# ziyangwang007/CV-SSL-MIS

Hardware: AMD Instinct MI355X
Metric: training images-or-volumes/sec/node (Mean-Teacher step) (higher is better)
Workload: dtype f32

## Files before the change

### cv-ssl-mis_amd/csrc/common.h

```cpp
#pragma once
#include <hip/hip_runtime.h>
#include <stdint.h>

#define MIS_OK 0
#define MIS_ERR_ARG (-1)
#define MIS_ERR_UNSUPPORTED (-2)
#define MIS_ERR_LAUNCH (-3)
#define MIS_ERR_WORKSPACE (-4)

#define MIS_NUM_XCD 8
#define MIS_WAVE 64

typedef float f32x4 __attribute__((ext_vector_type(4)));

typedef __bf16 mis_bf16x8 __attribute__((ext_vector_type(8)));
typedef unsigned mis_u32x4 __attribute__((ext_vector_type(4)));
struct MisBf3 { mis_u32x4 h, m, l; };

__device__ __forceinline__ void mis_bf3_split_pair(float x0, float x1, unsigned& h, unsigned& m, unsigned& l) {
    const unsigned u0 = __float_as_uint(x0), u1 = __float_as_uint(x1);
    h = __builtin_amdgcn_perm(u1, u0, 0x07060302u);
    const float r0 = x0 - __uint_as_float(u0 & 0xFFFF0000u), r1 = x1 - __uint_as_float(u1 & 0xFFFF0000u);
    const unsigned v0 = __float_as_uint(r0), v1 = __float_as_uint(r1);
    m = __builtin_amdgcn_perm(v1, v0, 0x07060302u);
// ... 81 lines not shown
__device__ __forceinline__ void dma_dwordx4(unsigned lds_byte, unsigned voff, i32x4 rsrc) {
    unsigned keep;
    asm volatile("s_mov_b32 %0, m0\n\ts_mov_b32 m0, %1\n\ts_nop 0\n\t"
                 "buffer_load_dwordx4 %2, %3, 0 offen lds\n\ts_mov_b32 m0, %0"
                 : "=&s"(keep) : "s"(lds_byte), "v"(voff), "s"(rsrc) : "memory");
}
__device__ __forceinline__ void dma_wait() { asm volatile("s_waitcnt vmcnt(0)" ::: "memory"); }

}

__device__ __forceinline__ float mis_dpp_f(float v, int ctrl) {
    switch (ctrl) {
        case 0: return __builtin_bit_cast(float, __builtin_amdgcn_update_dpp(0, __builtin_bit_cast(int, v), 0xB1, 0xF, 0xF, false));
        case 1: return __builtin_bit_cast(float, __builtin_amdgcn_update_dpp(0, __builtin_bit_cast(int, v), 0x4E, 0xF, 0xF, false));
        case 2: return __builtin_bit_cast(float, __builtin_amdgcn_update_dpp(0, __builtin_bit_cast(int, v), 0x141, 0xF, 0xF, false));
        default: return __builtin_bit_cast(float, __builtin_amdgcn_update_dpp(0, __builtin_bit_cast(int, v), 0x140, 0xF, 0xF, false));
    }
}
template <int LPR>
__device__ __forceinline__ float mis_group_sum(float v) {
    static_assert(LPR == 32 || LPR == 64, "row groups of 32 or 64 lanes");
    v += mis_dpp_f(v, 0);
    v += mis_dpp_f(v, 1);
    v += mis_dpp_f(v, 2);
    v += mis_dpp_f(v, 3);
    v += __builtin_bit_cast(float, __builtin_amdgcn_ds_swizzle(__builtin_bit_cast(int, v), (0x10 << 10) | 0x1F));
    if (LPR == 64) v += __shfl_xor(v, 32, 64);
    return v;
}

__device__ __forceinline__ float mis_sum8(float v) {
    v += mis_dpp_f(v, 0);
    v += mis_dpp_f(v, 1);
    v += mis_dpp_f(v, 2);
    return v;
}

template <int NCM>
__device__ __forceinline__ void mis_ln96_head_row(const float4 (&v)[3], const float4 (&g)[3], const float4 (&bt)[3],
                                                  const float4 (&wv)[NCM][3], float eps, float& mu, float& rs,
                                                  float (&pl)[NCM]) {
    float s = 0.f;
#pragma unroll
    for (int q = 0; q < 3; ++q) s += (v[q].x + v[q].y) + (v[q].z + v[q].w);
    mu = mis_sum8(s) / 96.f;
    float4 a[3];
    float ss = 0.f;
#pragma unroll
    for (int q = 0; q < 3; ++q) {
        a[q] = make_float4(v[q].x - mu, v[q].y - mu, v[q].z - mu, v[q].w - mu);
        ss += (a[q].x * a[q].x + a[q].y * a[q].y) + (a[q].z * a[q].z + a[q].w * a[q].w);
    }
    rs = 1.f / sqrtf(mis_sum8(ss) / 96.f + eps);
    float4 y[3];
#pragma unroll
    for (int q = 0; q < 3; ++q)
        y[q] = make_float4(a[q].x * rs * g[q].x + bt[q].x, a[q].y * rs * g[q].y + bt[q].y, a[q].z * rs * g[q].z + bt[q].z,
                           a[q].w * rs * g[q].w + bt[q].w);
#pragma unroll
    for (int n = 0; n < NCM; ++n) {
        float p = 0.f;
#pragma unroll
        for (int q = 0; q < 3; ++q) p += (y[q].x * wv[n][q].x + y[q].y * wv[n][q].y) + (y[q].z * wv[n][q].z + y[q].w * wv[n][q].w);
        pl[n] = mis_sum8(p);
    }
}

__device__ __forceinline__ float mis_wave_sum(float v) {
#pragma unroll
    for (int o = 32; o > 0; o >>= 1) v += __shfl_xor(v, o, 64);
    return v;
}

__device__ __forceinline__ double mis_wave_sum_d(double v) {
#pragma unroll
    for (int o = 32; o > 0; o >>= 1) v += __shfl_xor(v, o, 64);
    return v;
}

template <int NV>
__device__ __forceinline__ void mis_block_sum(float (&v)[NV], float* red) {
    const int lane = threadIdx.x & 63, wave = threadIdx.x >> 6;
#pragma unroll
    for (int i = 0; i < NV; ++i) v[i] = mis_wave_sum(v[i]);
    __syncthreads();
    if (lane == 0) {
#pragma unroll
        for (int i = 0; i < NV; ++i) red[wave * NV + i] = v[i];
    }
    __syncthreads();
    if (threadIdx.x == 0) {
        const int nw = blockDim.x >> 6;
#pragma unroll
        for (int i = 0; i < NV; ++i) {
            float s = 0.f;
            for (int w = 0; w < nw; ++w) s += red[w * NV + i];
            v[i] = s;
        }
    }
}

__device__ __forceinline__ void mis_philox4(uint32_t c0, uint32_t c1, uint32_t c2, uint32_t c3,
                                            uint32_t k0, uint32_t k1, uint32_t out[4]) {
#pragma unroll
    for (int r = 0; r < 10; ++r) {
        const uint64_t p0 = (uint64_t)0xD2511F53u * c0;
        const uint64_t p1 = (uint64_t)0xCD9E8D57u * c2;
        const uint32_t n0 = (uint32_t)(p1 >> 32) ^ c1 ^ k0;
        const uint32_t n1 = (uint32_t)p1;
        const uint32_t n2 = (uint32_t)(p0 >> 32) ^ c3 ^ k1;
        const uint32_t n3 = (uint32_t)p0;
        c0 = n0; c1 = n1; c2 = n2; c3 = n3;
        k0 += 0x9E3779B9u; k1 += 0xBB67AE85u;
    }
    out[0] = c0; out[1] = c1; out[2] = c2; out[3] = c3;
}

__device__ __forceinline__ float mis_u01(uint32_t r) { return (float)(r >> 8) * (1.0f / 16777216.0f); }

struct MisStepState {
    uint64_t seed;
    uint64_t offset;
    int64_t iter_num;
    float lr;
    float ema_alpha;
    float cons_weight;
    float cons_gate;
};

__device__ __forceinline__ void mis_gelu_parts(float x, float& cdf, float& u) {
    const float t = __builtin_amdgcn_rcpf(fmaf(0.3f, fabsf(x), 1.f));
    float p = 3.664988946e-02f;
    p = fmaf(p, t, -1.611761927e-01f);
    p = fmaf(p, t, 2.130432014e-01f);
    p = fmaf(p, t, -5.969779766e-02f);
    p = fmaf(p, t, 1.316696142e-01f);
    p = fmaf(p, t, 9.899286856e-02f);
    p = fmaf(p, t, 1.208983674e-01f);
    p = fmaf(p, t, 1.196200560e-01f);
    u = __builtin_amdgcn_exp2f(x * x * -0.72134752044448170f);
    const float e = p * t * u;
    cdf = x < 0.f ? e : 1.f - e;
}
__device__ __forceinline__ float mis_gelu(float x) {
    float cdf, u;
    mis_gelu_parts(x, cdf, u);
    return x * cdf;
}
__device__ __forceinline__ float mis_gelu_grad(float x) {
    float cdf, u;
    mis_gelu_parts(x, cdf, u);
    return fmaf(x * 0.3989422804014327f, u, cdf);
}
```

### cv-ssl-mis_amd/csrc/conv_fwd.hip

```cpp
#include "common.h"
#include <stdio.h>
#include <stdlib.h>

namespace {

struct ConvFwdArgs {
    const float* x; long long x_bs;
    const float* wp;
    const float* bias;
    float* y; long long y_bs;
    int N, Cin, Cout, Cin_pad, Cout_pad, D, H, W;
    int tiles_z, tiles_y, tiles_x, co_blocks;
    unsigned n_blocks, n_blocks_padded;
    int st2;
    float2* stat; long long stat_sc, stat_sn;
    int stagger, stagger_mod;
};

using namespace mis_dma;

template <int KD_, int KH_, int KW_, int TZ_, int TY_, int TX_, int CO_B_, int CI_B_, int NT_>
struct Cfg {
    static constexpr int KD = KD_, KH = KH_, KW = KW_, TZ = TZ_, TY = TY_, TX = TX_;
    static constexpr int CO_B = CO_B_, CI_B = CI_B_, NT = NT_;
// ... 218 lines not shown
            if (tid < C::CO_B) {
                const float2 p0 = red[tid], p1 = red[C::CO_B + tid], p2 = red[2 * C::CO_B + tid], p3 = red[3 * C::CO_B + tid];
                const long long tile = ((long long)tz * a.tiles_y + ty) * a.tiles_x + tx;
                a.stat[(long long)(co0 + tid) * a.stat_sc + (long long)n * a.stat_sn + tile] =
                    make_float2((p0.x + p1.x) + (p2.x + p3.x), (p0.y + p1.y) + (p2.y + p3.y));
            }
        }
        return;
    }
    float* __restrict__ yout = a.y + (long long)n * a.y_bs;
#pragma unroll
    for (int q = 0; q < C::NP; ++q) {
        const int p = (wave * C::NP + q) * 32 + 2 * lj;
        const int px = p % C::TX, py = (p / C::TX) % C::TY, pz = p / (C::TX * C::TY);
        const int gz = z0 + pz, gy = y0 + py, gx = x0 + px;
        const bool row_ok = gz < a.D && gy < a.H;
        const long long sp = ((long long)gz * a.H + gy) * a.W + gx;
#pragma unroll
        for (int m = 0; m < C::M; ++m) {
#pragma unroll
            for (int r = 0; r < 4; ++r) {
                const int co = co0 + m * 16 + lk * 4 + r;
                if (row_ok && co < a.Cout) {
                    const float bv = a.bias ? a.bias[co] : 0.f;
                    const float ve = acc[m][2 * q][r] + bv, vo = acc[m][2 * q + 1][r] + bv;
                    float* dst = yout + (long long)co * S + sp;
                    if (a.st2 && gx + 1 < a.W) {
                        *reinterpret_cast<float2*>(dst) = make_float2(ve, vo);
                    } else {
                        if (gx < a.W) dst[0] = ve;
                        if (gx + 1 < a.W) dst[1] = vo;
                    }
                }
            }
        }
    }
}

namespace small {
constexpr int TY = 8, TX = 64, HY = TY + 2, HX = TX + 2, RAW = HY * HX, NCH = (RAW + 63) / 64, XS = NCH * 64;
constexpr int CI = 16, LDS_BYTES = CI * XS * 4;
}

template <int STEP>
__device__ __forceinline__ void small_terms(const float* __restrict__ sx, int lane, const float* wreg, f32x4& acc0,
                                            f32x4& acc1) {
    if constexpr (STEP < small::CI * 12) {
        constexpr int c = STEP / 12, ir = (STEP % 12) / 3, dx = STEP % 3;
        const float b = sx[c * small::XS + ir * small::HX + dx + lane];
        if constexpr (ir <= 2) {
            constexpr int term = c * 9 + ir * 3 + dx;
            acc0 = __builtin_amdgcn_mfma_f32_4x4x1f32(wreg[term / 16], b, acc0, 4, term % 16, 0);
        }
        if constexpr (ir >= 1) {
            constexpr int term = c * 9 + (ir - 1) * 3 + dx;
            acc1 = __builtin_amdgcn_mfma_f32_4x4x1f32(wreg[term / 16], b, acc1, 4, term % 16, 0);
        }
        small_terms<STEP + 1>(sx, lane, wreg, acc0, acc1);
    }
}

__global__ __launch_bounds__(256) void conv_small_cout_kernel(const ConvFwdArgs a) {
    extern __shared__ __attribute__((aligned(16))) float mis_small_lds[];
    float* const sx = mis_small_lds;
    const unsigned L = mis_xcd_remap(blockIdx.x, a.n_blocks_padded);
    if (L >= a.n_blocks) return;
    const int tx = L % a.tiles_x, ty = (L / a.tiles_x) % a.tiles_y, n = L / (a.tiles_x * a.tiles_y);
    const int lane = threadIdx.x & 63;
    const int wave = __builtin_amdgcn_readfirstlane(threadIdx.x >> 6);
    const int y0 = ty * small::TY, x0 = tx * small::TX;
    const unsigned s_bytes = (unsigned)(a.H * a.W) * 4u;
    const i32x4 rx = make_rsrc(a.x + (long long)n * a.x_bs, (unsigned)a.Cin * s_bytes);
    const unsigned lds0 = lds_addr(sx);
#pragma unroll
    for (int p = 0; p < small::NCH; ++p) {
        const int e = p * 64 + lane;
        const int hy = e / small::HX, hx = e - hy * small::HX;
        const int gy = y0 + hy - 1, gx = x0 + hx - 1;
        const bool ok = e < small::RAW && (unsigned)gy < (unsigned)a.H && (unsigned)gx < (unsigned)a.W;
        const unsigned vo = ok ? (unsigned)(gy * a.W + gx) * 4u : OOB;
#pragma unroll
        for (int i = 0; i < 4; ++i) {
            const int c = wave + 4 * i;
            dma_dword(lds0 + (unsigned)(c * small::XS + p * 64) * 4u, vo + (unsigned)c * s_bytes, rx);
        }
    }
    float wreg[9];
#pragma unroll
    for (int k = 0; k < 9; ++k) {
        const int term = 16 * k + (lane >> 2);
        const int ci = term / 9;
        wreg[k] = ci < a.Cin_pad ? a.wp[(long long)term * a.Cout_pad + (lane & 3)] : 0.f;
    }
    dma_wait();
    __syncthreads();
    f32x4 acc[2] = {f32x4{0.f, 0.f, 0.f, 0.f}, f32x4{0.f, 0.f, 0.f, 0.f}};
    small_terms<0>(sx + (wave * 2) * small::HX, lane, wreg, acc[0], acc[1]);
#pragma unroll
    for (int r = 0; r < 2; ++r) {
        const int gy = y0 + wave * 2 + r, gx = x0 + lane;
        if (gy < a.H && gx < a.W) {
            float* __restrict__ o = a.y + (long long)n * a.y_bs + (long long)gy * a.W + gx;
#pragma unroll
            for (int m = 0; m < 4; ++m)
                if (m < a.Cout) o[(long long)m * a.H * a.W] = acc[r][m] + (a.bias ? a.bias[m] : 0.f);
        }
    }
}

template <int KD>
struct Cin1 {
    static constexpr int TZ = KD == 3 ? 4 : 1, TY = KD == 3 ? 8 : 32, TX = 16, WROWS = 8;
    static constexpr int HZ = TZ + KD - 1, HY = TY + 2, HX = TX + 2, HALO = HZ * HY * HX;
    static constexpr int TAPS = 9 * KD, NG = (TAPS + 3) / 4;
};

template <int KD>
__global__ __launch_bounds__(256) void conv_fwd_cin1_kernel(const ConvFwdArgs a) {
    using C = Cin1<KD>;
    __shared__ float sx[C::HALO];
    __shared__ float2 red[4 * 16];
    const unsigned L = mis_xcd_remap(blockIdx.x, a.n_blocks_padded);
    if (L >= a.n_blocks) return;
    unsigned t = L;
    const int tx = t % a.tiles_x; t /= a.tiles_x;
    const int ty = t % a.tiles_y; t /= a.tiles_y;
    const int tz = t % a.tiles_z; t /= a.tiles_z;
    const int n = t;
    const int z0 = tz * C::TZ, y0 = ty * C::TY, x0 = tx * C::TX;
    const int tid = threadIdx.x, lane = tid & 63, wave = tid >> 6, lk = lane >> 4, lj = lane & 15;
    const long long S = (long long)a.D * a.H * a.W;
    const float* __restrict__ xn = a.x + (long long)n * a.x_bs;
    for (int e = tid; e < C::HALO; e += 256) {
        const int hz = e / (C::HY * C::HX), r2 = e - hz * (C::HY * C::HX), hy = r2 / C::HX, hx = r2 - hy * C::HX;
        const int gz = z0 + hz - (KD == 3 ? 1 : 0), gy = y0 + hy - 1, gx = x0 + hx - 1;
        const bool ok = (unsigned)gz < (unsigned)a.D && (unsigned)gy < (unsigned)a.H && (unsigned)gx < (unsigned)a.W;
        sx[e] = ok ? xn[((long long)gz * a.H + gy) * a.W + gx] : 0.f;
    }
    float wa[C::NG];
    int toff[C::NG];
#pragma unroll
    for (int g = 0; g < C::NG; ++g) {
        const int tap = 4 * g + lk;
        wa[g] = tap < C::TAPS ? a.wp[tap * a.Cout_pad + lj] : 0.f;
        const int tc = tap < C::TAPS ? tap : C::TAPS - 1;
        toff[g] = ((tc / 9) * C::HY + (tc / 3) % 3) * C::HX + tc % 3;
    }
    float bv[4];
#pragma unroll
    for (int r = 0; r < 4; ++r) bv[r] = a.bias ? a.bias[lk * 4 + r] : 0.f;
    __syncthreads();
    const int wz = KD == 3 ? wave : 0, wy = KD == 3 ? 0 : wave * C::WROWS;
    const float* __restrict__ sb = sx + (wz * C::HY + wy) * C::HX + lj;
    float* __restrict__ yo = a.y + (long long)n * a.y_bs + ((long long)(z0 + wz) * a.H + y0 + wy) * a.W + x0 + lj;
    float s1[4] = {0.f, 0.f, 0.f, 0.f}, s2[4] = {0.f, 0.f, 0.f, 0.f};
#pragma unroll 2
    for (int row = 0; row < C::WROWS; ++row) {
        f32x4 acc = {0.f, 0.f, 0.f, 0.f};
#pragma unroll
        for (int g = 0; g < C::NG; ++g)
            acc = __builtin_amdgcn_mfma_f32_16x16x4f32(wa[g], sb[row * C::HX + toff[g]], acc, 0, 0, 0);
#pragma unroll
        for (int r = 0; r < 4; ++r) {
            const float v = acc[r] + bv[r];
            yo[(long long)(lk * 4 + r) * S + (long long)row * a.W] = v;
            s1[r] += v; s2[r] += v * v;
        }
    }
    if (a.stat) {
#pragma unroll
        for (int r = 0; r < 4; ++r)
#pragma unroll
            for (int o = 1; o < 16; o <<= 1) { s1[r] += __shfl_xor(s1[r], o, 64); s2[r] += __shfl_xor(s2[r], o, 64); }
        if (lj == 0) {
#pragma unroll
            for (int r = 0; r < 4; ++r) red[wave * 16 + lk * 4 + r] = make_float2(s1[r], s2[r]);
        }
        __syncthreads();
        if (tid < 16) {
            const float2 p0 = red[tid], p1 = red[16 + tid], p2 = red[32 + tid], p3 = red[48 + tid];
            const long long tile = ((long long)tz * a.tiles_y + ty) * a.tiles_x + tx;
            a.stat[(long long)tid * a.stat_sc + (long long)n * a.stat_sn + tile] =
                make_float2((p0.x + p1.x) + (p2.x + p3.x), (p0.y + p1.y) + (p2.y + p3.y));
        }
    }
}

int cin1_kd(const ConvFwdArgs& a, int kd, int kh, int kw) {
    if (kh != 3 || kw != 3 || a.Cin != 1 || a.Cout != 16) return 0;
    if (kd == 3 && a.D % Cin1<3>::TZ == 0 && a.H % Cin1<3>::TY == 0 && a.W % Cin1<3>::TX == 0) return 3;
    if (kd == 1 && a.D == 1 && a.H % Cin1<1>::TY == 0 && a.W % Cin1<1>::TX == 0) return 1;
    return 0;
}

template <int KD>
int launch_cin1(ConvFwdArgs a, hipStream_t stream) {
    using C = Cin1<KD>;
    a.tiles_z = a.D / C::TZ; a.tiles_y = a.H / C::TY; a.tiles_x = a.W / C::TX;
    const long long nb = (long long)a.N * a.tiles_z * a.tiles_y * a.tiles_x;
    if (nb <= 0 || nb > 0x7fffffffLL) return MIS_ERR_ARG;
    a.n_blocks = (unsigned)nb;
    a.n_blocks_padded = (unsigned)(mis_cdiv(nb, MIS_NUM_XCD) * MIS_NUM_XCD);
    hipLaunchKernelGGL(conv_fwd_cin1_kernel<KD>, dim3(a.n_blocks_padded), dim3(256), 0, stream, a);
    return mis_launch_status();
}

int launch_small_cout(ConvFwdArgs a, hipStream_t stream) {
    a.tiles_y = (int)mis_cdiv(a.H, small::TY);
    a.tiles_x = (int)mis_cdiv(a.W, small::TX);
    const long long nb = (long long)a.N * a.tiles_y * a.tiles_x;
    if (nb <= 0 || nb > 0x7fffffffLL) return MIS_ERR_ARG;
    a.n_blocks = (unsigned)nb;
    a.n_blocks_padded = (unsigned)(mis_cdiv(nb, MIS_NUM_XCD) * MIS_NUM_XCD);
    hipLaunchKernelGGL(conv_small_cout_kernel, dim3(a.n_blocks_padded), dim3(256), small::LDS_BYTES, stream, a);
    return mis_launch_status();
}

template <class C>
int launch_cfg(ConvFwdArgs a, hipStream_t stream) {
    a.tiles_z = (int)mis_cdiv(a.D, C::TZ);
    a.tiles_y = (int)mis_cdiv(a.H, C::TY);
    a.tiles_x = (int)mis_cdiv(a.W, C::TX);
    a.co_blocks = (int)mis_cdiv(a.Cout_pad, C::CO_B);
    const long long nb = (long long)a.N * a.tiles_z * a.tiles_y * a.tiles_x * a.co_blocks;
    if (nb <= 0 || nb > 0x7fffffffLL) return MIS_ERR_ARG;
    a.n_blocks = (unsigned)nb;
    a.n_blocks_padded = (unsigned)(mis_cdiv(nb, MIS_NUM_XCD) * MIS_NUM_XCD);
    static const int stagger = getenv("MIS_CF_STAGGER") ? atoi(getenv("MIS_CF_STAGGER")) : 0;
    static const int stagger_mod = getenv("MIS_CF_STAGGER_MOD") ? atoi(getenv("MIS_CF_STAGGER_MOD")) : 4;
    a.stagger = stagger; a.stagger_mod = stagger_mod;
    static std::atomic<unsigned long long> attr_done{0};
    if (mis_set_lds_attr(reinterpret_cast<const void*>(&conv_fwd_kernel<C>), C::LDS_BYTES, attr_done) != MIS_OK) return MIS_ERR_LAUNCH;
    hipLaunchKernelGGL(conv_fwd_kernel<C>, dim3(a.n_blocks_padded), dim3(256), C::LDS_BYTES, stream, a);
    return mis_launch_status();
}

}

extern "C" int mis_conv_cin_pad(int cin) { return (cin + 3) / 4 * 4; }
extern "C" int mis_conv_cout_pad(int cout) { return (cout + 15) / 16 * 16; }

namespace {

int dispatch_fwd(ConvFwdArgs a, int kd, int kh, int kw, hipStream_t stream, char* name, int name_len,
                 long long* stat_tiles = nullptr) {
#define MIS_CF(KD, KH, KW, TZ, TY, TX, COB, CIB, NT)                                                  \
    do {                                                                                              \
        if (stat_tiles) {    \
            const bool all = a.st2 && a.D % TZ == 0 && a.H % TY == 0 && a.W % TX == 0 && a.Cout % COB == 0;  \
            *stat_tiles = all ? (long long)(a.D / TZ) * (a.H / TY) * (a.W / TX) : 0;                  \
            return MIS_OK;                                                                            \
        }                                                                                             \
        if (name) {                                                                                   \
            snprintf(name, name_len, "conv_fwd_kernel<Cfg<%d, %d, %d, %d, %d, %d, %d, %d, %d>>", KD, KH, KW, \
                     TZ, TY, TX, COB, CIB, NT);                                                       \
            return MIS_OK;                                                                            \
        }                                                                                             \
        return launch_cfg<Cfg<KD, KH, KW, TZ, TY, TX, COB, CIB, NT>>(a, stream);                      \
    } while (0)
    const bool wide = a.Cout_pad >= 32 && a.Cout_pad % 32 == 0;
    if (const int c1 = cin1_kd(a, kd, kh, kw)) {
        if (stat_tiles) {
            *stat_tiles = c1 == 3 ? (long long)(a.D / Cin1<3>::TZ) * (a.H / Cin1<3>::TY) * (a.W / Cin1<3>::TX)
                                  : (long long)(a.H / Cin1<1>::TY) * (a.W / Cin1<1>::TX);
            return MIS_OK;
        }
        if (name) { snprintf(name, name_len, c1 == 3 ? "conv_fwd_cin1_kernel<3>" : "conv_fwd_cin1_kernel<1>"); return MIS_OK; }
        return c1 == 3 ? launch_cin1<3>(a, stream) : launch_cin1<1>(a, stream);
    }
    if (kd == 3 && kh == 3 && kw == 3) {
        if (a.W % 16 == 0 || a.W >= 64) {
            if (wide) MIS_CF(3, 3, 3, 4, 8, 16, 32, 4, 8); else MIS_CF(3, 3, 3, 4, 8, 16, 16, 4, 8);
        } else if (a.W % 8 == 0 && a.W >= 16) {
            const long long nb888 = (long long)a.N * mis_cdiv(a.D, 8) * mis_cdiv(a.H, 8) * mis_cdiv(a.W, 8) *
                                    mis_cdiv(a.Cout_pad, wide ? 32 : 16);
            if (nb888 < 512) {
                if (wide) MIS_CF(3, 3, 3, 4, 8, 8, 32, 4, 4); else MIS_CF(3, 3, 3, 4, 8, 8, 16, 4, 4);
            }
            if (wide) MIS_CF(3, 3, 3, 8, 8, 8, 32, 4, 8); else MIS_CF(3, 3, 3, 8, 8, 8, 16, 4, 8);
        } else if (a.W > 12) {
            if (wide) MIS_CF(3, 3, 3, 4, 4, 16, 32, 4, 4); else MIS_CF(3, 3, 3, 4, 4, 16, 16, 4, 4);
        } else if (a.W > 8) {
            MIS_CF(3, 3, 3, 2, 4, 16, 16, 4, 2);
        } else {
            MIS_CF(3, 3, 3, 2, 8, 8, 16, 4, 2);
        }
    }
    if (kd == 1 && kh == 3 && kw == 3) {
        if (a.D != 1) return MIS_ERR_UNSUPPORTED;
        if (a.Cout <= 4 && a.Cin_pad <= small::CI && a.H * (long long)a.W * (a.Cin + 1) * 4 < (1LL << 31)) {
            if (stat_tiles) { *stat_tiles = 0; return MIS_OK; }
            if (name) { snprintf(name, name_len, "conv_small_cout_kernel"); return MIS_OK; }
            return launch_small_cout(a, stream);
        }
        if (a.W >= 128) {
            if (wide) MIS_CF(1, 3, 3, 1, 16, 32, 32, 8, 8); else MIS_CF(1, 3, 3, 1, 16, 32, 16, 8, 8);
        } else {
            if (wide) MIS_CF(1, 3, 3, 1, 16, 16, 32, 8, 4); else MIS_CF(1, 3, 3, 1, 16, 16, 16, 8, 4);
        }
    }
    if (kd == 1 && kh == 1 && kw == 1) {
        if (a.D > 1) {
            if (wide) MIS_CF(1, 1, 1, 4, 8, 16, 32, 16, 8); else MIS_CF(1, 1, 1, 4, 8, 16, 16, 16, 8);
        } else if (a.W >= 32) {
            if (wide) MIS_CF(1, 1, 1, 1, 16, 32, 32, 16, 8); else MIS_CF(1, 1, 1, 1, 16, 32, 16, 16, 8);
        } else {
            if (wide) MIS_CF(1, 1, 1, 1, 16, 16, 32, 16, 4); else MIS_CF(1, 1, 1, 1, 16, 16, 16, 16, 4);
        }
    }
#undef MIS_CF
    return MIS_ERR_UNSUPPORTED;
}

ConvFwdArgs make_fwd_args(const float* x, long long x_bs, const float* wp, const float* bias, float* y,
                          long long y_bs, int N, int Cin, int Cout, int D, int H, int W) {
    ConvFwdArgs a{};
    a.x = x; a.x_bs = x_bs; a.wp = wp; a.bias = bias; a.y = y; a.y_bs = y_bs;
    a.N = N; a.Cin = Cin; a.Cout = Cout; a.D = D; a.H = H; a.W = W;
    a.Cin_pad = mis_conv_cin_pad(Cin);
    a.Cout_pad = mis_conv_cout_pad(Cout);
    a.st2 = (W % 2 == 0 && y_bs % 2 == 0 && ((uintptr_t)y & 7) == 0) ? 1 : 0;
    return a;
}

}

extern "C" int mis_conv_fwd(const float* x, long long x_bs, const float* wp, const float* bias,
                            float* y, long long y_bs, int N, int Cin, int Cout, int D, int H, int W,
                            int kd, int kh, int kw, hipStream_t stream) {
    if (!x || !wp || !y || N <= 0 || Cin <= 0 || Cout <= 0 || D <= 0 || H <= 0 || W <= 0) return MIS_ERR_ARG;
    const long long S = (long long)D * H * W;
    if (x_bs < (long long)Cin * S || y_bs < (long long)Cout * S) return MIS_ERR_ARG;
    if (((long long)Cin + 32) * S * 4 >= (1LL << 30) || ((uintptr_t)wp & 15) != 0) return MIS_ERR_UNSUPPORTED;
    return dispatch_fwd(make_fwd_args(x, x_bs, wp, bias, y, y_bs, N, Cin, Cout, D, H, W), kd, kh, kw, stream,
                        nullptr, 0);
}

extern "C" long long mis_conv_fwd_stat_tiles(int N, int Cin, int Cout, int D, int H, int W, int kd, int kh, int kw) {
    if (N <= 0 || Cin <= 0 || Cout <= 0 || D <= 0 || H <= 0 || W <= 0) return MIS_ERR_ARG;
    long long tiles = 0;
    const int st = dispatch_fwd(make_fwd_args(nullptr, 0, nullptr, nullptr, nullptr, 0, N, Cin, Cout, D, H, W), kd, kh,
                                kw, nullptr, nullptr, 0, &tiles);
    return st ? st : tiles;
}

extern "C" int mis_conv_fwd_stats(const float* x, long long x_bs, const float* wp, const float* bias, float* y,
                                  long long y_bs, int N, int Cin, int Cout, int D, int H, int W, int kd, int kh, int kw,
                                  float* stat, long long stat_sc, long long stat_sn, hipStream_t stream) {
    if (!x || !wp || !y || !stat || N <= 0 || Cin <= 0 || Cout <= 0 || D <= 0 || H <= 0 || W <= 0) return MIS_ERR_ARG;
    const long long S = (long long)D * H * W;
    if (x_bs < (long long)Cin * S || y_bs < (long long)Cout * S) return MIS_ERR_ARG;
    if (((long long)Cin + 32) * S * 4 >= (1LL << 30) || ((uintptr_t)wp & 15) != 0 || ((uintptr_t)stat & 7) != 0)
        return MIS_ERR_UNSUPPORTED;
    ConvFwdArgs a = make_fwd_args(x, x_bs, wp, bias, y, y_bs, N, Cin, Cout, D, H, W);
    long long tiles = 0;
    int st = dispatch_fwd(a, kd, kh, kw, nullptr, nullptr, 0, &tiles);
    if (st) return st;
    if (tiles <= 0) return MIS_ERR_UNSUPPORTED;
    a.stat = reinterpret_cast<float2*>(stat); a.stat_sc = stat_sc; a.stat_sn = stat_sn;
    return dispatch_fwd(a, kd, kh, kw, stream, nullptr, 0);
}

extern "C" int mis_conv_fwd_kernel_name(int N, int Cin, int Cout, int D, int H, int W, int kd, int kh, int kw,
                                        char* name, int name_len) {
    if (!name || name_len <= 0 || N <= 0 || Cin <= 0 || Cout <= 0 || D <= 0 || H <= 0 || W <= 0) return MIS_ERR_ARG;
    return dispatch_fwd(make_fwd_args(nullptr, 0, nullptr, nullptr, nullptr, 0, N, Cin, Cout, D, H, W), kd, kh, kw,
                        nullptr, name, name_len);
}
```

### cv-ssl-mis_amd/csrc/conv_wgrad_cin1.hip

```cpp
#include "common.h"

namespace {

template <int KD>
struct WC1 {
    static constexpr int TZ = KD == 3 ? 4 : 1, TY = KD == 3 ? 8 : 32, TX = 32;
    static constexpr int HZ = TZ + KD - 1, HY = TY + 2, HX = TX + 2, HALO = HZ * HY * HX;
    static constexpr int TAPS = 9 * KD, NG = (TAPS + 15) / 16;
};

struct Cin1Norm {
    const float* y; long long y_bs;
    const float* mean; const float* rstd; const float* gamma; const float* beta;
    const float2* sums;
    float slope;
    int per_sample;
};

struct Cin1Args {
    const float* x; long long x_bs;
    const float* dy; long long dy_bs;
    float* ws;
    int N, D, H, W;
    int tz, ty, tx, n_tiles;
};

template <int KD, bool NORM>
__global__ __launch_bounds__(256) void wgrad_cin1_kernel(const Cin1Args a, const Cin1Norm nb) {
    using C = WC1<KD>;
    constexpr int TZ = C::TZ, TY = C::TY, TX = C::TX, HY = C::HY, HX = C::HX, HALO = C::HALO, NG = C::NG;
    __shared__ float sx[HALO];
    const int tid = threadIdx.x, lane = tid & 63, wave = tid >> 6;
    const int lk = lane >> 4, lj = lane & 15;
    const long long S = (long long)a.D * a.H * a.W;
    int toff[NG];
#pragma unroll
    for (int g = 0; g < NG; ++g) {
        const int tap = g * 16 + lj < C::TAPS ? g * 16 + lj : C::TAPS - 1;
        toff[g] = ((tap / 9) * HY + (tap / 3) % 3) * HX + tap % 3;
    }
    f32x4 acc[NG];
#pragma unroll
    for (int g = 0; g < NG; ++g) acc[g] = f32x4{0.f, 0.f, 0.f, 0.f};
    const int wz = KD == 3 ? wave : 0, wy = KD == 3 ? 0 : wave * 8;
    for (int t = blockIdx.x; t < a.n_tiles; t += gridDim.x) {
        int r = t;
        const int bx = r % a.tx; r /= a.tx;
        const int by = r % a.ty; r /= a.ty;
        const int bz = r % a.tz; r /= a.tz;
        const int n = r;
        const int z0 = bz * TZ, y0 = by * TY, x0 = bx * TX;
        const float* __restrict__ xn = a.x + (long long)n * a.x_bs;
        __syncthreads();
        for (int e = tid; e < HALO; e += 256) {
            const int hz = e / (HY * HX), r2 = e - hz * (HY * HX), hy = r2 / HX, hx = r2 - hy * HX;
            const int gz = z0 + hz - (KD == 3 ? 1 : 0), gy = y0 + hy - 1, gx = x0 + hx - 1;
            const bool ok = (unsigned)gz < (unsigned)a.D && (unsigned)gy < (unsigned)a.H && (unsigned)gx < (unsigned)a.W;
            sx[e] = ok ? xn[((long long)gz * a.H + gy) * a.W + gx] : 0.f;
        }
        __syncthreads();
        const long long voff = (long long)lj * S + ((long long)(z0 + wz) * a.H + y0 + wy) * a.W + x0 + 4 * lk;
        const float* __restrict__ dyp = a.dy + (long long)n * a.dy_bs + voff;
        const float* __restrict__ yp = NORM ? nb.y + (long long)n * nb.y_bs + voff : nullptr;
        float cm = 0.f, crs = 1.f, cga = 1.f, cbe = 0.f, s1 = 0.f, s2 = 0.f;
        if constexpr (NORM) {
            const int grp = nb.per_sample ? n * 16 + lj : lj;
            cm = nb.mean[grp]; crs = nb.rstd[grp];
            cga = nb.gamma ? nb.gamma[lj] : 1.f; cbe = nb.beta ? nb.beta[lj] : 0.f;
            const float2 sm = nb.sums[grp];
            s1 = sm.x; s2 = sm.y;
        }
        const float* __restrict__ sb = sx + (wz * HY + wy) * HX + 4 * lk;
#pragma unroll 4
        for (int it = 0; it < 16; ++it) {
            const int row = it >> 1, half = it & 1;
            f32x4 d4 = *reinterpret_cast<const f32x4*>(dyp + (long long)row * a.W + half * 16);
            if constexpr (NORM) {
                const f32x4 y4 = *reinterpret_cast<const f32x4*>(yp + (long long)row * a.W + half * 16);
#pragma unroll
                for (int s = 0; s < 4; ++s) {
                    const float xh = (y4[s] - cm) * crs;
                    const float dz = xh * cga + cbe > 0.f ? d4[s] : d4[s] * nb.slope;
                    d4[s] = cga * crs * (dz - s1 - xh * s2);
                }
            }
            const float* __restrict__ sp = sb + row * HX + half * 16;
#pragma unroll
            for (int s = 0; s < 4; ++s) {
#pragma unroll
                for (int g = 0; g < NG; ++g)
                    acc[g] = __builtin_amdgcn_mfma_f32_16x16x4f32(d4[s], sp[toff[g] + s], acc[g], 0, 0, 0);
            }
        }
    }
    float* __restrict__ out = a.ws + ((long long)blockIdx.x * 4 + wave) * (NG * 256);
#pragma unroll
    for (int g = 0; g < NG; ++g)
#pragma unroll
        for (int r = 0; r < 4; ++r) out[g * 256 + (lk * 4 + r) * 16 + lj] = acc[g][r];
}

__global__ __launch_bounds__(256) void wgrad_cin1_reduce_kernel(const float* __restrict__ ws, float* __restrict__ dw,
                                                                int parts, int taps, int ng, int accumulate) {
    __shared__ float red[4];
    const int o = blockIdx.x;
    const int co = o / taps, tap = o - co * taps;
    const float* p = ws + (tap / 16) * 256 + co * 16 + tap % 16;
    float s = 0.f;
    for (int k = threadIdx.x; k < parts; k += 256) s += p[(long long)k * (ng * 256)];
#pragma unroll
    for (int d = 32; d > 0; d >>= 1) s += __shfl_xor(s, d, 64);
    if ((threadIdx.x & 63) == 0) red[threadIdx.x >> 6] = s;
    __syncthreads();
    if (threadIdx.x == 0) {
        s = (red[0] + red[1]) + (red[2] + red[3]);
        dw[o] = accumulate ? dw[o] + s : s;
    }
}

int grid_for(long long n_tiles) { return (int)(n_tiles < 1024 ? n_tiles : 1024); }

template <int KD>
long long tiles_of(int N, int D, int H, int W) {
    return (long long)N * (D / WC1<KD>::TZ) * (H / WC1<KD>::TY) * (W / WC1<KD>::TX);
}

template <int KD>
int launch_cin1_kd(const float* x, long long x_bs, const float* dy, long long dy_bs, const Cin1Norm* nb, float* dw,
                   float* ws, int N, int D, int H, int W, int accumulate, hipStream_t stream) {
    using C = WC1<KD>;
    Cin1Args a{};
    a.x = x; a.x_bs = x_bs; a.dy = dy; a.dy_bs = dy_bs; a.ws = ws;
    a.N = N; a.D = D; a.H = H; a.W = W;
    a.tz = D / C::TZ; a.ty = H / C::TY; a.tx = W / C::TX;
    const long long n_tiles = tiles_of<KD>(N, D, H, W);
    if (n_tiles > 0x7fffffffLL) return MIS_ERR_ARG;
    a.n_tiles = (int)n_tiles;
    const int grid = grid_for(n_tiles);
    if (nb) hipLaunchKernelGGL((wgrad_cin1_kernel<KD, true>), dim3(grid), dim3(256), 0, stream, a, *nb);
    else hipLaunchKernelGGL((wgrad_cin1_kernel<KD, false>), dim3(grid), dim3(256), 0, stream, a, Cin1Norm{});
    hipLaunchKernelGGL(wgrad_cin1_reduce_kernel, dim3(16 * C::TAPS), dim3(256), 0, stream, ws, dw, grid * 4, C::TAPS, C::NG,
                       accumulate);
    return mis_launch_status();
}

}

bool mis_wgrad_cin1_eligible(int N, int Cin, int Cout, int D, int H, int W, int kd, int kh, int kw) {
    if (kh != 3 || kw != 3 || Cin != 1 || Cout != 16) return false;
    if (kd == 3) return D % WC1<3>::TZ == 0 && H % WC1<3>::TY == 0 && W % WC1<3>::TX == 0;
    return kd == 1 && D == 1 && H % WC1<1>::TY == 0 && W % WC1<1>::TX == 0;
}

long long mis_wgrad_cin1_workspace_bytes(int N, int D, int H, int W) {
    return D == 1 ? (long long)grid_for(tiles_of<1>(N, D, H, W)) * 4 * WC1<1>::NG * 256 * 4
                  : (long long)grid_for(tiles_of<3>(N, D, H, W)) * 4 * WC1<3>::NG * 256 * 4;
}

static int launch_cin1(const float* x, long long x_bs, const float* dy, long long dy_bs, const Cin1Norm* nb, float* dw,
                       float* ws, long long ws_bytes, int N, int D, int H, int W, int accumulate, hipStream_t stream) {
    if (((uintptr_t)dy & 15) || dy_bs % 4) return MIS_ERR_UNSUPPORTED;
    if (ws_bytes < mis_wgrad_cin1_workspace_bytes(N, D, H, W)) return MIS_ERR_WORKSPACE;
    return D == 1 ? launch_cin1_kd<1>(x, x_bs, dy, dy_bs, nb, dw, ws, N, D, H, W, accumulate, stream)
                  : launch_cin1_kd<3>(x, x_bs, dy, dy_bs, nb, dw, ws, N, D, H, W, accumulate, stream);
}

int mis_wgrad_cin1(const float* x, long long x_bs, const float* dy, long long dy_bs, float* dw, float* ws,
                   long long ws_bytes, int N, int D, int H, int W, int accumulate, hipStream_t stream) {
    return launch_cin1(x, x_bs, dy, dy_bs, nullptr, dw, ws, ws_bytes, N, D, H, W, accumulate, stream);
}

extern "C" int mis_conv_wgrad_cin1_norm_eligible(int N, int Cout, int D, int H, int W) {
    return mis_wgrad_cin1_eligible(N, 1, Cout, D, H, W, D == 1 ? 1 : 3, 3, 3) ? 1 : 0;
}

extern "C" int mis_conv_wgrad_cin1_norm(const float* x, long long x_bs, const float* da, long long da_bs, const float* y,
                                        long long y_bs, int N, int D, int H, int W, int per_sample, const float* mean,
                                        const float* rstd, const float* gamma, const float* beta, const float* sums,
                                        float slope, float* dw, float* workspace, long long workspace_bytes,
                                        int accumulate, hipStream_t stream) {
    if (!x || !da || !y || !mean || !rstd || !sums || !dw || !workspace || N <= 0) return MIS_ERR_ARG;
    if (!mis_wgrad_cin1_eligible(N, 1, 16, D, H, W, D == 1 ? 1 : 3, 3, 3) || (per_sample && (gamma || beta)))
        return MIS_ERR_UNSUPPORTED;
    if (((uintptr_t)y & 15) || y_bs % 4 || ((uintptr_t)sums & 7)) return MIS_ERR_UNSUPPORTED;
    const Cin1Norm nb{y, y_bs, mean, rstd, gamma, beta, reinterpret_cast<const float2*>(sums), slope, per_sample};
    return launch_cin1(x, x_bs, da, da_bs, &nb, dw, workspace, workspace_bytes, N, D, H, W, accumulate, stream);
}
```

### cv-ssl-mis_amd/csrc/norm_act.hip

```cpp
#include "common.h"
#include <type_traits>

namespace {

struct Geo {
    int N, C, per_sample;
    long long S;
    long long x_bs;
    int P;
    int nchunks;
    int G;
    int cg;
};

__host__ __device__ inline int pick_P(long long S) {
    long long p = (S + 16383) / 16384;
    if (p < 1) p = 1;
    if (p > 32) p = 32;
    return (int)p;
}

Geo make_geo(int N, int C, long long S, long long x_bs, int per_sample, int cg = 1) {
    Geo g;
    g.N = N; g.C = C; g.S = S; g.x_bs = x_bs; g.per_sample = per_sample; g.cg = cg;
// ... 46 lines not shown
    long long So;
};

__device__ __forceinline__ void pool_grad4(const PoolGrad& pg, int n, int c, int C, unsigned e, float (&g)[4]) {
    const unsigned HW = (unsigned)(pg.H * pg.W);
    const unsigned z = e / HW, r = e - z * HW;
    const unsigned y = r / (unsigned)pg.W, x0 = r - y * (unsigned)pg.W;
    const unsigned zo = z / (unsigned)pg.pz;
    const unsigned o = (zo * ((unsigned)pg.H >> 1) + (y >> 1)) * ((unsigned)pg.W >> 1) + (x0 >> 1);
    const unsigned local = (z - zo * (unsigned)pg.pz) * 4u + (y & 1u) * 2u;
    const float2 d = *reinterpret_cast<const float2*>(pg.dp + (long long)n * pg.dp_bs + (long long)c * pg.So + o);
    const unsigned code = *reinterpret_cast<const unsigned short*>(pg.idx + ((long long)n * C + c) * pg.So + o);
    const unsigned c0 = code & 0xffu, c1 = code >> 8;
    g[0] = c0 == local ? d.x : 0.f;
    g[1] = c0 == local + 1u ? d.x : 0.f;
    g[2] = c1 == local ? d.y : 0.f;
    g[3] = c1 == local + 1u ? d.y : 0.f;
}

__device__ __forceinline__ void block_sum2_d(double (&v)[2], double* red) {
    const int lane = threadIdx.x & 63, wave = threadIdx.x >> 6;
    v[0] = mis_wave_sum_d(v[0]); v[1] = mis_wave_sum_d(v[1]);
    __syncthreads();
    if (lane == 0) { red[wave * 2] = v[0]; red[wave * 2 + 1] = v[1]; }
    __syncthreads();
    if (threadIdx.x == 0) {
        v[0] = ((red[0] + red[2]) + red[4]) + red[6];
        v[1] = ((red[1] + red[3]) + red[5]) + red[7];
    }
}

template <typename T2>
__global__ __launch_bounds__(256) void stats_partial_kernel(const float* __restrict__ x, Geo g,
                                                            T2* __restrict__ part) {
    __shared__ double red[8];
    const int p = blockIdx.x, k = blockIdx.y, grp = blockIdx.z;
    const int n = g.per_sample ? grp / g.C : k;
    const int c = g.per_sample ? grp % g.C : grp;
    const float* __restrict__ base = x + (long long)n * g.x_bs + (long long)c * g.S;
    const long long units = g.S >> 2;
    const long long per = (units + g.P - 1) / g.P;
    const long long u0 = p * per, u1 = (u0 + per < units) ? u0 + per : units;
    double v[2] = {0.0, 0.0};
    for (long long u = u0 + threadIdx.x; u < u1; u += 256) {
        const float4 q = *reinterpret_cast<const float4*>(base + u * 4);
        v[0] += ((double)q.x + (double)q.y) + ((double)q.z + (double)q.w);
        v[1] += ((double)q.x * q.x + (double)q.y * q.y) + ((double)q.z * q.z + (double)q.w * q.w);
    }
    block_sum2_d(v, red);
    if (threadIdx.x == 0) {
        T2 o;
        o.x = (decltype(o.x))v[0]; o.y = (decltype(o.y))v[1];
        part[((long long)grp * g.nchunks + k) * g.P + p] = o;
    }
}

template <typename T2>
__global__ __launch_bounds__(256) void stats_final_kernel(const T2* __restrict__ part, Geo g, float eps,
                                                          float* __restrict__ mean, float* __restrict__ rstd,
                                                          float* running_mean, float* running_var,
                                                          long long* num_batches, float momentum, int tpg) {
    constexpr bool WIDE = std::is_same<T2, double2>::value;
    __shared__ double red[16];
    const int lane = threadIdx.x & 63, wave = threadIdx.x >> 6;
    const int grp = tpg == 256 ? (int)blockIdx.x : (int)blockIdx.x * 4 + wave;
    const int t = tpg == 256 ? (int)threadIdx.x : lane;
    const int np = g.nchunks * g.P;
    double s = 0.0, ss = 0.0, sf = 0.0, ssf = 0.0;
    if (grp < g.G) {
        const T2* __restrict__ pg = part + (long long)grp * np;
        int i = t;
        for (; i + 3 * tpg < np; i += 4 * tpg) {
            const T2 q0 = pg[i], q1 = pg[i + tpg], q2 = pg[i + 2 * tpg], q3 = pg[i + 3 * tpg];
            s += q0.x; ss += q0.y; s += q1.x; ss += q1.y; s += q2.x; ss += q2.y; s += q3.x; ss += q3.y;
            if constexpr (WIDE) {
                sf += (float)q0.x; ssf += (float)q0.y; sf += (float)q1.x; ssf += (float)q1.y;
                sf += (float)q2.x; ssf += (float)q2.y; sf += (float)q3.x; ssf += (float)q3.y;
            }
        }
        for (; i < np; i += tpg) {
            const T2 q = pg[i];
            s += q.x; ss += q.y;
            if constexpr (WIDE) { sf += (float)q.x; ssf += (float)q.y; }
        }
    }
    s = mis_wave_sum_d(s); ss = mis_wave_sum_d(ss);
    if constexpr (WIDE) { sf = mis_wave_sum_d(sf); ssf = mis_wave_sum_d(ssf); }
    if (tpg == 256) {
        if (lane == 0) { red[wave] = s; red[4 + wave] = ss; red[8 + wave] = sf; red[12 + wave] = ssf; }
        __syncthreads();
        s = ((red[0] + red[1]) + red[2]) + red[3];
        ss = ((red[4] + red[5]) + red[6]) + red[7];
        sf = ((red[8] + red[9]) + red[10]) + red[11];
        ssf = ((red[12] + red[13]) + red[14]) + red[15];
    }
    if (grp < g.G && t == 0) {
        const double E = (double)g.nchunks * (double)g.S;
        double m = s / E;
        double var = ss / E - m * m;
        if (var < 0.0) var = 0.0;
        if constexpr (WIDE) {
            const double mf = sf / E;
            double vf = ssf / E - mf * mf;
            if (vf < 0.0) vf = 0.0;
            if (mf * mf <= 3.0 * vf) { m = mf; var = vf; }
        }
        mean[grp] = (float)m;
        rstd[grp] = (float)(1.0 / sqrt(var + (double)eps));
        if (running_mean && !g.per_sample) {
            const double unb = E > 1.0 ? var * E / (E - 1.0) : var;
            running_mean[grp] = (float)((1.0 - momentum) * running_mean[grp] + momentum * m);
            running_var[grp] = (float)((1.0 - momentum) * running_var[grp] + momentum * unb);
            if (num_batches && grp == 0) *num_batches += 1;
        }
    }
}

template <typename T2>
void launch_stats_final(const T2* part, const Geo& g, float eps, float* mean, float* rstd, float* running_mean,
                        float* running_var, long long* num_batches, float momentum, hipStream_t stream) {
    const int tpg = g.nchunks * g.P > 256 ? 256 : 64;
    hipLaunchKernelGGL(stats_final_kernel<T2>, dim3(tpg == 256 ? g.G : (g.G + 3) / 4), dim3(256), 0, stream, part, g, eps,
                       mean, rstd, running_mean, running_var, num_batches, momentum, tpg);
}

__global__ __launch_bounds__(256) void channel_sum_final_kernel(const float2* __restrict__ part, Geo g,
                                                                float* __restrict__ out, int accumulate) {
    const int grp = blockIdx.x * 4 + (threadIdx.x >> 6), lane = threadIdx.x & 63;
    if (grp >= g.G) return;
    const int np = g.nchunks * g.P;
    double s = 0.0;
    for (int i = lane; i < np; i += 64) s += part[(long long)grp * np + i].x;
    s = mis_wave_sum_d(s);
    if (lane == 0) out[grp] = accumulate ? out[grp] + (float)s : (float)s;
}

__global__ void running_to_stats_kernel(const float* __restrict__ rm, const float* __restrict__ rv, float eps,
                                        float* __restrict__ mean, float* __restrict__ rstd, int C) {
    const int c = blockIdx.x * blockDim.x + threadIdx.x;
    if (c < C) { mean[c] = rm[c]; rstd[c] = 1.f / sqrtf(rv[c] + eps); }
}

constexpr int APPLY_U = 4;

template <bool RES>
__global__ __launch_bounds__(256) void apply_fwd_kernel(const float* __restrict__ x, Geo g,
                                                        const float* __restrict__ mean,
                                                        const float* __restrict__ rstd,
                                                        const float* __restrict__ gamma,
                                                        const float* __restrict__ beta, float slope, DropCfg d,
                                                        float* __restrict__ y, long long y_bs, ResArgs ra) {
    const int c = blockIdx.y, n = blockIdx.z;
    const int grp = g.per_sample ? (n * g.C + c) / g.cg : c;
    const float sc = (gamma ? gamma[c] : 1.f) * rstd[grp];
    const float sh = (beta ? beta[c] : 0.f) - mean[grp] * sc;
    const float* __restrict__ xb = x + (long long)n * g.x_bs + (long long)c * g.S;
    float* __restrict__ yb = y + (long long)n * y_bs + (long long)c * g.S;
    const unsigned long long lbase = ((unsigned long long)n * g.C + c) * g.S;
    const long long units = g.S >> 2;
    const bool drop = d.p > 0.f;
#pragma unroll
    for (int i = 0; i < APPLY_U; ++i) {
        const long long u = ((long long)blockIdx.x * APPLY_U + i) * 256 + threadIdx.x;
        if (u >= units) break;
        const float4 q = *reinterpret_cast<const float4*>(xb + u * 4);
        float v[4] = {q.x * sc + sh, q.y * sc + sh, q.z * sc + sh, q.w * sc + sh};
        float4 rq = make_float4(0.f, 0.f, 0.f, 0.f);
        if constexpr (RES) {
            rq = *reinterpret_cast<const float4*>(ra.r + (long long)n * ra.r_bs + (long long)c * g.S + u * 4);
            if (!ra.post) { v[0] += rq.x; v[1] += rq.y; v[2] += rq.z; v[3] += rq.w; }
        }
#pragma unroll
        for (int j = 0; j < 4; ++j) v[j] = v[j] > 0.f ? v[j] : v[j] * slope;
        if constexpr (RES) {
            if (ra.post) { v[0] += rq.x; v[1] += rq.y; v[2] += rq.z; v[3] += rq.w; }
        }
        if (drop) {
            float s[4];
            drop_scale4(d, lbase + u * 4, (unsigned)(n * g.C + c), s);
#pragma unroll
            for (int j = 0; j < 4; ++j) v[j] *= s[j];
        }
        *reinterpret_cast<float4*>(yb + u * 4) = make_float4(v[0], v[1], v[2], v[3]);
    }
}

template <int PZ>
__global__ __launch_bounds__(256) void apply_fwd_pool_kernel(const float* __restrict__ x, Geo g,
                                                             const float* __restrict__ mean,
                                                             const float* __restrict__ rstd,
                                                             const float* __restrict__ gamma,
                                                             const float* __restrict__ beta, float slope, DropCfg d,
                                                             float* __restrict__ y, long long y_bs,
                                                             float* __restrict__ pooled, long long p_bs,
                                                             unsigned char* __restrict__ idx, int H, int W) {
    const int Ho = H >> 1, Wo = W >> 1, Wq = Wo >> 2;
    const int pl = blockIdx.x * 256 + threadIdx.x;
    if (pl >= Ho * Wq) return;
    const int zo = blockIdx.y, nc = blockIdx.z;
    const int n = nc / g.C, c = nc - n * g.C;
    const int yo = pl / Wq, xq = pl - yo * Wq;
    const int grp = g.per_sample ? (n * g.C + c) / g.cg : c;
    const float sc = (gamma ? gamma[c] : 1.f) * rstd[grp];
    const float sh = (beta ? beta[c] : 0.f) - mean[grp] * sc;
    const float* __restrict__ xb = x + (long long)n * g.x_bs + (long long)c * g.S;
    float* __restrict__ yb = y + (long long)n * y_bs + (long long)c * g.S;
    const unsigned long long lbase = ((unsigned long long)n * g.C + c) * g.S;
    const bool drop = d.p > 0.f;
    float best[4] = {-INFINITY, -INFINITY, -INFINITY, -INFINITY};
    unsigned bi[4] = {0, 0, 0, 0};
#pragma unroll
    for (int dz = 0; dz < PZ; ++dz)
#pragma unroll
        for (int dy = 0; dy < 2; ++dy) {
            const unsigned e = (unsigned)(((zo * PZ + dz) * H + (yo * 2 + dy)) * W + xq * 8);
            float v[8];
#pragma unroll
            for (int h = 0; h < 2; ++h) {
                const float4 q = *reinterpret_cast<const float4*>(xb + e + 4 * h);
                float t[4] = {q.x * sc + sh, q.y * sc + sh, q.z * sc + sh, q.w * sc + sh};
#pragma unroll
                for (int j = 0; j < 4; ++j) t[j] = t[j] > 0.f ? t[j] : t[j] * slope;
                if (drop) {
                    float s4[4];
                    drop_scale4(d, lbase + e + 4 * h, (unsigned)(n * g.C + c), s4);
#pragma unroll
                    for (int j = 0; j < 4; ++j) t[j] *= s4[j];
                }
                *reinterpret_cast<float4*>(yb + e + 4 * h) = make_float4(t[0], t[1], t[2], t[3]);
#pragma unroll
                for (int j = 0; j < 4; ++j) v[4 * h + j] = t[j];
            }
#pragma unroll
            for (int j = 0; j < 4; ++j)
#pragma unroll
                for (int dx = 0; dx < 2; ++dx) {
                    const float t = v[2 * j + dx];
                    if (t > best[j] || t != t) { best[j] = t; bi[j] = dz * 4 + dy * 2 + dx; }
                }
        }
    const long long So = (long long)gridDim.y * Ho * Wo;
    const unsigned o = (unsigned)((zo * Ho + yo) * Wo + xq * 4);
    *reinterpret_cast<float4*>(pooled + (long long)n * p_bs + (long long)c * So + o) =
        make_float4(best[0], best[1], best[2], best[3]);
    *reinterpret_cast<unsigned*>(idx + (long long)nc * So + o) = bi[0] | (bi[1] << 8) | (bi[2] << 16) | (bi[3] << 24);
}

template <bool DACC, bool RES = false>
__global__ __launch_bounds__(256) void bwd_partial_kernel(const float* __restrict__ x, Geo g,
                                                          const float* __restrict__ da, long long da_bs,
                                                          const float* __restrict__ mean,
                                                          const float* __restrict__ rstd,
                                                          const float* __restrict__ gamma,
                                                          const float* __restrict__ beta, float slope, DropCfg d,
                                                          float2* __restrict__ part, PoolGrad pg, ResArgs ra) {
    __shared__ double red[8];
    const int p = blockIdx.x, k = blockIdx.y, grp = blockIdx.z;
    const int n = g.per_sample ? grp / g.C : k;
    const int c = g.per_sample ? grp % g.C : grp;
    const int sg = g.per_sample ? grp / g.cg : grp;
    const float m = mean[sg], rs = rstd[sg];
    const float ga = gamma ? gamma[c] : 1.f, be = beta ? beta[c] : 0.f;
    const float* __restrict__ xb = x + (long long)n * g.x_bs + (long long)c * g.S;
    const float* __restrict__ db = da ? da + (long long)n * da_bs + (long long)c * g.S : nullptr;
    const unsigned long long lbase = ((unsigned long long)n * g.C + c) * g.S;
    const long long units = g.S >> 2;
    const long long per = (units + g.P - 1) / g.P;
    const long long u0 = p * per, u1 = (u0 + per < units) ? u0 + per : units;
    const bool drop = d.p > 0.f;
    typedef typename std::conditional<DACC, double, float>::type acc_t;
    acc_t v[2] = {0, 0};
    for (long long u = u0 + threadIdx.x; u < u1; u += 256) {
        const float4 q = *reinterpret_cast<const float4*>(xb + u * 4);
        const float4 gq = db ? *reinterpret_cast<const float4*>(db + u * 4) : make_float4(0.f, 0.f, 0.f, 0.f);
        const float xs[4] = {q.x, q.y, q.z, q.w};
        float gs[4] = {gq.x, gq.y, gq.z, gq.w};
        float rv[4] = {0.f, 0.f, 0.f, 0.f};
        if constexpr (RES) {
            const float4 rq = *reinterpret_cast<const float4*>(ra.r + (long long)n * ra.r_bs + (long long)c * g.S + u * 4);
            rv[0] = rq.x; rv[1] = rq.y; rv[2] = rq.z; rv[3] = rq.w;
        }
        if (pg.dp) {
            float pgr[4];
            pool_grad4(pg, n, c, g.C, (unsigned)(u * 4), pgr);
#pragma unroll
            for (int j = 0; j < 4; ++j) gs[j] += pgr[j];
        }
        if (drop) {
            float s[4];
            drop_scale4(d, lbase + u * 4, (unsigned)(n * g.C + c), s);
#pragma unroll
            for (int j = 0; j < 4; ++j) gs[j] *= s[j];
        }
#pragma unroll
        for (int j = 0; j < 4; ++j) {
            const float xh = (xs[j] - m) * rs;
            const float z = xh * ga + be + rv[j];
            const float dz = z > 0.f ? gs[j] : gs[j] * slope;
            v[0] += dz;
            v[1] += (acc_t)dz * (acc_t)xh;
        }
    }
    if constexpr (DACC) {
        block_sum2_d(v, red);
    } else {
        mis_block_sum<2>(v, reinterpret_cast<float*>(red));
    }
    if (threadIdx.x == 0) part[((long long)grp * g.nchunks + k) * g.P + p] = make_float2((float)v[0], (float)v[1]);
}

__global__ __launch_bounds__(256) void bwd_final_kernel(const float2* __restrict__ part, Geo g,
                                                        float2* __restrict__ sums, float* dgamma, float* dbeta,
                                                        int accumulate) {
    const int grp = blockIdx.x * 4 + (threadIdx.x >> 6), lane = threadIdx.x & 63;
    if (grp >= g.G) return;
    const int np = g.nchunks * g.P;
    double s1 = 0.0, s2 = 0.0;
    for (int i = lane; i < np; i += 64) {
        const float2 q = part[(long long)grp * np + i];
        s1 += q.x; s2 += q.y;
    }
    s1 = mis_wave_sum_d(s1); s2 = mis_wave_sum_d(s2);
    if (lane == 0) {
        const double E = (double)g.nchunks * (double)g.S;
        sums[grp] = make_float2((float)(s1 / E), (float)(s2 / E));
        if (dgamma && !g.per_sample) {
// ... 885 lines not shown
```

### cv-ssl-mis_amd/mis_hip/lib.py

```python
import ctypes
import os

import torch

_HERE = os.path.dirname(os.path.abspath(__file__))
LIB_PATH = os.environ.get("MIS_HIP_LIB") or os.path.join(_HERE, "libmis_hip.so")

_lib = None

_ERRORS = {
    -1: "MIS_ERR_ARG (bad pointer / size / stride)",
    -2: "MIS_ERR_UNSUPPORTED (shape not covered by the gfx950 kernel family)",
    -3: "MIS_ERR_LAUNCH (HIP launch failure)",
    -4: "MIS_ERR_WORKSPACE (workspace too small)",
}

c_p = ctypes.c_void_p
c_i = ctypes.c_int
c_ll = ctypes.c_longlong
c_f = ctypes.c_float
c_d = ctypes.c_double
c_u = ctypes.c_uint
c_ull = ctypes.c_ulonglong

PROTOTYPES = {
    "mis_abi_version": (c_i, []),
    "mis_conv_cin_pad": (c_i, [c_i]),
    "mis_conv_cout_pad": (c_i, [c_i]),
    "mis_conv_packed_floats": (c_ll, [c_i, c_i, c_i, c_i]),
    "mis_conv_pack_weights": (c_i, [c_p, c_p, c_i, c_i, c_i, c_i, c_p]),
    "mis_conv_pack_job_bytes": (c_i, []),
    "mis_conv_pack_job": (c_ll, [c_p, c_p, c_p, c_i, c_i, c_i, c_i, c_ll]),
    "mis_conv_pack_batch": (c_i, [c_p, c_i, c_ll, c_p]),
    "mis_conv_fwd": (c_i, [c_p, c_ll, c_p, c_p, c_p, c_ll, c_i, c_i, c_i, c_i, c_i, c_i, c_i, c_i, c_i, c_p]),
    "mis_conv_fwd_stat_tiles": (c_ll, [c_i, c_i, c_i, c_i, c_i, c_i, c_i, c_i, c_i]),
    "mis_conv_fwd_stats": (c_i, [c_p, c_ll, c_p, c_p, c_p, c_ll, c_i, c_i, c_i, c_i, c_i, c_i, c_i, c_i, c_i, c_p, c_ll,
                                 c_ll, c_p]),
    "mis_norm_stats_finalize": (c_i, [c_p, c_i, c_i, c_ll, c_i, c_i, c_f, c_p, c_p, c_p, c_p, c_p, c_f, c_p]),
    "mis_conv_fwd_kernel_name": (c_i, [c_i, c_i, c_i, c_i, c_i, c_i, c_i, c_i, c_i, ctypes.c_char_p, c_i]),
    "mis_conv3d_wino_select": (c_i, [c_i, c_i, c_i, c_i, c_i, c_i]),
    "mis_conv3d_wino_stat_tiles": (c_ll, [c_i, c_i, c_i, c_i]),
    "mis_conv3d_wino_kernel_name": (c_i, [c_i, ctypes.c_char_p, c_i]),
    "mis_conv3d_wino_fwd": (c_i, [c_p, c_ll, c_p, c_p, c_p, c_ll, c_i, c_i, c_i, c_i, c_i, c_i, c_p, c_ll, c_ll, c_i, c_p]),
    "mis_conv1x1_gemm_workspace_bytes": (c_ll, [c_i, c_i, c_i, c_ll]),
    "mis_conv1x1_gemm": (c_i, [c_p, c_ll, c_p, c_ll, c_p, c_p, c_ll, c_i, c_i, c_i, c_ll, c_i, c_p, c_ll, c_p]),
    "mis_conv1x1_wgrad_workspace_bytes": (c_ll, [c_i, c_i, c_i, c_ll]),
    "mis_conv1x1_wgrad": (c_i, [c_p, c_ll, c_p, c_ll, c_p, c_ll, c_i, c_i, c_i, c_ll, c_i, c_p, c_ll, c_p]),
    "mis_conv3d_wino_fwd_splits": (c_i, [c_i, c_i, c_i, c_i, c_i, c_i, c_i]),
    "mis_conv3d_wino_fwd_workspace_bytes": (c_ll, [c_i, c_i, c_i, c_i, c_i, c_i, c_i]),
    "mis_conv3d_wino_fwd_ws": (c_i, [c_p, c_ll, c_p, c_p, c_p, c_ll, c_i, c_i, c_i, c_i, c_i, c_i, c_p, c_ll, c_ll, c_i, c_p, c_ll,
                                     c_p]),
    "mis_conv3d_wino_dgrad_norm": (c_i, [c_p, c_ll, c_p, c_p, c_ll, c_i, c_i, c_i, c_i, c_i, c_i, c_p, c_ll, c_p, c_f, c_p,
                                         c_ll, c_ll, c_i, c_p]),
    "mis_norm_res_act_fwd": (c_i, [c_p, c_ll, c_p, c_ll, c_p, c_ll, c_i, c_i, c_ll, c_i, c_p, c_p, c_p, c_p, c_f, c_i, c_p]),
    "mis_norm_res_act_bwd": (c_i, [c_p, c_ll, c_p, c_ll, c_p, c_ll, c_p, c_ll, c_p, c_ll, c_i, c_i, c_i, c_ll, c_i, c_p, c_p,
                                   c_p, c_p, c_f, c_p, c_p, c_i, c_i, c_p, c_ll, c_p]),
    "mis_norm_act_bwd_tiles": (c_i, [c_p, c_ll, c_p, c_ll, c_p, c_ll, c_i, c_i, c_ll, c_p, c_p, c_f, c_p, c_i, c_p, c_p]),
    "mis_conv2d_wino_select": (c_i, [c_i, c_i, c_i, c_i, c_i]),
    "mis_conv2d_wino_stat_tiles": (c_ll, [c_i, c_i, c_i]),
    "mis_conv2d_wino_kernel_name": (c_i, [c_i, ctypes.c_char_p, c_i]),
    "mis_conv2d_wino_fwd": (c_i, [c_p, c_ll, c_p, c_p, c_p, c_ll, c_i, c_i, c_i, c_i, c_i, c_p, c_ll, c_ll, c_i, c_p]),
    "mis_conv2d_wino_wgrad_select": (c_i, [c_i, c_i, c_i, c_i, c_i]),
    "mis_conv2d_wino_wgrad_kernel_name": (c_i, [c_i, ctypes.c_char_p, c_i]),
    "mis_conv2d_wino_wgrad_workspace_bytes": (c_ll, [c_i, c_i, c_i, c_i, c_i, c_i]),
    "mis_conv2d_wino_wgrad": (c_i, [c_p, c_ll, c_p, c_ll, c_p, c_p, c_ll, c_i, c_i, c_i, c_i, c_i, c_i, c_i, c_p]),
    "mis_conv3d_wino_wgrad_select": (c_i, [c_i, c_i, c_i, c_i, c_i, c_i]),
    "mis_conv3d_wino_wgrad_kernel_name": (c_i, [c_i, ctypes.c_char_p, c_i]),
    "mis_conv3d_wino_wgrad_workspace_bytes": (c_ll, [c_i, c_i, c_i, c_i, c_i, c_i, c_i]),
    "mis_conv3d_wino_wgrad": (c_i, [c_p, c_ll, c_p, c_ll, c_p, c_p, c_ll, c_i, c_i, c_i, c_i, c_i, c_i, c_i, c_i, c_p]),
    "mis_conv_wgrad_workspace_bytes": (c_ll, [c_i, c_i, c_i, c_i, c_i, c_i, c_i, c_i, c_i]),
    "mis_conv_wgrad_kernel_name": (c_i, [c_i, c_i, c_i, c_i, c_i, c_i, c_i, c_i, c_i, ctypes.c_char_p, c_i]),
    "mis_conv_wgrad": (c_i, [c_p, c_ll, c_p, c_ll, c_p, c_p, c_ll, c_i, c_i, c_i, c_i, c_i, c_i, c_i, c_i, c_i,
                             c_i, c_p]),
    "mis_norm_workspace_bytes": (c_ll, [c_i, c_i, c_ll, c_i]),
    "mis_norm_stats": (c_i, [c_p, c_ll, c_i, c_i, c_ll, c_i, c_f, c_p, c_p, c_p, c_p, c_p, c_f, c_p, c_ll, c_p]),
    "mis_channel_sum": (c_i, [c_p, c_ll, c_i, c_i, c_ll, c_p, c_i, c_p, c_ll, c_p]),
    "mis_norm_stats_from_running":(c_i, [c_p, c_p, c_f, c_p, c_p, c_i, c_p]),
    "mis_norm_act_fwd": (c_i, [c_p, c_ll, c_p, c_ll, c_i, c_i, c_ll, c_i, c_p, c_p, c_p, c_p, c_f, c_f, c_u, c_p,
                               c_p, c_p]),
    "mis_norm_act_bwd": (c_i, [c_p, c_ll, c_p, c_ll, c_p, c_ll, c_i, c_i, c_ll, c_i, c_p, c_p, c_p, c_p, c_f, c_f,
                               c_u, c_p, c_p, c_p, c_p, c_i, c_p, c_ll, c_p]),
    "mis_norm_act_fwd_g": (c_i, [c_p, c_ll, c_p, c_ll, c_i, c_i, c_ll, c_i, c_i, c_p, c_p, c_p, c_p, c_f, c_f, c_u, c_p,
                                 c_p, c_p]),
    "mis_norm_act_bwd_g": (c_i, [c_p, c_ll, c_p, c_ll, c_p, c_ll, c_i, c_i, c_ll, c_i, c_i, c_i, c_p, c_p, c_p, c_p, c_f,
                                 c_f, c_u, c_p, c_p, c_p, c_p, c_i, c_p, c_ll, c_p]),
    "mis_norm_act_fwd_pool": (c_i, [c_p, c_ll, c_p, c_ll, c_p, c_ll, c_p, c_i, c_i, c_i, c_i, c_i, c_i, c_i, c_p, c_p, c_p,
                                    c_p, c_f, c_f, c_u, c_p, c_p, c_p]),
    "mis_norm_act_bwd_pool": (c_i, [c_p, c_ll, c_p, c_ll, c_p, c_ll, c_p, c_p, c_ll, c_i, c_i, c_i, c_i, c_i, c_i, c_i, c_p,
                                    c_p, c_p, c_p, c_f, c_f, c_u, c_p, c_p, c_p, c_p, c_i, c_p, c_ll, c_p]),
    "mis_norm_act_bwd_sums": (c_i, [c_p, c_ll, c_p, c_ll, c_i, c_i, c_ll, c_i, c_p, c_p, c_p, c_p, c_f, c_p, c_p, c_p, c_i,
                                    c_p, c_ll, c_p]),
    "mis_conv_wgrad_cin1_norm_eligible": (c_i, [c_i, c_i, c_i, c_i, c_i]),
    "mis_conv_wgrad_cin1_norm": (c_i, [c_p, c_ll, c_p, c_ll, c_p, c_ll, c_i, c_i, c_i, c_i, c_i, c_p, c_p, c_p, c_p, c_p,
                                       c_f, c_p, c_p, c_ll, c_i, c_p]),
    "mis_norm_head_eligible": (c_i, [c_i, c_i]),
    "mis_norm_head_workspace_bytes": (c_ll, [c_i, c_i, c_ll, c_i, c_i]),
    "mis_norm_head_fwd": (c_i, [c_p, c_ll, c_i, c_i, c_ll, c_i, c_p, c_p, c_p, c_p, c_f, c_f, c_u, c_p, c_p, c_p, c_p, c_i,
                                c_p, c_ll, c_p]),
    "mis_norm_head_bwd": (c_i, [c_p, c_ll, c_p, c_ll, c_p, c_ll, c_i, c_i, c_ll, c_i, c_p, c_p, c_p, c_p, c_f, c_f, c_u,
                                c_p, c_p, c_p, c_i, c_p, c_p, c_i, c_p, c_p, c_i, c_p, c_ll, c_p]),
    "mis_maxpool2_fwd": (c_i, [c_p, c_ll, c_p, c_ll, c_p, c_i, c_i, c_i, c_i, c_i, c_p]),
    "mis_maxpool2_bwd": (c_i, [c_p, c_ll, c_p, c_p, c_ll, c_i, c_i, c_i, c_i, c_i, c_i, c_p]),
    "mis_upsample2_fwd": (c_i, [c_p, c_ll, c_p, c_ll, c_i, c_i, c_i, c_i, c_i, c_i, c_p]),
    "mis_upsample2_bwd": (c_i, [c_p, c_ll, c_p, c_ll, c_i, c_i, c_i, c_i, c_i, c_i, c_i, c_p]),
    "mis_loss_tail_workspace_bytes": (c_ll, [c_i, c_i, c_ll]),
    "mis_loss_tail": (c_i, [c_p, c_ll, c_p, c_ll, c_p, c_i, c_i, c_i, c_i, c_ll, c_f, c_p, c_f, c_p, c_p, c_ll,
                            c_p, c_ll, c_p]),
    "mis_cross_teaching_tail_workspace_bytes": (c_ll, [c_i, c_i, c_ll]),
    "mis_cross_teaching_tail": (c_i, [c_p, c_ll, c_p, c_ll, c_p, c_i, c_i, c_i, c_i, c_ll, c_f, c_p, c_p, c_p, c_ll,
                                      c_p, c_ll, c_p]),
    "mis_softmax_mean_accumulate": (c_i, [c_p, c_ll, c_p, c_ll, c_i, c_i, c_i, c_ll, c_f, c_i, c_p]),
    "mis_uamt_tail_workspace_bytes": (c_ll, [c_i, c_i, c_ll]),
    "mis_uamt_tail": (c_i, [c_p, c_ll, c_p, c_ll, c_p, c_ll, c_p, c_i, c_i, c_i, c_i, c_ll, c_f, c_p, c_ll, c_d, c_f,
                            c_p, c_p, c_ll, c_p, c_ll, c_p]),
    "mis_beta_sample": (c_i, [c_p, c_i, c_d, c_u, c_p, c_p]),
    "mis_ict_mix": (c_i, [c_p, c_p, c_p, c_i, c_i, c_ll, c_p]),
    "mis_ict_tail_workspace_bytes": (c_ll, [c_i, c_i, c_ll]),
    "mis_ict_tail": (c_i, [c_p, c_ll, c_p, c_ll, c_p, c_ll, c_p, c_p, c_i, c_i, c_i, c_i, c_ll, c_f, c_p, c_f, c_p, c_p,
                           c_ll, c_p, c_ll, c_p]),
    "mis_rot90": (c_i, [c_p, c_ll, c_p, c_ll, c_i, c_i, c_i, c_i, c_p, c_ll, c_p, c_i, c_p]),
    "mis_dct_tail_workspace_bytes": (c_ll, [c_i, c_i, c_i, c_i, c_i]),
    "mis_dct_tail": (c_i, [c_p, c_ll, c_p, c_ll, c_p, c_i, c_i, c_i, c_i, c_i, c_i, c_p, c_ll, c_p, c_i, c_f, c_f, c_p, c_p,
                           c_ll, c_p, c_ll, c_p, c_ll, c_p]),
    "mis_grad_combine": (c_i, [c_p, c_p, c_ll, c_i, c_p]),
    "mis_triple_view_tail_workspace_bytes": (c_ll, [c_i, c_i, c_ll]),
    "mis_triple_view_tail": (c_i, [c_p, c_ll, c_p, c_ll, c_p, c_ll, c_p, c_i, c_i, c_i, c_i, c_ll, c_f, c_p, c_p, c_p, c_p,
                                   c_p, c_ll, c_p, c_ll, c_p, c_ll, c_p, c_ll, c_p]),
    "mis_cross_pseudo_tail": (c_i, [c_p, c_ll, c_p, c_ll, c_p, c_i, c_i, c_i, c_i, c_ll, c_f, c_p, c_i, c_p, c_p, c_ll,
                                    c_p, c_ll, c_p]),
    "mis_cross_pseudo_mt_tail": (c_i, [c_p, c_ll, c_p, c_ll, c_p, c_ll, c_p, c_i, c_i, c_i, c_i, c_ll, c_f, c_f, c_p,
                                       c_i, c_p, c_p, c_ll, c_p, c_ll, c_p]),
    "mis_dice_workspace_bytes": (c_ll, [c_i, c_i, c_ll]),
    "mis_dice_loss_fwd": (c_i, [c_p, c_ll, c_p, c_i, c_i, c_i, c_ll, c_p, c_p, c_p, c_ll, c_p]),
    "mis_dice_loss_bwd": (c_i, [c_p, c_ll, c_p, c_i, c_i, c_i, c_ll, c_p, c_p, c_p, c_ll, c_p]),
    "mis_softmax_mse": (c_i, [c_p, c_ll, c_p, c_ll, c_p, c_ll, c_p, c_ll, c_i, c_i, c_ll, c_i, c_p]),
    "mis_ema_update": (c_i, [c_p, c_p, c_ll, c_f, c_p]),
    "mis_sgd_ema_step": (c_i, [c_p, c_p, c_p, c_p, c_ll, c_f, c_f, c_f, c_f, c_f, c_p, c_p]),
    "mis_teacher_noise": (c_i, [c_p, c_p, c_ll, c_f, c_f, c_u, c_p, c_p]),
    "mis_step_init": (c_i, [c_p, c_ull, c_ll, c_d, c_d, c_d, c_d, c_d, c_ll, c_ll, c_i, c_p]),
    "mis_step_advance": (c_i, [c_p, c_d, c_d, c_d, c_d, c_d, c_ll, c_ll, c_i, c_p]),
    "mis_argmax_channels": (c_i, [c_p, c_ll, c_p, c_i, c_i, c_ll, c_p]),
    "mis_conv_k2s2_eligible": (c_i, [c_i, c_i, c_i, c_i, c_i, c_i]),
    "mis_conv_k2s2_down": (c_i, [c_p, c_ll, c_p, c_p, c_p, c_ll, c_i, c_i, c_i, c_i, c_i, c_i, c_i, c_p]),
    "mis_conv_k2s2_up": (c_i, [c_p, c_ll, c_p, c_p, c_p, c_ll, c_i, c_i, c_i, c_i, c_i, c_i, c_i, c_p]),
    "mis_conv_k2s2_wgrad_eligible": (c_i, [c_i, c_i, c_i, c_i, c_i]),
    "mis_conv_k2s2_wgrad_workspace_bytes": (c_ll, [c_i, c_i]),
    "mis_conv_k2s2_wgrad": (c_i, [c_p, c_ll, c_p, c_ll, c_p, c_i, c_i, c_i, c_i, c_i, c_i, c_i, c_p, c_ll, c_p]),
    "mis_debug_poison_lds": (c_i, [c_p, c_p]),
    "mis_debug_spin": (c_i, [c_i, c_i, c_i, c_p, c_p]),
    "mis_debug_wgrad_prof": (c_i, [c_p]),
    "mis_space_to_depth2": (c_i, [c_p, c_ll, c_p, c_ll, c_p, c_i, c_i, c_i, c_i, c_i, c_i, c_i, c_p]),
    "mis_space_to_depth2d": (c_i, [c_p, c_ll, c_p, c_ll, c_p, c_i, c_i, c_i, c_i, c_i, c_i, c_p]),
    "mis_add": (c_i, [c_p, c_ll, c_p, c_ll, c_p, c_ll, c_i, c_i, c_ll, c_p]),
    "mis_gemm_workspace_bytes": (c_ll, [c_i, c_i, c_i, c_i]),
    "mis_gemm_dw_workspace_bytes": (c_ll, [c_i, c_i, c_i]),
    "mis_gemm_dw": (c_i, [c_p, c_ll, c_p, c_ll, c_p, c_ll, c_p, c_i, c_i, c_i, c_i, c_p, c_ll, c_p]),
    "mis_gemm_dw_parts": (c_i, [c_p, c_ll, c_p, c_ll, c_p, c_ll, c_p, c_i, c_i, c_i, c_i, c_p, c_ll, c_p, c_p]),
    "mis_gemm_set_split_precision": (c_i, [c_i]),
    "mis_gemm_nt_kernel_name": (c_i, [c_i, c_i, c_i, c_i, ctypes.c_char_p, c_i]),
    "mis_gemm_tn_kernel_name": (c_i, [c_p, c_ll, c_p, c_ll, c_p, c_ll, c_i, c_i, c_i, ctypes.c_char_p, c_i]),
    "mis_gemm_expand_ln_head": (c_i, [c_p, c_ll, c_p, c_ll, c_p, c_i, c_i, c_i, c_i, c_i, c_i, c_p, c_p, c_p, c_i, c_f, c_p, c_p,
                                      c_p, c_ll, c_p]),
    "mis_gemm_split_bytes": (c_ll, [c_i, c_i]),
    "mis_gemm_split_b": (c_i, [c_p, c_ll, c_i, c_i, c_p, c_p]),
    "mis_gemm_split_b_layout": (c_i, [c_p, c_ll, c_i, c_i, c_p, c_i, c_p]),
    "mis_gemm_split_job_layout": (c_ll, [c_p, c_p, c_ll, c_i, c_i, c_p, c_ll, c_i]),
    "mis_gemm_nt_split_natural": (c_i, [c_i, c_i, c_i]),
    "mis_gemm_nt_split_layout": (c_i, [c_p, c_ll, c_p, c_p, c_ll, c_p, c_i, c_i, c_i, c_i, c_i, c_p, c_ll, c_p, c_ll, c_p, c_ll,
                                       c_i, c_i, c_i, c_i, c_p, c_ll, c_i, c_p]),
    "mis_gemm_nt_split_layout_kernel_name": (c_i, [c_i, c_i, c_i, c_i, c_i, ctypes.c_char_p, c_i]),
    "mis_gemm_expand_ln_head_split": (c_i, [c_p, c_ll, c_p, c_p, c_i, c_i, c_i, c_i, c_i, c_i, c_p, c_p, c_p, c_i, c_f, c_p, c_p, c_p,
                                            c_ll, c_p]),
    "mis_gemm_nt_residual_ln": (c_i, [c_p, c_ll, c_p, c_p, c_i, c_i, c_i, c_p, c_ll, c_p, c_ll, c_p, c_ll, c_p, c_p, c_f, c_p, c_ll,
                                      c_p, c_p, c_p]),
    "mis_gemm_split_job_bytes": (c_ll, []),
    "mis_gemm_split_job": (c_ll, [c_p, c_p, c_ll, c_i, c_i, c_p, c_ll]),
    "mis_gemm_split_batch": (c_i, [c_p, c_i, c_ll, c_p]),
    "mis_gemm_nt_split_workspace_bytes": (c_ll, [c_i, c_i, c_i]),
    "mis_gemm_nt_split": (c_i, [c_p, c_ll, c_p, c_p, c_ll, c_p, c_i, c_i, c_i, c_i, c_i, c_p, c_ll, c_p, c_ll, c_p, c_ll,
                                c_i, c_i, c_i, c_i, c_p, c_ll, c_p]),
    "mis_gemm_nt_split_kernel_name": (c_i, [c_i, c_i, c_i, c_i, ctypes.c_char_p, c_i]),
    "mis_gemm_expand": (c_i, [c_p, c_ll, c_p, c_ll, c_p, c_i, c_i, c_i, c_i, c_i, c_i, c_p]),
    "mis_gemm": (c_i, [c_p, c_ll, c_p, c_ll, c_p, c_ll, c_p, c_i, c_i, c_i, c_i, c_i, c_p, c_ll, c_p]),
    "mis_gemm_ex": (c_i, [c_p, c_ll, c_p, c_ll, c_p, c_ll, c_p, c_i, c_i, c_i, c_i, c_p, c_ll, c_p, c_ll, c_p, c_ll, c_p,
                          c_ll, c_p]),
    "mis_droppath_table": (c_i, [c_p, c_p, c_p, c_i, c_i, c_p, c_p]),
    "mis_transpose": (c_i, [c_p, c_ll, c_p, c_ll, c_i, c_i, c_p]),
    "mis_win3d_gather": (c_i, [c_p, c_p] + [c_i] * 12 + [c_p]),
    "mis_win3d_windows": (c_ll, [c_i] * 7),
    "mis_merge3d": (c_i, [c_p, c_p, c_i, c_i, c_i, c_i, c_i, c_i, c_p]),
    "mis_win3d_attn_fwd": (c_i, [c_p, c_ll, c_p, c_ll, c_p, c_p, c_p, c_i, c_i, c_i, c_i, c_p]),
    "mis_win3d_attn_workspace_bytes": (c_ll, [c_i, c_i, c_i]),
    "mis_win3d_attn_bwd": (c_i, [c_p, c_ll, c_p, c_p, c_ll, c_p, c_ll, c_p, c_p, c_p, c_p, c_i, c_i, c_i, c_i, c_i, c_p,
                                 c_ll, c_p]),
    "mis_transpose_job_bytes": (c_ll, []),
    "mis_transpose_job": (c_ll, [c_p, c_p, c_p, c_i, c_i, c_ll]),
    "mis_transpose_batch": (c_i, [c_p, c_i, c_ll, c_p]),
    "mis_layernorm_fwd": (c_i, [c_p, c_ll, c_p, c_ll, c_p, c_p, c_p, c_p, c_ll, c_i, c_f, c_p]),
    "mis_colreduce_workspace_bytes": (c_ll, [c_ll, c_i]),
    "mis_layernorm_bwd": (c_i, [c_p, c_ll, c_p, c_ll, c_p, c_ll, c_p, c_p, c_p, c_p, c_p, c_ll, c_i, c_i, c_i, c_p,
                                c_ll, c_p]),
    "mis_layernorm_bwd_parts": (c_i, [c_p, c_ll, c_p, c_ll, c_p, c_ll, c_p, c_p, c_p, c_ll, c_i, c_i, c_p, c_ll, c_p]),
    "mis_layernorm_bwd_final": (c_i, [c_p, c_ll, c_ll, c_i, c_p, c_p, c_i, c_p]),
    "mis_colsum_job_bytes": (c_ll, []),
    "mis_colreduce_slabs": (c_ll, [c_ll]),
    "mis_colsum_job": (c_ll, [c_p, c_p, c_ll, c_ll, c_i, c_i, c_p, c_p, c_i, c_ll]),
    "mis_colsum_batch": (c_i, [c_p, c_i, c_ll, c_p]),
    "mis_layernorm_bwd_residual_parts": (c_i, [c_p, c_ll, c_p, c_ll, c_p, c_ll, c_p, c_ll, c_i, c_p, c_ll, c_p, c_ll, c_p, c_p,
                                               c_p, c_ll, c_i, c_p, c_ll, c_p]),
    "mis_colsum": (c_i, [c_p, c_ll, c_ll, c_i, c_p, c_i, c_p, c_ll, c_p]),
    "mis_gelu": (c_i, [c_p, c_p, c_p, c_ll, c_i, c_p]),
    "mis_residual_droppath": (c_i, [c_p, c_ll, c_p, c_ll, c_p, c_ll, c_p, c_ll, c_ll, c_i, c_ll, c_f, c_u, c_p, c_p,
                                    c_i, c_p]),
    "mis_token_rearrange": (c_i, [c_p, c_ll, c_p, c_ll, c_i, c_i, c_i, c_i, c_i, c_i, c_i, c_p]),
    "mis_patch_im2col": (c_i, [c_p, c_ll, c_p, c_i, c_i, c_i, c_i, c_p]),
    "mis_ln_head_fwd": (c_i, [c_p, c_ll, c_p, c_p, c_p, c_p, c_p, c_p, c_ll, c_i, c_ll, c_i, c_i, c_f, c_p]),
    "mis_ln_head_workspace_bytes": (c_ll, [c_ll, c_i, c_i]),
    "mis_ln_head_bwd": (c_i, [c_p, c_ll, c_p, c_p, c_p, c_p, c_p, c_p, c_ll, c_p, c_ll, c_i, c_p, c_p, c_p, c_i, c_i, c_ll,
                              c_i, c_i, c_p, c_ll, c_p]),
    "mis_ln_head_bwd_unshuffle": (c_i, [c_p, c_ll, c_p, c_p, c_p, c_p, c_p, c_p, c_ll, c_p, c_ll, c_i, c_p, c_p, c_p, c_i, c_i, c_i,
                                        c_i, c_i, c_i, c_i, c_p, c_ll, c_p]),
    "mis_head_fwd": (c_i, [c_p, c_ll, c_p, c_p, c_ll, c_i, c_ll, c_i, c_i, c_p]),
    "mis_head_workspace_bytes": (c_ll, [c_i, c_i]),
    "mis_head_bwd": (c_i, [c_p, c_ll, c_p, c_p, c_ll, c_p, c_ll, c_p, c_i, c_i, c_ll, c_i, c_i, c_p, c_ll, c_p]),
    "mis_window_attention_fwd": (c_i, [c_p, c_ll, c_p, c_ll, c_p, c_i, c_i, c_i, c_i, c_i, c_f, c_p]),
    "mis_window_attention_workspace_bytes": (c_ll, [c_i, c_i, c_i, c_i]),
    "mis_window_attention_bwd": (c_i, [c_p, c_ll, c_p, c_ll, c_p, c_ll, c_p, c_p, c_i, c_i, c_i, c_i, c_i, c_i, c_f,
                                       c_p, c_ll, c_p]),
    "mis_patch_im2col_c": (c_i, [c_p, c_ll, c_p, c_i, c_i, c_i, c_i, c_i, c_p]),
    "mis_window_attention_fwd_ws": (c_i, [c_p, c_ll, c_p, c_ll, c_p, c_i, c_i, c_i, c_i, c_i, c_f, c_i, c_p]),
    "mis_window_attention_workspace_bytes_ws": (c_ll, [c_i, c_i, c_i, c_i, c_i]),
    "mis_window_attention_bwd_ws": (c_i, [c_p, c_ll, c_p, c_ll, c_p, c_ll, c_p, c_p, c_i, c_i, c_i, c_i, c_i, c_i, c_f,
                                          c_i, c_p, c_ll, c_p]),
    "mis_window_attention_bwd_parts_ws": (c_i, [c_p, c_ll, c_p, c_ll, c_p, c_ll, c_p, c_i, c_i, c_i, c_i, c_i, c_f, c_i, c_p,
                                                c_ll, c_p]),
    "mis_window_attention_dtable_ws": (c_i, [c_p, c_ll, c_p, c_i, c_i, c_i, c_i, c_i, c_i, c_p]),
    "mis_window_attention_table_partials": (c_i, [c_i, c_i, c_i, c_i, c_i, c_p, c_p]),
    "mis_full_attention_fwd": (c_i, [c_p, c_ll, c_p, c_ll, c_p, c_i, c_i, c_i, c_f, c_p]),
    "mis_full_attention_workspace_bytes": (c_ll, [c_i, c_i, c_i]),
    "mis_full_attention_bwd": (c_i, [c_p, c_ll, c_p, c_ll, c_p, c_ll, c_p, c_i, c_i, c_i, c_f, c_p, c_ll, c_p]),
    "mis_patch3d_im2col": (c_i, [c_p, c_ll, c_p, c_i, c_i, c_i, c_i, c_i, c_p]),
    "mis_add_rowcycle": (c_i, [c_p, c_ll, c_p, c_p, c_ll, c_ll, c_i, c_i, c_p]),
    "mis_sum_rowcycle": (c_i, [c_p, c_ll, c_p, c_ll, c_i, c_i, c_p]),
    "mis_augment2d": (c_i, [c_p, c_p, c_p, c_i, c_i, c_i, c_p, c_p, c_p]),
    "mis_crop_rotflip3d": (c_i, [c_p, c_p, c_p, c_i, c_i, c_i, c_i, c_p, c_p, c_i, c_p]),
    "mis_surface_metrics_workspace_bytes": (c_ll, [c_i, c_i, c_i]),
    "mis_surface_metrics": (c_i, [c_p, c_p, c_i, c_i, c_i, c_i, c_i, c_p, c_p, c_ll, c_p]),
# ... 176 lines not shown
```

### cv-ssl-mis_amd/mis_hip/ops.py

```python
import ctypes as _ctypes
import os as _os

import torch

from . import lib as _l

_scratch = {}


def _geom(t):
    if t.dim() != 5 or t.dtype != torch.float32:
        raise RuntimeError(f"expected 5-D fp32 [N,C,D,H,W], got {tuple(t.shape)} {t.dtype}")
    _l.require_gpu(t)
    N, C, D, H, W = t.shape
    S = D * H * W
    st = t.stride()
    if C > 1 and st[1] != S or (D > 1 and st[2] != H * W) or (H > 1 and st[3] != W) or (W > 1 and st[4] != 1):
        raise RuntimeError(f"activation view must be dense in (C,D,H,W); strides {st} shape {tuple(t.shape)}")
    bs = st[0] if N > 1 else max(st[0], C * S)
    if bs < C * S:
        bs = C * S
    return N, C, D, H, W, S, bs


# ... 372 lines not shown
        nb = L.mis_conv2d_wino_wgrad_workspace_bytes(N, Cin, Cout, H, W, wino2)
        if nb < 0:
            _l.check(nb, "mis_conv2d_wino_wgrad_workspace_bytes")
        ws = scratch(nb, "wgrad")
        _l.check(L.mis_conv2d_wino_wgrad(_l.ptr(x), xbs, _l.ptr(dy), dbs, _l.ptr(dw), _l.ptr(ws), ws.numel(), N, Cin, Cout,
                                         H, W, int(accumulate), wino2, _l.stream_ptr()), "mis_conv2d_wino_wgrad")
        buf = _ctypes.create_string_buffer(96)
        _l.check(L.mis_conv2d_wino_wgrad_kernel_name(wino2, buf, 96), "mis_conv2d_wino_wgrad_kernel_name")
        return buf.value.decode()
    nb = L.mis_conv_wgrad_workspace_bytes(N, Cin, Cout, D, H, W, kd, kh, kw)
    if nb < 0:
        _l.check(nb, "mis_conv_wgrad_workspace_bytes")
    ws = scratch(nb, "wgrad")
    _tag(f"direct_wgrad:k{kd}{kh}{kw}@{W}")
    _l.check(L.mis_conv_wgrad(_l.ptr(x), xbs, _l.ptr(dy), dbs, _l.ptr(dw), _l.ptr(ws), ws.numel(), N, Cin, Cout,
                              D, H, W, kd, kh, kw, int(accumulate), _l.stream_ptr()), "mis_conv_wgrad")
    buf = _ctypes.create_string_buffer(96)
    _l.check(L.mis_conv_wgrad_kernel_name(N, Cin, Cout, D, H, W, kd, kh, kw, buf, 96), "mis_conv_wgrad_kernel_name")
    return buf.value.decode()


def norm_stats(x, per_sample, eps, mean, rstd, running_mean=None, running_var=None, num_batches=None,
               momentum=0.1):
    L = _l.load()
    N, C, D, H, W, S, xbs = _geom(x)
    nb = L.mis_norm_workspace_bytes(N, C, S, int(per_sample))
    ws = scratch(nb, "norm")
    _l.check(L.mis_norm_stats(_l.ptr(x), xbs, N, C, S, int(per_sample), eps, _l.ptr(mean), _l.ptr(rstd),
                              _l.ptr(running_mean), _l.ptr(running_var), _l.ptr(num_batches), momentum,
                              _l.ptr(ws), ws.numel(), _l.stream_ptr()), "mis_norm_stats")


def channel_sum(x, out, accumulate=False):
    L = _l.load()
    N, C, D, H, W, S, xbs = _geom(x)
    nb = L.mis_norm_workspace_bytes(N, C, S, 0)
    ws = scratch(nb, "norm")
    _l.check(L.mis_channel_sum(_l.ptr(x), xbs, N, C, S, _l.ptr(out), int(accumulate), _l.ptr(ws), ws.numel(),
                               _l.stream_ptr()), "mis_channel_sum")


def norm_stats_from_running(running_mean, running_var, eps, mean, rstd):
    L = _l.load()
    _l.check(L.mis_norm_stats_from_running(_l.ptr(running_mean), _l.ptr(running_var), eps, _l.ptr(mean),
                                           _l.ptr(rstd), running_mean.numel(), _l.stream_ptr()),
             "mis_norm_stats_from_running")


def norm_act_fwd(x, y, per_sample, mean, rstd, gamma, beta, slope, drop_p=0.0, drop_salt=0, state=None,
                 drop_mask=None, cg=1):
    L = _l.load()
    N, C, D, H, W, S, xbs = _geom(x)
    _, _, _, _, _, _, ybs = _geom(y)
    _l.check(L.mis_norm_act_fwd_g(_l.ptr(x), xbs, _l.ptr(y), ybs, N, C, S, int(per_sample), int(cg), _l.ptr(mean),
                                  _l.ptr(rstd), _l.ptr(gamma), _l.ptr(beta), slope, drop_p, drop_salt,
                                  _l.ptr(state), _l.ptr(drop_mask), _l.stream_ptr()), "mis_norm_act_fwd_g")


def norm_act_bwd(x, da, dx, per_sample, mean, rstd, gamma, beta, slope, drop_p=0.0, drop_salt=0, state=None,
                 drop_mask=None, dgamma=None, dbeta=None, accumulate_affine=False, cg=1, no_norm=False):
    L = _l.load()
    N, C, D, H, W, S, xbs = _geom(x)
    _, _, _, _, _, _, dabs = _geom(da)
    _, _, _, _, _, _, dxbs = _geom(dx)
    nb = L.mis_norm_workspace_bytes(N, C, S, int(per_sample))
    ws = scratch(nb, "norm")
    _l.check(L.mis_norm_act_bwd_g(_l.ptr(x), xbs, _l.ptr(da), dabs, _l.ptr(dx), dxbs, N, C, S, int(per_sample),
                                  int(cg), int(no_norm), _l.ptr(mean), _l.ptr(rstd), _l.ptr(gamma), _l.ptr(beta),
                                  slope, drop_p, drop_salt, _l.ptr(state), _l.ptr(drop_mask), _l.ptr(dgamma),
                                  _l.ptr(dbeta), int(accumulate_affine), _l.ptr(ws), ws.numel(), _l.stream_ptr()),
             "mis_norm_act_bwd_g")


def norm_res_act_fwd(x, res, y, per_sample, mean, rstd, gamma, beta, slope, post=False):
    L = _l.load()
    N, C, D, H, W, S, xbs = _geom(x)
    rbs, ybs = _geom(res)[6], _geom(y)[6]
    _l.check(L.mis_norm_res_act_fwd(_l.ptr(x), xbs, _l.ptr(res), rbs, _l.ptr(y), ybs, N, C, S, int(per_sample),
                                    _l.ptr(mean), _l.ptr(rstd), _l.ptr(gamma), _l.ptr(beta), slope, int(post),
                                    _l.stream_ptr()), "mis_norm_res_act_fwd")


def norm_res_act_bwd(x, res, dy, dx, dres, accumulate_dres, per_sample, mean, rstd, gamma, beta, slope, dgamma=None,
                     dbeta=None, accumulate_affine=False, post=False):
    L = _l.load()
    N, C, D, H, W, S, xbs = _geom(x)
    rbs, dybs, dxbs, drbs = _geom(res)[6], _geom(dy)[6], _geom(dx)[6], _geom(dres)[6]
    ws = scratch(L.mis_norm_workspace_bytes(N, C, S, int(per_sample)), "norm")
    _l.check(L.mis_norm_res_act_bwd(_l.ptr(x), xbs, _l.ptr(res), rbs, _l.ptr(dy), dybs, _l.ptr(dx), dxbs, _l.ptr(dres),
                                    drbs, int(accumulate_dres), N, C, S, int(per_sample), _l.ptr(mean), _l.ptr(rstd),
                                    _l.ptr(gamma), _l.ptr(beta), slope, _l.ptr(dgamma), _l.ptr(dbeta),
                                    int(accumulate_affine), int(post), _l.ptr(ws), ws.numel(), _l.stream_ptr()),
             "mis_norm_res_act_bwd")


def norm_act_fwd_pool(x, y, pooled, idx, per_sample, mean, rstd, gamma, beta, slope, drop_p=0.0, drop_salt=0, state=None,
                      drop_mask=None, cg=1):
    L = _l.load()
    N, C, D, H, W, S, xbs = _geom(x)
    _, _, _, _, _, _, ybs = _geom(y)
    _, _, _, _, _, _, pbs = _geom(pooled)
    _l.check(L.mis_norm_act_fwd_pool(_l.ptr(x), xbs, _l.ptr(y), ybs, _l.ptr(pooled), pbs, _l.ptr(idx), N, C, D, H, W,
                                     int(per_sample), int(cg), _l.ptr(mean), _l.ptr(rstd), _l.ptr(gamma), _l.ptr(beta),
                                     slope, drop_p, drop_salt, _l.ptr(state), _l.ptr(drop_mask), _l.stream_ptr()),
             "mis_norm_act_fwd_pool")


def norm_act_bwd_pool(x, da, dpool, idx, dx, per_sample, mean, rstd, gamma, beta, slope, drop_p=0.0, drop_salt=0,
                      state=None, drop_mask=None, dgamma=None, dbeta=None, accumulate_affine=False, cg=1):
    L = _l.load()
    N, C, D, H, W, S, xbs = _geom(x)
    dabs = _geom(da)[6] if da is not None else 0
    _, _, _, _, _, _, dpbs = _geom(dpool)
    _, _, _, _, _, _, dxbs = _geom(dx)
    ws = scratch(L.mis_norm_workspace_bytes(N, C, S, int(per_sample)), "norm")
    _l.check(L.mis_norm_act_bwd_pool(_l.ptr(x), xbs, _l.ptr(da), dabs, _l.ptr(dpool), dpbs, _l.ptr(idx), _l.ptr(dx), dxbs,
                                     N, C, D, H, W, int(per_sample), int(cg), _l.ptr(mean), _l.ptr(rstd), _l.ptr(gamma),
                                     _l.ptr(beta), slope, drop_p, drop_salt, _l.ptr(state), _l.ptr(drop_mask),
                                     _l.ptr(dgamma), _l.ptr(dbeta), int(accumulate_affine), _l.ptr(ws), ws.numel(),
                                     _l.stream_ptr()), "mis_norm_act_bwd_pool")


def norm_act_bwd_sums(x, da, per_sample, mean, rstd, gamma, beta, slope, sums, dgamma=None, dbeta=None,
                      accumulate_affine=False):
    L = _l.load()
    N, C, D, H, W, S, xbs = _geom(x)
    _, _, _, _, _, _, dabs = _geom(da)
    ws = scratch(L.mis_norm_workspace_bytes(N, C, S, int(per_sample)), "norm")
    _l.check(L.mis_norm_act_bwd_sums(_l.ptr(x), xbs, _l.ptr(da), dabs, N, C, S, int(per_sample), _l.ptr(mean),
                                     _l.ptr(rstd), _l.ptr(gamma), _l.ptr(beta), slope, _l.ptr(sums), _l.ptr(dgamma),
                                     _l.ptr(dbeta), int(accumulate_affine), _l.ptr(ws), ws.numel(), _l.stream_ptr()),
             "mis_norm_act_bwd_sums")


def conv_wgrad_cin1_norm_eligible(N, Cout, D, H, W):
    return bool(_l.load().mis_conv_wgrad_cin1_norm_eligible(N, Cout, D, H, W))


def conv_wgrad_cin1_norm(x, da, y, per_sample, mean, rstd, gamma, beta, sums, slope, dw, accumulate=False):
    L = _l.load()
    N, Cin, D, H, W, S, xbs = _geom(x)
    _, _, _, _, _, _, dabs = _geom(da)
    _, Cout, _, _, _, _, ybs = _geom(y)
    nb = L.mis_conv_wgrad_workspace_bytes(N, Cin, Cout, D, H, W, 1 if D == 1 else 3, 3, 3)
    if nb < 0:
        _l.check(nb, "mis_conv_wgrad_workspace_bytes")
    ws = scratch(nb, "wgrad")
    _l.check(L.mis_conv_wgrad_cin1_norm(_l.ptr(x), xbs, _l.ptr(da), dabs, _l.ptr(y), ybs, N, D, H, W, int(per_sample),
                                        _l.ptr(mean), _l.ptr(rstd), _l.ptr(gamma), _l.ptr(beta), _l.ptr(sums), slope,
                                        _l.ptr(dw), _l.ptr(ws), ws.numel(), int(accumulate), _l.stream_ptr()),
             "mis_conv_wgrad_cin1_norm")


def norm_head_eligible(C, K, per_sample, gamma, beta, cg=1, no_norm=False):
    return bool(_l.load().mis_norm_head_eligible(C, K)) and cg == 1 and not no_norm and not (
        per_sample and (gamma is not None or beta is not None))


def norm_head_fwd(x, logits, per_sample, mean, rstd, gamma, beta, slope, w, b, drop_p=0.0, drop_salt=0, state=None,
                  drop_mask=None):
    L = _l.load()
    N, C, D, H, W, S, xbs = _geom(x)
    _, K, _, _, _, _, lbs = _geom(logits)
    _l.check(L.mis_norm_head_fwd(_l.ptr(x), xbs, N, C, S, int(per_sample), _l.ptr(mean), _l.ptr(rstd), _l.ptr(gamma),
                                 _l.ptr(beta), slope, drop_p, drop_salt, _l.ptr(state), _l.ptr(drop_mask), _l.ptr(w),
                                 _l.ptr(b), K, _l.ptr(logits), lbs, _l.stream_ptr()), "mis_norm_head_fwd")


def norm_head_bwd(x, dlogits, dx, per_sample, mean, rstd, gamma, beta, slope, w, dw, db, drop_p=0.0, drop_salt=0,
                  state=None, drop_mask=None, dgamma=None, dbeta=None, accumulate_affine=False, accumulate_w=False):
    L = _l.load()
    N, C, D, H, W, S, xbs = _geom(x)
    _, K, _, _, _, _, dlbs = _geom(dlogits)
    _, _, _, _, _, _, dxbs = _geom(dx)
    nb = L.mis_norm_head_workspace_bytes(N, C, S, int(per_sample), K)
    ws = scratch(nb, "norm")
    _l.check(L.mis_norm_head_bwd(_l.ptr(x), xbs, _l.ptr(dlogits), dlbs, _l.ptr(dx), dxbs, N, C, S, int(per_sample),
                                 _l.ptr(mean), _l.ptr(rstd), _l.ptr(gamma), _l.ptr(beta), slope, drop_p, drop_salt,
                                 _l.ptr(state), _l.ptr(drop_mask), _l.ptr(w), K, _l.ptr(dgamma), _l.ptr(dbeta),
                                 int(accumulate_affine), _l.ptr(dw), _l.ptr(db), int(accumulate_w), _l.ptr(ws),
                                 ws.numel(), _l.stream_ptr()), "mis_norm_head_bwd")


def group_norm_stats(x, cg, eps, mean, rstd):
    L = _l.load()
    N, C, D, H, W, S, xbs = _geom(x)
    G = C // cg
    nb = L.mis_norm_workspace_bytes(N, G, cg * S, 1)
    ws = scratch(nb, "norm")
    _l.check(L.mis_norm_stats(_l.ptr(x), xbs, N, G, cg * S, 1, eps, _l.ptr(mean), _l.ptr(rstd), None, None, None,
                              0.0, _l.ptr(ws), ws.numel(), _l.stream_ptr()), "mis_norm_stats")


def maxpool2_fwd(x, y, idx):
    L = _l.load()
    N, C, D, H, W, S, xbs = _geom(x)
    _, _, _, _, _, _, ybs = _geom(y)
    _l.check(L.mis_maxpool2_fwd(_l.ptr(x), xbs, _l.ptr(y), ybs, _l.ptr(idx), N, C, D, H, W, _l.stream_ptr()),
             "mis_maxpool2_fwd")


def maxpool2_bwd(dy, idx, dx, accumulate=False):
    L = _l.load()
    N, C, D, H, W, S, dxbs = _geom(dx)
    _, _, _, _, _, _, dybs = _geom(dy)
    _l.check(L.mis_maxpool2_bwd(_l.ptr(dy), dybs, _l.ptr(idx), _l.ptr(dx), dxbs, N, C, D, H, W, int(accumulate),
                                _l.stream_ptr()), "mis_maxpool2_bwd")


def upsample2_fwd(x, y, align_corners):
    L = _l.load()
    N, C, D, H, W, S, xbs = _geom(x)
    _, _, _, _, _, _, ybs = _geom(y)
    _l.check(L.mis_upsample2_fwd(_l.ptr(x), xbs, _l.ptr(y), ybs, N, C, D, H, W, int(align_corners),
                                 _l.stream_ptr()), "mis_upsample2_fwd")


def upsample2_bwd(dy, dx, align_corners, accumulate=False):
    L = _l.load()
    N, C, D, H, W, S, dxbs = _geom(dx)
    _, _, _, _, _, _, dybs = _geom(dy)
    _l.check(L.mis_upsample2_bwd(_l.ptr(dy), dybs, _l.ptr(dx), dxbs, N, C, D, H, W, int(align_corners),
                                 int(accumulate), _l.stream_ptr()), "mis_upsample2_bwd")


def loss_tail(student, teacher, label, labeled_bs, out, dlogits=None, cons_weight=0.0, state=None,
              loss_scale=1.0):
    L = _l.load()
    B, C, D, H, W, S, sbs = _geom(student)
    tbs = 0
    if teacher is not None:
        Bt, Ct, _, _, _, St, tbs = _geom(teacher)
        assert Bt == B - labeled_bs and Ct == C and St == S
    if label is not None:
        _l.require_gpu(label)
        assert label.is_contiguous() and label.dtype in (torch.uint8, torch.int64)
        assert label.numel() >= labeled_bs * S
    lb = 1 if (label is None or label.dtype == torch.uint8) else 8
    dbs = 0
    if dlogits is not None:
        dbs = _geom(dlogits)[6]
    nb = L.mis_loss_tail_workspace_bytes(B, C, S)
    ws = scratch(nb, "tail")
    _l.check(L.mis_loss_tail(_l.ptr(student), sbs, _l.ptr(teacher), tbs, _l.ptr(label), lb, B, labeled_bs, C, S,
                             cons_weight, _l.ptr(state), loss_scale, _l.ptr(out), _l.ptr(dlogits), dbs,
                             _l.ptr(ws), ws.numel(), _l.stream_ptr()), "mis_loss_tail")


def softmax_mean_accumulate(logits, acc, repeats, scale, first):
    L = _l.load()
    Bl, C, D, H, W, S, lbs = _geom(logits)
    U, Ca, _, _, _, Sa, abs_ = _geom(acc)
    assert Bl == repeats * U and Ca == C and Sa == S
    _l.check(L.mis_softmax_mean_accumulate(_l.ptr(logits), lbs, _l.ptr(acc), abs_, U, repeats, C, S, scale,
                                           int(first), _l.stream_ptr()), "mis_softmax_mean_accumulate")


def uamt_tail(student, teacher, mean_probs, label, labeled_bs, out, max_iterations, dlogits=None, cons_weight=0.0,
              state=None, iter_num=0, loss_scale=1.0):
    L = _l.load()
    B, C, D, H, W, S, sbs = _geom(student)
    Bt, Ct, _, _, _, St, tbs = _geom(teacher)
    Bm, Cm, _, _, _, Sm, mbs = _geom(mean_probs)
    assert Bt == Bm == B - labeled_bs and Ct == Cm == C and St == Sm == S
    _l.require_gpu(label)
    assert label.is_contiguous() and label.dtype in (torch.uint8, torch.int64) and label.numel() >= labeled_bs * S
    lb = 1 if label.dtype == torch.uint8 else 8
    dbs = _geom(dlogits)[6] if dlogits is not None else 0
    nb = L.mis_uamt_tail_workspace_bytes(B, C, S)
    ws = scratch(nb, "tail")
    _l.check(L.mis_uamt_tail(_l.ptr(student), sbs, _l.ptr(teacher), tbs, _l.ptr(mean_probs), mbs, _l.ptr(label), lb,
                             B, labeled_bs, C, S, cons_weight, _l.ptr(state), int(iter_num), float(max_iterations),
                             loss_scale, _l.ptr(out), _l.ptr(dlogits), dbs, _l.ptr(ws), ws.numel(),
                             _l.stream_ptr()), "mis_uamt_tail")


ICT_BETA_SALT = 0x1C7BE7A0


def beta_sample(lam, alpha, state, salt=ICT_BETA_SALT):
    L = _l.load()
    _l.require_gpu(lam, state)
    assert lam.dtype == torch.float32 and lam.is_contiguous() and lam.numel() > 0
    if not float(alpha) > 0.0:
        raise ValueError(f"Beta(alpha, alpha) needs alpha > 0, got {alpha}")
    _l.check(L.mis_beta_sample(_l.ptr(lam), lam.numel(), float(alpha), int(salt) & 0xFFFFFFFF, _l.ptr(state),
                               _l.stream_ptr()), "mis_beta_sample")


def ict_mix(x, lam, labeled_bs, out):
    L = _l.load()
    _l.require_gpu(x, lam, out)
    M = lam.numel()
    assert x.dtype == out.dtype == lam.dtype == torch.float32
    assert x.is_contiguous() and out.is_contiguous() and lam.is_contiguous()
    assert x.shape[0] == labeled_bs + 2 * M and out.shape[0] == labeled_bs + M
    assert tuple(x.shape[1:]) == tuple(out.shape[1:])
    n = x[0].numel()
    _l.check(L.mis_ict_mix(_l.ptr(x), _l.ptr(out), _l.ptr(lam), labeled_bs, M, n, _l.stream_ptr()), "mis_ict_mix")


def ict_tail(student, teacher0, teacher1, lam, label, labeled_bs, out, dlogits=None, cons_weight=0.0, state=None,
             loss_scale=1.0):
    L = _l.load()
    B, C, D, H, W, S, sbs = _geom(student)
    M = B - labeled_bs
# ... 218 lines not shown
```

### cv-ssl-mis_amd/mis_hip/plan.py

```python
import itertools
import math
import os

import torch
import torch.nn as nn

from . import lib as _lib
from . import ops

_net_ids = itertools.count(1)

FUSE_CONV_STATS = os.environ.get("MIS_FUSE_STATS", "1") != "0"
FUSE_HEAD = os.environ.get("MIS_FUSE_HEAD", "1") != "0"
FUSE_FIRST = os.environ.get("MIS_FUSE_FIRST", "1") != "0"
FUSE_POOL = os.environ.get("MIS_FUSE_POOL", "1") != "0"
FUSE_POOL_FWD = os.environ.get("MIS_FUSE_POOL_FWD", "1") != "0"
WGRAD_STREAM = os.environ.get("MIS_WGRAD_STREAM", "1") != "0"
FUSE_DGRAD_NORM = os.environ.get("MIS_FUSE_DGRAD_NORM", "1") != "0"
PROGRESS_SYNC_MAIN = os.environ.get("MIS_PROGRESS_SYNC_MAIN", "0") == "1"
NORM_RES = os.environ.get("MIS_NORM_RES", "1") != "0"


class Act:

    def __init__(self, shape=None, parent=None, c0=0, C=None, tensor=None):
        self.parent, self.c0 = parent, c0
        self._written = False
        self.g = None
        if tensor is not None:
            self.t = tensor
        elif parent is not None:
            self.t = parent.t[:, c0:c0 + C]
        else:
            self.t = torch.empty(shape, dtype=torch.float32, device="cuda")

    @property
    def shape(self):
        return tuple(self.t.shape)

    def slice(self, c0, C):
        return Act(parent=self, c0=c0, C=C)

    def grad(self):
        if self.g is None:
            if self.parent is not None:
                self.g = self.parent.grad()[:, self.c0:self.c0 + self.t.shape[1]]
            else:
                self.g = torch.empty(self.shape, dtype=torch.float32, device="cuda")
        return self.g

    def _root(self):
        a = self
        while a.parent is not None:
            a = a.parent
        return a

    @property
    def written(self):
        return self._written or self._root()._written

    def mark_written(self):
        self._written = True

    def reset(self):
        self._written = False


class Ctx:

    def __init__(self, training, state=None, drop_masks=None, dropout=True, rng_stream=0):
        self.training = training
        self.rng_stream = rng_stream
        self.dropout = dropout
        self.state = state
        self.drop_masks = drop_masks


class ConvOp:
    def __init__(self, x, y, w, b, ksize, need_dx, bias_grad):
        self.x, self.y, self.w, self.b = x, y, w, b
        self.ksize, self.need_dx, self.bias_grad = tuple(ksize), need_dx, bias_grad
        self.cout, self.cin = w.data.shape[0], w.data.shape[1]
        N, _, D, H, W = y.shape
        self.wino_f = ops.conv_wino_select(N, self.cin, self.cout, D, H, W, self.ksize)
        self.wino_b = ops.conv_wino_select(N, self.cout, self.cin, D, H, W, self.ksize) if need_dx else -1
        self.wp = None
        self.wpd = None
        self.batched = False
        self.stat = None
        self.stat_norm = None
        self._dx_tmp = None
        self.fused_into = None
        self.norm_bwd = None
        self.dgrad_norm = None

    def fwd(self, ctx):
        if self.fused_into is not None:
            return
        if not self.batched:
            self.wp = ops.conv_pack(self.w.data, ops.conv_wino_pack_mode(self.wino_f, False) if self.wino_f >= 0 else 0,
                                    out=self.wp)
        stat = self.stat if (self.stat is not None and (self.stat_norm.per_sample or ctx.training)) else None
        ops.conv_fwd(self.x.t, self.wp, None if self.b is None else self.b.data, self.y.t, self.cin, self.cout,
                     self.ksize, stat=stat, wino=self.wino_f)

    def bwd(self, ctx):
        if self.fused_into is not None:
            return
        if self.norm_bwd is not None:
            n = self.norm_bwd
            ops.conv_wgrad_cin1_norm(self.x.t, n.y.grad(), self.y.t, n.per_sample, n.mean, n.rstd,
                                     None if n.gamma is None else n.gamma.data, None if n.beta is None else n.beta.data,
                                     n.sums, n.slope, self.w.grad)
            return
        dy = self.y.grad()
        side = getattr(ctx, "wgrad_stream", None) if self.need_dx else None
        if side is not None:
            _lib.wait_stream(side, torch.cuda.current_stream())
            with torch.cuda.stream(side):
                run_deferred(ctx)
                ops.conv_wgrad(self.x.t, dy, self.w.grad, self.ksize)
                if self.b is not None and self.bias_grad:
                    ops.channel_sum(dy, self.b.grad)
        else:
            ops.conv_wgrad(self.x.t, dy, self.w.grad, self.ksize)
            if self.b is not None and self.bias_grad:
                ops.channel_sum(dy, self.b.grad)
        if self.need_dx:
            if not self.batched:
                self.wpd = ops.conv_pack(self.w.data, ops.conv_wino_pack_mode(self.wino_b, True) if self.wino_b >= 0 else 1,
                                         out=self.wpd)
            if self.x.written:
                if self._dx_tmp is None:
                    self._dx_tmp = torch.empty(self.x.shape, dtype=torch.float32, device="cuda")
                ops.conv_fwd(dy, self.wpd, None, self._dx_tmp, self.cout, self.cin, self.ksize, wino=self.wino_b)
                ops.add(self.x.grad(), self._dx_tmp, self.x.grad())
            elif self.dgrad_norm is not None:
                n = self.dgrad_norm
                ops.conv_dgrad_norm(dy, self.wpd, self.x.grad(), self.cout, self.cin, n.x.t, n.mean, n.slope, n.ext_part,
                                    self.wino_b)
                n.ext_ready = True
            else:
                ops.conv_fwd(dy, self.wpd, None, self.x.grad(), self.cout, self.cin, self.ksize, wino=self.wino_b)
            self.x.mark_written()


class NormActOp:

    def __init__(self, x, y, per_sample, gamma, beta, running, slope, drop_p, site, eps=1e-5, momentum=0.1, cg=1,
                 no_norm=False):
        self.x, self.y, self.per_sample = x, y, per_sample
        self.cg, self.no_norm = cg, no_norm
        self.gamma, self.beta, self.running = gamma, beta, running
        self.slope, self.drop_p, self.site, self.eps, self.momentum = slope, drop_p, site, eps, momentum
        self.salt = 0
        self.fused = None
        self.drop3d = False
        N, C = x.shape[0], x.shape[1]
        G = N * C // cg if per_sample else C
        self.mean = torch.zeros(G, dtype=torch.float32, device="cuda")
        self.rstd = torch.ones(G, dtype=torch.float32, device="cuda")
        self._p = 0.0
        self._mask = None
        self.pool = None
        self.sums = None
        self.ext_part = None
        self.ext_tiles, self.ext_ready, self.ext_sums = 0, False, None
        self.res = None
        self.res_post = False
        self.head = None
        self.head_w = self.head_b = None

    def fwd(self, ctx):
        if self.no_norm:
            pass
        elif not self.per_sample and not ctx.training:
            ops.norm_stats_from_running(self.running[0], self.running[1], self.eps, self.mean, self.rstd)
        else:
            rm, rv, nbt = self.running if (self.running is not None and ctx.training) else (None, None, None)
            if self.fused is not None:
                N, C = self.x.shape[0], self.x.shape[1]
                S = self.x.shape[2] * self.x.shape[3] * self.x.shape[4]
                ops.norm_stats_finalize(self.fused[0], N, C // self.cg, S * self.cg, self.fused[1] * self.cg,
                                        self.per_sample, self.eps, self.mean, self.rstd, rm, rv, nbt, self.momentum)
            elif self.cg > 1:
                ops.group_norm_stats(self.x.t, self.cg, self.eps, self.mean, self.rstd)
            else:
                ops.norm_stats(self.x.t, self.per_sample, self.eps, self.mean, self.rstd, rm, rv, nbt, self.momentum)
        self._p = self.drop_p if (ctx.training and ctx.dropout) else 0.0
        self._mask = ctx.drop_masks.get(self.site) if (ctx.drop_masks and self._p > 0) else None
        self.salt = ((ctx.rng_stream & 0x7FFF) << 16) | self.site | (0x80000000 if self.drop3d else 0)
        self._state = ctx.state
        if self._p > 0 and self._mask is None and ctx.state is None:
            raise RuntimeError("dropout is active but no device step state was supplied (Ctx.state)")
        if self.res is not None:
            ops.norm_res_act_fwd(self.x.t, self.res.t, self.y.t, self.per_sample, self.mean, self.rstd,
                                 None if self.gamma is None else self.gamma.data,
                                 None if self.beta is None else self.beta.data, self.slope, post=self.res_post)
            return
        if self.pool is not None and self.pool.fwd_fused:
            pl = self.pool
            ops.norm_act_fwd_pool(self.x.t, self.y.t, pl.y.t, pl.idx, self.per_sample, self.mean, self.rstd,
                                  None if self.gamma is None else self.gamma.data,
                                  None if self.beta is None else self.beta.data, self.slope, self._p, self.salt,
                                  self._state, self._mask, cg=self.cg)
            return
        if self.head is not None:
            h = self.head
            ops.norm_head_fwd(self.x.t, h.y.t, self.per_sample, self.mean, self.rstd,
                              None if self.gamma is None else self.gamma.data,
                              None if self.beta is None else self.beta.data, self.slope,
                              h.w.data.view(h.cout, h.cin), None if h.b is None else h.b.data, self._p, self.salt,
                              self._state, self._mask)
            return
        ops.norm_act_fwd(self.x.t, self.y.t, self.per_sample, self.mean, self.rstd,
                         None if self.gamma is None else self.gamma.data,
                         None if self.beta is None else self.beta.data, self.slope, self._p, self.salt,
                         self._state, self._mask, cg=self.cg)

    def bwd(self, ctx):
        assert not self.x.written
        if self.res is not None:
            r = self.res
            ops.norm_res_act_bwd(self.x.t, r.t, self.y.grad(), self.x.grad(), r.grad(), r.written, self.per_sample,
                                 self.mean, self.rstd, None if self.gamma is None else self.gamma.data,
                                 None if self.beta is None else self.beta.data, self.slope,
                                 None if self.gamma is None else self.gamma.grad,
                                 None if self.beta is None else self.beta.grad, post=self.res_post)
            r.mark_written()
            self.x.mark_written()
            return
        if self.ext_ready:
            self.ext_ready = False
            to_sums = self.sums is not None
            ops.norm_act_bwd_tiles(self.x.t, self.y.grad(), None if to_sums else self.x.grad(), self.mean, self.rstd,
                                   self.slope, self.ext_part, self.ext_tiles, self.sums if to_sums else self.ext_sums)
            if not to_sums:
                self.x.mark_written()
            return
        if self.sums is not None:
            ops.norm_act_bwd_sums(self.x.t, self.y.grad(), self.per_sample, self.mean, self.rstd,
                                  None if self.gamma is None else self.gamma.data,
                                  None if self.beta is None else self.beta.data, self.slope, self.sums,
                                  None if self.gamma is None else self.gamma.grad,
                                  None if self.beta is None else self.beta.grad)
            return
        if self.pool is not None:
            pl = self.pool
            ops.norm_act_bwd_pool(self.x.t, self.y.grad() if self.y.written else None, pl.y.grad(), pl.idx, self.x.grad(),
                                  self.per_sample, self.mean, self.rstd,
                                  None if self.gamma is None else self.gamma.data,
                                  None if self.beta is None else self.beta.data, self.slope, self._p, self.salt,
                                  self._state, self._mask, None if self.gamma is None else self.gamma.grad,
                                  None if self.beta is None else self.beta.grad, cg=self.cg)
            self.x.mark_written()
            return
        if self.head is not None:
            h = self.head
            ops.norm_head_bwd(self.x.t, h.y.grad(), self.x.grad(), self.per_sample, self.mean, self.rstd,
                              None if self.gamma is None else self.gamma.data,
                              None if self.beta is None else self.beta.data, self.slope,
                              h.w.data.view(h.cout, h.cin), h.w.grad.view(h.cout, h.cin),
                              h.b.grad if (h.b is not None and h.bias_grad) else None, self._p, self.salt, self._state,
                              self._mask, None if self.gamma is None else self.gamma.grad,
                              None if self.beta is None else self.beta.grad)
            self.x.mark_written()
            return
        ops.norm_act_bwd(self.x.t, self.y.grad(), self.x.grad(), self.per_sample, self.mean, self.rstd,
                         None if self.gamma is None else self.gamma.data,
                         None if self.beta is None else self.beta.data, self.slope, self._p, self.salt,
                         self._state, self._mask,
                         None if self.gamma is None else self.gamma.grad,
                         None if self.beta is None else self.beta.grad, cg=self.cg, no_norm=self.no_norm)
        self.x.mark_written()


class MaxPoolOp:
    def __init__(self, x, y):
        self.x, self.y = x, y
        self.idx = torch.empty(y.t.numel(), dtype=torch.uint8, device="cuda")
        self.fused_into = None
        self.fwd_fused = False

    def fwd(self, ctx):
        if self.fwd_fused:
            return
        ops.maxpool2_fwd(self.x.t, self.y.t, self.idx)

    def bwd(self, ctx):
        if self.fused_into is not None:
            return
        ops.maxpool2_bwd(self.y.grad(), self.idx, self.x.grad(), accumulate=self.x.written)
        self.x.mark_written()


class UpsampleOp:
    def __init__(self, x, y, align_corners):
        self.x, self.y, self.align = x, y, align_corners

    def fwd(self, ctx):
        ops.upsample2_fwd(self.x.t, self.y.t, self.align)

    def bwd(self, ctx):
        ops.upsample2_bwd(self.y.grad(), self.x.grad(), self.align, accumulate=self.x.written)
        self.x.mark_written()


class DownConvOp:

    def __init__(self, x, y, w, b, bias_grad=False, need_dx=True, in_shape=None):
        self.x, self.y, self.w, self.b, self.bias_grad, self.need_dx = x, y, w, b, bias_grad, need_dx
        N, Cin, D, H, W = in_shape if in_shape is not None else x.shape
        self.in_shape = (N, Cin, D, H, W)
        self.cin8, self.cout = 8 * Cin, w.data.shape[0]
        coarse = (D // 2, H // 2, W // 2)
        self.direct = ops.conv_k2s2_eligible(Cin, self.cout, coarse, False)
        self.direct_dx = ops.conv_k2s2_eligible(self.cout, Cin, coarse, True)
        self.direct_wg = ops.conv_k2s2_wgrad_eligible(Cin, self.cout, coarse)
        self._xs = None if self.direct else self._new_xs()
        self._xs_valid = False
        self.dxs = None
        self.wp = self.wpd = None
        self._wT = None

    def _new_xs(self):
        N, Cin, D, H, W = self.in_shape
        return torch.empty((N, self.cin8, D // 2, H // 2, W // 2), dtype=torch.float32, device="cuda")

    def fwd(self, ctx):
        if self.direct:
            self._xs_valid = False
            ops.conv_k2s2_down(self.x.t, self.w.data, None if self.b is None else self.b.data, self.y.t)
            return
        ops.space_to_depth2(self.x.t, self._xs, self.in_shape, True)
        self._xs_valid = True
        if ops.conv1x1_gemm_eligible(self._xs, self.y.t, self.cin8, self.cout):
            from . import tops
            if self._wT is None:
                self._wT = torch.empty((self.cin8, self.cout), dtype=torch.float32, device="cuda")
            tops.transpose(self.w.data.view(self.cout, self.cin8), self._wT)
            ops.conv1x1_gemm(self._xs, self._wT, None if self.b is None else self.b.data, self.y.t)
            return
        self.wp = ops.conv_pack_raw(self.w.data, self.cout, self.cin8, 1, 0, out=self.wp)
        ops.conv_fwd(self._xs, self.wp, None if self.b is None else self.b.data, self.y.t, self.cin8, self.cout, (1, 1, 1))

    def bwd(self, ctx):
        dy = self.y.grad()
# ... 45 lines not shown
    def _new_y8(self):
        N, _, d, h, wd = self.x.shape
        return torch.empty((N, self.cout8, d, h, wd), dtype=torch.float32, device="cuda")

    def fwd(self, ctx):
        if self.direct and ops.conv_k2s2_up_output_ok(self.y.t):
            ops.conv_k2s2_up(self.x.t, self.w.data, None if self.b is None else self.b.data, self.y.t)
            return
        if self.y8 is None:
            self.y8 = self._new_y8()
        if ops.conv1x1_gemm_eligible(self.x.t, self.y8, self.cin, self.cout8):
            ops.conv1x1_gemm(self.x.t, self.w.data.view(self.cin, self.cout8), None, self.y8)
        else:
            self.wp = ops.conv_pack_raw(self.w.data, self.cout8, self.cin, 1, 2, out=self.wp)
            ops.conv_fwd(self.x.t, self.wp, None, self.y8, self.cin, self.cout8, (1, 1, 1))
        ops.space_to_depth2(self.y8, self.y.t, self.y.shape, False, bias=None if self.b is None else self.b.data)

    def bwd(self, ctx):
        from . import tops
        if self.bias_grad and self.b is not None:
            ops.channel_sum(self.y.grad(), self.b.grad)
        dyf = self.y.grad()
        if self.direct_wg and self.direct_dx and ops.conv_k2s2_wgrad_operands_ok(self.x.t, dyf):
            ops.conv_k2s2_wgrad(self.x.t, dyf, self.w.grad.view(-1))
        else:
            if self.dy8 is None:
                self.dy8 = self._new_y8()
                self.dw8 = torch.empty((self.cout8, self.cin), dtype=torch.float32, device="cuda")
            ops.space_to_depth2(dyf, self.dy8, self.y.shape, True)
            if ops.conv1x1_wgrad_eligible(self.x.t, self.dy8):
                ops.conv1x1_wgrad(self.x.t, self.dy8, self.w.grad.view(self.cin, self.cout8))
            else:
                ops.conv_wgrad(self.x.t, self.dy8, self.dw8, (1, 1, 1))
                tops.transpose(self.dw8, self.w.grad.view(self.cin, self.cout8))
        assert not self.x.written
        if self.direct_dx:
            ops.conv_k2s2_down(self.y.grad(), self.w.data, None, self.x.grad())
            self.x.mark_written()
            return
        if ops.conv1x1_gemm_eligible(self.dy8, self.x.grad(), self.cout8, self.cin):
            if self._wT is None:
                self._wT = torch.empty((self.cout8, self.cin), dtype=torch.float32, device="cuda")
            tops.transpose(self.w.data.view(self.cin, self.cout8), self._wT)
            ops.conv1x1_gemm(self.dy8, self._wT, None, self.x.grad())
        else:
            self.wpd = ops.conv_pack_raw(self.w.data, self.cout8, self.cin, 1, 3, out=self.wpd)
            ops.conv_fwd(self.dy8, self.wpd, None, self.x.grad(), self.cout8, self.cin, (1, 1, 1))
        self.x.mark_written()


class UpConv2dOp:

    def __init__(self, x, y, w, b, bias_grad=True):
        self.x, self.y, self.w, self.b, self.bias_grad = x, y, w, b, bias_grad
        N, Cin, d, h, wd = x.shape
        assert d == 1
        self.cin, self.cout4 = Cin, 4 * w.data.shape[1]
        self.y4 = torch.empty((N, self.cout4, 1, h, wd), dtype=torch.float32, device="cuda")
        self.dy4 = self.dw4 = None
        self.wp = self.wpd = None

    def fwd(self, ctx):
        self.wp = ops.conv_pack_raw(self.w.data, self.cout4, self.cin, 1, 2, out=self.wp)
        ops.conv_fwd(self.x.t, self.wp, None, self.y4, self.cin, self.cout4, (1, 1, 1))
        ops.space_to_depth2d(self.y4, self.y.t, self.y.shape, False, bias=None if self.b is None else self.b.data)

    def bwd(self, ctx):
        from . import tops
        dyf = self.y.grad()
        if self.bias_grad and self.b is not None:
            ops.channel_sum(dyf, self.b.grad)
        if self.dy4 is None:
            self.dy4 = torch.empty_like(self.y4)
            self.dw4 = torch.empty((self.cout4, self.cin), dtype=torch.float32, device="cuda")
        ops.space_to_depth2d(dyf, self.dy4, self.y.shape, True)
        ops.conv_wgrad(self.x.t, self.dy4, self.dw4, (1, 1, 1))
        tops.transpose(self.dw4, self.w.grad.view(self.cin, self.cout4))
        assert not self.x.written
        self.wpd = ops.conv_pack_raw(self.w.data, self.cout4, self.cin, 1, 3, out=self.wpd)
        ops.conv_fwd(self.dy4, self.wpd, None, self.x.grad(), self.cout4, self.cin, (1, 1, 1))
        self.x.mark_written()


class AddOp:

    def __init__(self, a, b, out):
        self.a, self.b, self.out = a, b, out

    def fwd(self, ctx):
        ops.add(self.a.t, self.b.t, self.out.t)

    def bwd(self, ctx):
        dout = self.out.grad()
        for t in (self.a, self.b):
            if t.written:
                ops.add(t.grad(), dout, t.grad())
            else:
                ops.add(dout, None, t.grad())
            t.mark_written()


class Plan:

    def __init__(self, net, in_shape):
        self.net = net
        self.in_shape = tuple(in_shape)
        self._tbatch = None
        self.ops = []
        self.acts = []
        self.inp = Act(tensor=torch.empty(0, device="cuda"))
        self.acts.append(self.inp)
        self._wgrad_stream = None
        self._salt = itertools.count(0)
        self.out = None
        self._packs = None
        self._head_checked = False
        self.generation = 0
        self._progress = None

    def new(self, C, spatial, N=None):
        a = Act((self.in_shape[0] if N is None else N, C) + tuple(spatial))
        self.acts.append(a)
        return a

    def view(self, parent, c0, C):
        a = parent.slice(c0, C)
        self.acts.append(a)
        return a

    def conv(self, x, y, w, b, ksize, need_dx=True, bias_grad=True):
        self.ops.append(ConvOp(x, y, w, b, ksize, need_dx, bias_grad))
        return y

    def norm_act(self, x, y, per_sample, gamma=None, beta=None, running=None, slope=0.0, drop_p=0.0, drop3d=False,
                 cg=1, no_norm=False):
        op = NormActOp(x, y, per_sample, gamma, beta, running, slope, drop_p, next(self._salt), cg=cg, no_norm=no_norm)
        op.drop3d = drop3d
        prev = self.ops[-1] if self.ops else None
        if FUSE_CONV_STATS and not no_norm and type(prev) is ConvOp and prev.y is x:
            N, C, D, H, W = x.shape
            T = ops.conv_stat_tiles(N, prev.cin, prev.cout, D, H, W, prev.ksize, wino=prev.wino_f)
            if T > 0:
                part = torch.empty((C * N * T, 2), dtype=torch.float32, device="cuda")
                prev.stat = (part, T, C * T) if per_sample else (part, N * T, T)
                prev.stat_norm = op
                op.fused = (part, T)
        if (FUSE_FIRST and type(prev) is ConvOp and prev.y is x and not prev.need_dx and prev.cin == 1
                and prev.ksize in ((3, 3, 3), (1, 3, 3)) and drop_p == 0.0 and cg == 1 and not no_norm
                and not (per_sample and (gamma is not None or beta is not None)) and x.parent is None
                and ops.conv_wgrad_cin1_norm_eligible(x.shape[0], prev.cout, *x.shape[2:])):
            op.sums = torch.empty((x.shape[0] * x.shape[1] if per_sample else x.shape[1], 2), dtype=torch.float32,
                                  device="cuda")
            prev.norm_bwd = op
        self.ops.append(op)
        return y

    @staticmethod
    def can_norm_res_act(x):
        return NORM_RES and (x.shape[2] * x.shape[3] * x.shape[4]) % 4 == 0

    def norm_res_act(self, x, res, y, per_sample, gamma=None, beta=None, running=None, slope=0.0):
        assert self.can_norm_res_act(x) and tuple(res.shape) == tuple(x.shape)
        assert not (per_sample and (gamma is not None or beta is not None))
        self.norm_act(x, y, per_sample, gamma, beta, running, slope)
        self.ops[-1].res = res
        return y

    def down_conv(self, x, y, w, b, bias_grad=False):
        self.ops.append(DownConvOp(x, y, w, b, bias_grad))
        return y

    def up_conv(self, x, y, w, b, bias_grad=False):
        self.ops.append(UpConvOp(x, y, w, b, bias_grad))
        return y

    def up_conv2d(self, x, y, w, b, bias_grad=True):
        self.ops.append(UpConv2dOp(x, y, w, b, bias_grad))
        return y

    def add(self, a, b, out=None, fuse=False):
        prev = self.ops[-1] if self.ops else None
        if (fuse and NORM_RES and type(prev) is NormActOp and prev.y is a and a.parent is None and prev.res is None
                and prev.pool is None and prev.sums is None and not prev.no_norm and prev.drop_p == 0.0 and prev.cg == 1
                and not (prev.per_sample and (prev.gamma is not None or prev.beta is not None))
                and self.can_norm_res_act(a)):
            prev.res, prev.res_post = b, True
            if out is not None and out in self.acts:
                self.acts.remove(out)
            return a
        if out is None:
            out = self.new(a.shape[1], a.shape[2:], N=a.shape[0])
        self.ops.append(AddOp(a, b, out))
        return out

    def maxpool(self, x, y):
        op = MaxPoolOp(x, y)
        if FUSE_POOL:
            prod = next((o for o in reversed(self.ops) if type(o) is NormActOp and o.y is x), None)
            N, C, D, H, W = x.shape
            if (prod is not None and prod.pool is None and prod.head is None and prod.sums is None and not prod.no_norm
                    and W % 4 == 0 and H % 2 == 0 and (D == 1 or D % 2 == 0) and D * H * W < 2 ** 31):
                prod.pool, op.fused_into = op, prod
                op.fwd_fused = FUSE_POOL_FWD and D == 1 and W % 8 == 0 and prod is self.ops[-1] and y.parent is None
        self.ops.append(op)
        return y

    def upsample(self, x, y, align_corners):
        self.ops.append(UpsampleOp(x, y, align_corners))
        return y

    def _pack(self, mode):
        if self._packs is None:
            convs = [op for op in self.ops if type(op) is ConvOp]
            L = ops._l.load()
            fj, bj = [], []
            for op in convs:
                taps = op.w.data[0, 0].numel()
                mf = ops.conv_wino_pack_mode(op.wino_f, False) if op.wino_f >= 0 else 0
                mb = ops.conv_wino_pack_mode(op.wino_b, True) if op.wino_b >= 0 else 1
                op.wp = torch.empty(L.mis_conv_packed_floats(op.cout, op.cin, taps, mf), dtype=torch.float32,
                                    device="cuda")
                fj.append((op.w.data, op.wp, mf))
                if op.need_dx:
                    op.wpd = torch.empty(L.mis_conv_packed_floats(op.cout, op.cin, taps, mb), dtype=torch.float32,
                                         device="cuda")
                    bj.append((op.w.data, op.wpd, mb))
                op.batched = True
            self._packs = (ops.PackBatch(fj) if fj else None, ops.PackBatch(bj) if bj else None)
        if self._packs[mode] is not None:
            self._packs[mode].run()

    def _transpose_linear_weights(self):
        if self._tbatch is None:
            from . import tops
            from .swin_plan import LinearOp
            jobs = []
            for op in self.ops:
                if isinstance(op, LinearOp) and op.need_dx and op.w2.is_contiguous():
                    op.wT = torch.empty((op.w2.shape[1], op.w2.shape[0]), dtype=torch.float32, device="cuda")
                    op.wT_batched = True
                    jobs.append((op.w2, op.wT))
            self._tbatch = tops.TransposeBatch(jobs) if jobs else False
        if self._tbatch:
            self._tbatch.run()

    def _split_linear_weights(self, transposed):
        if self._tbatch is False:
            return False
        from .swin_plan import split_linear_weights
        return split_linear_weights(self, self.ops, transposed)

    def _fuse_dgrad_norm(self):
        if not FUSE_DGRAD_NORM:
            return
        L = ops._l.load()
        for conv in self.ops:
            if type(conv) is not ConvOp or not conv.need_dx or conv.wino_b not in (0, 1) or conv.ksize != (3, 3, 3):
                continue
            if conv.fused_into is not None or conv.x.parent is not None:
                continue
            norm = next((o for o in self.ops if type(o) is NormActOp and o.y is conv.x), None)
            if norm is None or not norm.per_sample or norm.gamma is not None or norm.beta is not None or norm.cg != 1:
                continue
            if norm.no_norm or norm.drop_p > 0 or norm.pool is not None or norm.head is not None or norm.res is not None:
                continue
            N, C = norm.x.shape[0], norm.x.shape[1]
            if N * C > 384:
                continue
            readers = 0
            for op in self.ops:
                if op is norm:
                    continue
                for v in vars(op).values():
                    if isinstance(v, Act) and v._root() is norm.y:
                        readers += 1
            if readers != 1:
                continue
            _, _, D, H, W = norm.x.shape
            tiles = int(L.mis_conv3d_wino_stat_tiles(D, H, W, conv.wino_b))
            norm.ext_part = torch.zeros(N * C * tiles, 2, dtype=torch.float32, device="cuda")
            norm.ext_tiles = tiles
            norm.ext_sums = torch.zeros(N * C, 2, dtype=torch.float32, device="cuda")
            conv.dgrad_norm = norm

    def _fuse_head(self):
        self._head_checked = True
        if not FUSE_HEAD or len(self.ops) < 2:
            return
        norm, conv = self.ops[-2], self.ops[-1]
        if type(norm) is not NormActOp or type(conv) is not ConvOp or conv.ksize != (1, 1, 1) or conv.x is not norm.y:
            return
        if norm.y.parent is not None or conv.y is not self.out or not conv.need_dx or norm.res is not None:
            return
        for op in self.ops[:-1]:
            for v in vars(op).values():
                if isinstance(v, Act) and v is not norm.y and v._root() is norm.y:
                    return
                if v is norm.y and op is not norm:
                    return
        if not ops.norm_head_eligible(conv.cin, conv.cout, norm.per_sample, norm.gamma, norm.beta, norm.cg, norm.no_norm):
            return
        norm.head, norm.head_w, norm.head_b = conv, conv.w, conv.b
        conv.fused_into = norm

    def forward(self, x5, ctx):
        assert tuple(x5.shape) == self.in_shape, (tuple(x5.shape), self.in_shape)
# ... 319 lines not shown
```

### include/mis_hip.h

```cpp
#ifndef MIS_HIP_H
#define MIS_HIP_H

#ifdef __cplusplus
extern "C" {
#endif

#define MIS_OK 0
#define MIS_ERR_ARG (-1)
#define MIS_ERR_UNSUPPORTED (-2)
#define MIS_ERR_LAUNCH (-3)
#define MIS_ERR_WORKSPACE (-4)

typedef void* mis_stream_t;

typedef struct MisStepState MisStepState;

int mis_abi_version(void);

int mis_conv_cin_pad(int cin);
int mis_conv_cout_pad(int cout);
long long mis_conv_packed_floats(int Cout, int Cin, int taps, int mode);
int mis_conv_pack_weights(const float* w, float* wp, int Cout, int Cin, int taps, int mode, mis_stream_t stream);
int mis_conv_pack_job_bytes(void);
long long mis_conv_pack_job(void* job_out, const float* w, float* wp, int Cout, int Cin, int taps, int mode,
                            long long start);
int mis_conv_pack_batch(const void* jobs_device, int n, long long total_floats, mis_stream_t stream);
int mis_conv_fwd(const float* x, long long x_bs, const float* wp, const float* bias, float* y, long long y_bs,
                 int N, int Cin, int Cout, int D, int H, int W, int kd, int kh, int kw, mis_stream_t stream);
long long mis_conv_fwd_stat_tiles(int N, int Cin, int Cout, int D, int H, int W, int kd, int kh, int kw);
int mis_conv_fwd_stats(const float* x, long long x_bs, const float* wp, const float* bias, float* y, long long y_bs,
                       int N, int Cin, int Cout, int D, int H, int W, int kd, int kh, int kw, float* stat,
                       long long stat_sc, long long stat_sn, mis_stream_t stream);
int mis_norm_stats_finalize(const float* part, int N, int C, long long S, int tiles, int per_sample, float eps,
                            float* mean, float* rstd, float* running_mean, float* running_var,
                            long long* num_batches_tracked, float momentum, mis_stream_t stream);
int mis_conv_fwd_kernel_name(int N, int Cin, int Cout, int D, int H, int W, int kd, int kh, int kw, char* name,
                             int name_len);
int mis_conv3d_wino_select(int N, int Cin, int Cout, int D, int H, int W);
long long mis_conv3d_wino_stat_tiles(int D, int H, int W, int variant);
int mis_conv3d_wino_kernel_name(int variant, char* name, int name_len);
int mis_conv3d_wino_fwd(const float* x, long long x_bs, const float* wt, const float* bias, float* y, long long y_bs,
                        int N, int Cin, int Cout, int D, int H, int W, float* stat, long long stat_sc,
                        long long stat_sn, int variant, mis_stream_t stream);
int mis_conv3d_wino_fwd_splits(int N, int Cin, int Cout, int D, int H, int W, int variant);
long long mis_conv3d_wino_fwd_workspace_bytes(int N, int Cin, int Cout, int D, int H, int W, int variant);
int mis_conv3d_wino_fwd_ws(const float* x, long long x_bs, const float* wt, const float* bias, float* y, long long y_bs,
                           int N, int Cin, int Cout, int D, int H, int W, float* stat, long long stat_sc, long long stat_sn,
                           int variant, float* workspace, long long workspace_bytes, mis_stream_t stream);
int mis_conv3d_wino_dgrad_norm(const float* dy, long long dy_bs, const float* wt, float* da, long long da_bs, int N,
                               int Cin, int Cout, int D, int H, int W, const float* xn, long long xn_bs,
                               const float* mean, float slope, float* part, long long part_sc, long long part_sn,
                               int variant, mis_stream_t stream);
int mis_conv2d_wino_select(int N, int Cin, int Cout, int H, int W);
long long mis_conv2d_wino_stat_tiles(int H, int W, int variant);
int mis_conv2d_wino_kernel_name(int variant, char* name, int name_len);
int mis_conv2d_wino_fwd(const float* x, long long x_bs, const float* wt, const float* bias, float* y, long long y_bs,
                        int N, int Cin, int Cout, int H, int W, float* stat, long long stat_sc, long long stat_sn,
                        int variant, mis_stream_t stream);
int mis_conv2d_wino_wgrad_select(int N, int Cin, int Cout, int H, int W);
int mis_conv2d_wino_wgrad_kernel_name(int variant, char* name, int name_len);
long long mis_conv2d_wino_wgrad_workspace_bytes(int N, int Cin, int Cout, int H, int W, int variant);
int mis_conv2d_wino_wgrad(const float* x, long long x_bs, const float* dy, long long dy_bs, float* dw, float* workspace,
                          long long workspace_bytes, int N, int Cin, int Cout, int H, int W, int accumulate, int variant,
                          mis_stream_t stream);
int mis_conv3d_wino_wgrad_select(int N, int Cin, int Cout, int D, int H, int W);
int mis_conv3d_wino_wgrad_kernel_name(int variant, char* name, int name_len);
long long mis_conv3d_wino_wgrad_workspace_bytes(int N, int Cin, int Cout, int D, int H, int W, int variant);
int mis_conv3d_wino_wgrad(const float* x, long long x_bs, const float* dy, long long dy_bs, float* dw, float* workspace,
                          long long workspace_bytes, int N, int Cin, int Cout, int D, int H, int W, int accumulate,
                          int variant, mis_stream_t stream);
long long mis_conv_wgrad_workspace_bytes(int N, int Cin, int Cout, int D, int H, int W, int kd, int kh, int kw);
int mis_conv_wgrad_kernel_name(int N, int Cin, int Cout, int D, int H, int W, int kd, int kh, int kw, char* name,
                               int name_len);
int mis_conv_wgrad(const float* x, long long x_bs, const float* dy, long long dy_bs, float* dw, float* workspace,
                   long long workspace_bytes, int N, int Cin, int Cout, int D, int H, int W, int kd, int kh,
                   int kw, int accumulate, mis_stream_t stream);
int mis_channel_sum(const float* x, long long x_bs, int N, int C, long long S, float* out, int accumulate,
                    void* workspace, long long workspace_bytes, mis_stream_t stream);

long long mis_norm_workspace_bytes(int N, int C, long long S, int per_sample);
int mis_norm_stats(const float* x, long long x_bs, int N, int C, long long S, int per_sample, float eps,
                   float* mean, float* rstd, float* running_mean, float* running_var,
                   long long* num_batches_tracked, float momentum, void* workspace, long long workspace_bytes,
                   mis_stream_t stream);
int mis_norm_stats_from_running(const float* running_mean, const float* running_var, float eps, float* mean,
                                float* rstd, int C, mis_stream_t stream);
int mis_norm_act_fwd(const float* x, long long x_bs, float* y, long long y_bs, int N, int C, long long S,
                     int per_sample, const float* mean, const float* rstd, const float* gamma, const float* beta,
                     float slope, float drop_p, unsigned drop_salt, const MisStepState* state,
                     const float* drop_mask, mis_stream_t stream);
int mis_norm_act_bwd(const float* x, long long x_bs, const float* da, long long da_bs, float* dx, long long dx_bs,
                     int N, int C, long long S, int per_sample, const float* mean, const float* rstd,
                     const float* gamma, const float* beta, float slope, float drop_p, unsigned drop_salt,
                     const MisStepState* state, const float* drop_mask, float* dgamma, float* dbeta,
                     int accumulate_affine, void* workspace, long long workspace_bytes, mis_stream_t stream);
int mis_norm_act_fwd_g(const float* x, long long x_bs, float* y, long long y_bs, int N, int C, long long S,
                       int per_sample, int cg, const float* mean, const float* rstd, const float* gamma,
                       const float* beta, float slope, float drop_p, unsigned drop_salt, const MisStepState* state,
                       const float* drop_mask, mis_stream_t stream);
int mis_norm_act_bwd_g(const float* x, long long x_bs, const float* da, long long da_bs, float* dx, long long dx_bs,
                       int N, int C, long long S, int per_sample, int cg, int no_norm, const float* mean,
                       const float* rstd, const float* gamma, const float* beta, float slope, float drop_p,
                       unsigned drop_salt, const MisStepState* state, const float* drop_mask, float* dgamma,
                       float* dbeta, int accumulate_affine, void* workspace, long long workspace_bytes,
                       mis_stream_t stream);

int mis_norm_act_bwd_sums(const float* x, long long x_bs, const float* da, long long da_bs, int N, int C, long long S,
                          int per_sample, const float* mean, const float* rstd, const float* gamma, const float* beta,
                          float slope, float* sums, float* dgamma, float* dbeta, int accumulate_affine, void* workspace,
                          long long workspace_bytes, mis_stream_t stream);
int mis_norm_act_bwd_tiles(const float* x, long long x_bs, const float* da, long long da_bs, float* dx, long long dx_bs,
                           int N, int C, long long S, const float* mean, const float* rstd, float slope,
                           const float* part, int tiles, float* sums, mis_stream_t stream);
int mis_norm_res_act_fwd(const float* x, long long x_bs, const float* res, long long res_bs, float* y, long long y_bs,
                         int N, int C, long long S, int per_sample, const float* mean, const float* rstd,
                         const float* gamma, const float* beta, float slope, int add_after_act, mis_stream_t stream);
int mis_norm_res_act_bwd(const float* x, long long x_bs, const float* res, long long res_bs, const float* dy,
                         long long dy_bs, float* dx, long long dx_bs, float* dres, long long dres_bs, int accumulate_dres,
                         int N, int C, long long S, int per_sample, const float* mean, const float* rstd,
                         const float* gamma, const float* beta, float slope, float* dgamma, float* dbeta,
                         int accumulate_affine, int add_after_act, void* workspace, long long workspace_bytes,
                         mis_stream_t stream);
int mis_conv_wgrad_cin1_norm_eligible(int N, int Cout, int D, int H, int W);
int mis_conv_wgrad_cin1_norm(const float* x, long long x_bs, const float* da, long long da_bs, const float* y,
                             long long y_bs, int N, int D, int H, int W, int per_sample, const float* mean,
                             const float* rstd, const float* gamma, const float* beta, const float* sums, float slope,
                             float* dw, float* workspace, long long workspace_bytes, int accumulate,
                             mis_stream_t stream);

int mis_norm_head_eligible(int C, int K);
long long mis_norm_head_workspace_bytes(int N, int C, long long S, int per_sample, int K);
int mis_norm_head_fwd(const float* x, long long x_bs, int N, int C, long long S, int per_sample, const float* mean,
                      const float* rstd, const float* gamma, const float* beta, float slope, float drop_p,
                      unsigned drop_salt, const MisStepState* state, const float* drop_mask, const float* w,
                      const float* b, int K, float* logits, long long l_bs, mis_stream_t stream);
int mis_norm_head_bwd(const float* x, long long x_bs, const float* dlogits, long long dl_bs, float* dx, long long dx_bs,
                      int N, int C, long long S, int per_sample, const float* mean, const float* rstd,
                      const float* gamma, const float* beta, float slope, float drop_p, unsigned drop_salt,
                      const MisStepState* state, const float* drop_mask, const float* w, int K, float* dgamma,
                      float* dbeta, int accumulate_affine, float* dw, float* db, int accumulate_w, void* workspace,
                      long long workspace_bytes, mis_stream_t stream);

int mis_norm_act_fwd_pool(const float* x, long long x_bs, float* y, long long y_bs, float* pooled, long long p_bs,
                          unsigned char* idx, int N, int C, int D, int H, int W, int per_sample, int cg,
                          const float* mean, const float* rstd, const float* gamma, const float* beta, float slope,
                          float drop_p, unsigned drop_salt, const MisStepState* state, const float* drop_mask,
                          mis_stream_t stream);
int mis_norm_act_bwd_pool(const float* x, long long x_bs, const float* da, long long da_bs, const float* dpool,
                          long long dp_bs, const unsigned char* idx, float* dx, long long dx_bs, int N, int C, int D,
                          int H, int W, int per_sample, int cg, const float* mean, const float* rstd,
                          const float* gamma, const float* beta, float slope, float drop_p, unsigned drop_salt,
                          const MisStepState* state, const float* drop_mask, float* dgamma, float* dbeta,
                          int accumulate_affine, void* workspace, long long workspace_bytes, mis_stream_t stream);

int mis_maxpool2_fwd(const float* x, long long x_bs, float* y, long long y_bs, unsigned char* idx, int N, int C,
                     int D, int H, int W, mis_stream_t stream);
int mis_maxpool2_bwd(const float* dy, long long dy_bs, const unsigned char* idx, float* dx, long long dx_bs,
                     int N, int C, int D, int H, int W, int accumulate, mis_stream_t stream);
int mis_upsample2_fwd(const float* x, long long x_bs, float* y, long long y_bs, int N, int C, int D, int H,
                      int W, int align_corners, mis_stream_t stream);
int mis_upsample2_bwd(const float* dy, long long dy_bs, float* dx, long long dx_bs, int N, int C, int D, int H,
                      int W, int align_corners, int accumulate, mis_stream_t stream);

long long mis_loss_tail_workspace_bytes(int B, int C, long long S);
int mis_loss_tail(const float* student, long long s_bs, const float* teacher, long long t_bs, const void* label,
                  int label_bytes, int B, int L, int C, long long S, float cons_weight,
                  const MisStepState* state, float loss_scale, float* out, float* dlogits, long long d_bs,
                  void* workspace, long long workspace_bytes, mis_stream_t stream);

long long mis_cross_teaching_tail_workspace_bytes(int B, int C, long long S);
int mis_cross_pseudo_tail(const float* own, long long s_bs, const float* other, long long o_bs, const void* label,
                          int label_bytes, int B, int L, int C, long long S, float cons_weight,
                          const MisStepState* state, int pseudo_ce, float* out, float* dlogits, long long d_bs,
                          void* workspace, long long workspace_bytes, mis_stream_t stream);
int mis_cross_pseudo_mt_tail(const float* own, long long s_bs, const float* other, long long o_bs,
                             const float* teacher, long long t_bs, const void* label, int label_bytes, int B, int L,
                             int C, long long S, float cons_weight, float mt_weight, const MisStepState* state,
                             int pseudo_ce, float* out, float* dlogits, long long d_bs, void* workspace,
                             long long workspace_bytes, mis_stream_t stream);
int mis_cross_teaching_tail(const float* own, long long s_bs, const float* other, long long o_bs, const void* label,
                            int label_bytes, int B, int L, int C, long long S, float cons_weight,
                            const MisStepState* state, float* out, float* dlogits, long long d_bs, void* workspace,
                            long long workspace_bytes, mis_stream_t stream);

int mis_softmax_mean_accumulate(const float* logits, long long l_bs, float* acc, long long a_bs, int U, int R, int C,
                                long long S, float scale, int first, mis_stream_t stream);
long long mis_uamt_tail_workspace_bytes(int B, int C, long long S);
int mis_uamt_tail(const float* student, long long s_bs, const float* teacher, long long t_bs, const float* mean_probs,
                  long long mp_bs, const void* label, int label_bytes, int B, int L, int C, long long S,
                  float cons_weight, const MisStepState* state, long long iter_num, double max_iterations,
                  float loss_scale, float* out, float* dlogits, long long d_bs, void* workspace,
                  long long workspace_bytes, mis_stream_t stream);

int mis_beta_sample(float* lam, int M, double alpha, unsigned salt, const MisStepState* state, mis_stream_t stream);
int mis_ict_mix(const float* x, float* out, const float* lam, int L, int M, long long n, mis_stream_t stream);
long long mis_ict_tail_workspace_bytes(int B, int C, long long S);
int mis_ict_tail(const float* student, long long s_bs, const float* teacher0, long long t0_bs, const float* teacher1,
                 long long t1_bs, const float* lam, const void* label, int label_bytes, int L, int M, int C,
                 long long S, float cons_weight, const MisStepState* state, float loss_scale, float* out,
                 float* dlogits, long long d_bs, void* workspace, long long workspace_bytes, mis_stream_t stream);

int mis_rot90(const float* in, long long in_bs, float* out, long long out_bs, int N, int C, int H, int W, const int* sched,
              long long n_sched, const MisStepState* state, int k_override, mis_stream_t stream);
long long mis_dct_tail_workspace_bytes(int L, int U, int C, int H, int W);
int mis_dct_tail(const float* logits_a, long long a_bs, const float* logits_r, long long r_bs, const void* label,
                 int label_bytes, int L, int U, int C, int H, int W, const int* sched, long long n_sched,
                 const MisStepState* state, int k_override, float cons_weight, float loss_scale, float* out, float* dA,
                 long long dA_bs, float* dR, long long dR_bs, void* workspace, long long workspace_bytes,
                 mis_stream_t stream);
int mis_grad_combine(float* dst, const float* src, long long n, int accumulate, mis_stream_t stream);

long long mis_triple_view_tail_workspace_bytes(int B, int C, long long S);
int mis_triple_view_tail(const float* z1, long long z1_bs, const float* z2, long long z2_bs, const float* z3,
                         long long z3_bs, const void* label, int label_bytes, int B, int L, int C, long long S,
                         float cons_weight, const MisStepState* state, float* out1, float* out2, float* out3, float* d1,
                         long long d1_bs, float* d2, long long d2_bs, float* d3, long long d3_bs, void* workspace,
                         long long workspace_bytes, mis_stream_t stream);

long long mis_dice_workspace_bytes(int B, int C, long long S);
int mis_dice_loss_fwd(const float* probs, long long p_bs, const void* label, int label_bytes, int B, int C,
                      long long S, const float* weight, float* out, void* workspace, long long workspace_bytes,
                      mis_stream_t stream);
int mis_dice_loss_bwd(const float* probs, long long p_bs, const void* label, int label_bytes, int B, int C,
                      long long S, const void* workspace, const float* grad_out, float* dprobs, long long d_bs,
                      mis_stream_t stream);
int mis_softmax_mse(const float* input_logits, long long a_bs, const float* target_logits, long long b_bs,
                    const float* grad_out, long long g_bs, float* out, long long o_bs, int B, int C, long long S,
                    int backward, mis_stream_t stream);
int mis_ema_update(float* ema_param, const float* param, long long n, float alpha, mis_stream_t stream);

int mis_sgd_ema_step(float* param, const float* grad, float* momentum_buf, float* ema_param, long long n,
                     float lr, float momentum, float weight_decay, float ema_alpha, float grad_scale,
                     const MisStepState* state, mis_stream_t stream);
int mis_teacher_noise(const float* x, float* y, long long n, float sigma, float clamp_abs, unsigned salt,
                      const MisStepState* state, mis_stream_t stream);
int mis_step_init(MisStepState* state, unsigned long long seed, long long iter_num, double base_lr,
                  double max_iterations, double ema_decay, double consistency, double rampup, long long ramp_div,
                  long long cons_start_iter, int lr_post_increment, mis_stream_t stream);
int mis_step_advance(MisStepState* state, double base_lr, double max_iterations, double ema_decay,
                     double consistency, double rampup, long long ramp_div, long long cons_start_iter,
                     int lr_post_increment, mis_stream_t stream);
int mis_argmax_channels(const float* x, long long x_bs, unsigned char* out, int B, int C, long long S,
                        mis_stream_t stream);

int mis_conv_k2s2_eligible(int Cin, int Cout, int Do, int Ho, int Wo, int up);
int mis_conv_k2s2_down(const float* x, long long x_bs, const float* w, const float* bias, float* y, long long y_bs, int N,
                       int Cin, int Cout, int Do, int Ho, int Wo, int accumulate, mis_stream_t stream);
int mis_conv_k2s2_up(const float* x, long long x_bs, const float* w, const float* bias, float* y, long long y_bs, int N,
                     int Cin, int Cout, int Do, int Ho, int Wo, int accumulate, mis_stream_t stream);
int mis_conv_k2s2_wgrad_eligible(int CF, int CC, int Do, int Ho, int Wo);
long long mis_conv_k2s2_wgrad_workspace_bytes(int CF, int CC);
int mis_conv_k2s2_wgrad(const float* coarse, long long c_bs, const float* fine, long long f_bs, float* dw, int N, int CF,
                        int CC, int Do, int Ho, int Wo, int accumulate, float* workspace, long long workspace_bytes,
                        mis_stream_t stream);
int mis_space_to_depth2(const float* src, long long src_bs, float* dst, long long dst_bs, const float* bias, int N,
                        int C, int D, int H, int W, int to_depth, int accumulate, mis_stream_t stream);
int mis_space_to_depth2d(const float* src, long long src_bs, float* dst, long long dst_bs, const float* bias, int N, int C,
                         int H, int W, int to_depth, int accumulate, mis_stream_t stream);
int mis_add(const float* a, long long a_bs, const float* b, long long b_bs, float* out, long long o_bs, int N, int C,
            long long S, mis_stream_t stream);

long long mis_gemm_workspace_bytes(int M, int N, int K, int trans);

long long mis_gemm_dw_workspace_bytes(int M, int N, int K);
int mis_gemm_dw(const float* dy, long long lddy, const float* x, long long ldx, float* dW, long long lddw, float* db, int M,
                int N, int K, int accumulate, float* workspace, long long workspace_bytes, hipStream_t stream);
int mis_gemm_dw_parts(const float* dy, long long lddy, const float* x, long long ldx, float* dW, long long lddw, float* db,
                      int M, int N, int K, int accumulate, float* workspace, long long workspace_bytes, int* slices,
                      hipStream_t stream);
int mis_gemm_nt_kernel_name(int M, int N, int K, int epilogue, char* name, int name_len);
int mis_gemm_set_split_precision(int mask);
int mis_gemm_tn_kernel_name(const float* A, long long lda, const float* B, long long ldb, const float* C, long long ldc,
                            int M, int N, int K, char* name, int name_len);
int mis_gemm_expand_ln_head(const float* x, long long lda, const float* W, long long ldb, float* out, int B, int H, int Wd,
                            int K, int P, int c, const float* gamma, const float* beta, const float* head_w, int NC,
                            float eps, float* mean, float* rstd, float* logits, long long logits_bs, mis_stream_t stream);
int mis_gemm_expand_ln_head_split(const float* x, long long lda, const void* B3, float* out, int B, int H, int W, int K, int P,
                                  int c, const float* gamma, const float* beta, const float* head_w, int NC, float eps,
                                  float* mean, float* rstd, float* logits, long long logits_bs, hipStream_t stream);
long long mis_gemm_split_bytes(int N, int K);
int mis_gemm_split_b(const float* B, long long ldb, int N, int K, void* B3, mis_stream_t stream);
// ... 179 lines not shown
```

Before: 452.8.

## Recompute first-layer Cin=1 conv instead of storing its pre-norm output

In the forward pass, the first 3x3x3 conv (Cin=1, Cout=16) now runs a stats-only pass that skips writing its 16-channel output. A fused conv+norm+LeakyReLU kernel then recomputes the conv and writes the activation directly. In the backward pass, the weight-gradient kernel recomputes the conv output with MFMA instead of reading the stored tensor. This trades cheap recomputation from a single-channel input for less memory traffic on a 16-channel full-resolution tensor, at the cost of running the conv three times. The pre-activation is still written in the fused forward when backward needs it.

```diff
diff --git a/cv-ssl-mis_amd/csrc/common.h b/cv-ssl-mis_amd/csrc/common.h
--- a/cv-ssl-mis_amd/csrc/common.h
+++ b/cv-ssl-mis_amd/csrc/common.h
@@ -257,3 +257,13 @@
     mis_gelu_parts(x, cdf, u);
     return fmaf(x * 0.3989422804014327f, u, cdf);
 }
+
+__device__ __forceinline__ void mis_norm_scale_shift(float gamma, float beta, float mean, float rstd, float& sc, float& sh) {
+    sc = gamma * rstd;
+    sh = beta - mean * sc;
+}
+__device__ __forceinline__ float mis_norm_lin(float x, float sc, float sh) { return x * sc + sh; }
+__device__ __forceinline__ float mis_lrelu(float v, float slope) { return v > 0.f ? v : v * slope; }
+__device__ __forceinline__ float mis_norm_act_apply(float x, float sc, float sh, float slope) {
+    return mis_lrelu(mis_norm_lin(x, sc, sh), slope);
+}
diff --git a/cv-ssl-mis_amd/csrc/conv_fwd.hip b/cv-ssl-mis_amd/csrc/conv_fwd.hip
--- a/cv-ssl-mis_amd/csrc/conv_fwd.hip
+++ b/cv-ssl-mis_amd/csrc/conv_fwd.hip
@@ -394,6 +394,7 @@
     __syncthreads();
     const int wz = KD == 3 ? wave : 0, wy = KD == 3 ? 0 : wave * C::WROWS;
     const float* __restrict__ sb = sx + (wz * C::HY + wy) * C::HX + lj;
+    const bool store = a.y != nullptr;
     float* __restrict__ yo = a.y + (long long)n * a.y_bs + ((long long)(z0 + wz) * a.H + y0 + wy) * a.W + x0 + lj;
     float s1[4] = {0.f, 0.f, 0.f, 0.f}, s2[4] = {0.f, 0.f, 0.f, 0.f};
 #pragma unroll 2
@@ -405,7 +406,7 @@
 #pragma unroll
         for (int r = 0; r < 4; ++r) {
             const float v = acc[r] + bv[r];
-            yo[(long long)(lk * 4 + r) * S + (long long)row * a.W] = v;
+            if (store) yo[(long long)(lk * 4 + r) * S + (long long)row * a.W] = v;
             s1[r] += v; s2[r] += v * v;
         }
     }
@@ -424,6 +425,100 @@
             const long long tile = ((long long)tz * a.tiles_y + ty) * a.tiles_x + tx;
             a.stat[(long long)tid * a.stat_sc + (long long)n * a.stat_sn + tile] =
                 make_float2((p0.x + p1.x) + (p2.x + p3.x), (p0.y + p1.y) + (p2.y + p3.y));
+        }
+    }
+}
+
+struct Cin1W {
+    static constexpr int TZ = 4, TY = 8, TX = 32;
+    static constexpr int HZ = TZ + 2, HY = TY + 2, HX = TX + 2, HALO = HZ * HY * HX;
+    static constexpr int TAPS = 27, NG = 7;
+    static constexpr int RS = TX + 4;
+};
+
+struct Cin1NormArgs {
+    const float* x; long long x_bs;
+    const float* wp; const float* bias;
+    float* r; long long r_bs;
+    float* y; long long y_bs;
+    const float* mean; const float* rstd; const float* gamma; const float* beta;
+    float slope;
+    int per_sample;
+    int D, H, W, Cout_pad;
+    int tiles_z, tiles_y, tiles_x;
+    unsigned n_blocks, n_blocks_padded;
+};
+
+__global__ __launch_bounds__(256) void conv_cin1_norm_act_kernel(const Cin1NormArgs a) {
+    using C = Cin1W;
+    __shared__ float sx[C::HALO];
+    __shared__ __attribute__((aligned(16))) float stage[4][2][16 * C::RS];
+    const unsigned L = mis_xcd_remap(blockIdx.x, a.n_blocks_padded);
+    if (L >= a.n_blocks) return;
+    unsigned t = L;
+    const int tx = t % a.tiles_x; t /= a.tiles_x;
+    const int ty = t % a.tiles_y; t /= a.tiles_y;
+    const int tz = t % a.tiles_z; t /= a.tiles_z;
+    const int n = t;
+    const int z0 = tz * C::TZ, y0 = ty * C::TY, x0 = tx * C::TX;
+    const int tid = threadIdx.x, lane = tid & 63, wave = tid >> 6, lk = lane >> 4, lj = lane & 15;
+    const long long S = (long long)a.D * a.H * a.W;
+    const float* __restrict__ xn = a.x + (long long)n * a.x_bs;
+    for (int e = tid; e < C::HALO; e += 256) {
+        const int hz = e / (C::HY * C::HX), r2 = e - hz * (C::HY * C::HX), hy = r2 / C::HX, hx = r2 - hy * C::HX;
+        const int gz = z0 + hz - 1, gy = y0 + hy - 1, gx = x0 + hx - 1;
+        const bool ok = (unsigned)gz < (unsigned)a.D && (unsigned)gy < (unsigned)a.H && (unsigned)gx < (unsigned)a.W;
+        sx[e] = ok ? xn[((long long)gz * a.H + gy) * a.W + gx] : 0.f;
+    }
+    float wa[C::NG];
+    int toff[C::NG];
+#pragma unroll
+    for (int g = 0; g < C::NG; ++g) {
+        const int tap = 4 * g + lk;
+        wa[g] = tap < C::TAPS ? a.wp[tap * a.Cout_pad + lj] : 0.f;
+        const int tc = tap < C::TAPS ? tap : C::TAPS - 1;
+        toff[g] = ((tc / 9) * C::HY + (tc / 3) % 3) * C::HX + tc % 3;
+    }
+    float bv[4];
+#pragma unroll
+    for (int r = 0; r < 4; ++r) bv[r] = a.bias ? a.bias[lk * 4 + r] : 0.f;
+    const int sc0 = lane >> 3, sx4 = (lane & 7) * 4;
+    float sc[2], sh[2];
+#pragma unroll
+    for (int i = 0; i < 2; ++i) {
+        const int c = sc0 + 8 * i, grp = a.per_sample ? n * 16 + c : c;
+        mis_norm_scale_shift(a.gamma ? a.gamma[c] : 1.f, a.beta ? a.beta[c] : 0.f, a.mean[grp], a.rstd[grp], sc[i], sh[i]);
+    }
+    __syncthreads();
+    const float* __restrict__ sb = sx + (wave * C::HY) * C::HX + lj;
+    const long long vbase = ((long long)(z0 + wave) * a.H + y0) * a.W + x0 + sx4;
+    float* __restrict__ yo = a.y + (long long)n * a.y_bs + vbase;
+    float* __restrict__ ro = a.r ? a.r + (long long)n * a.r_bs + vbase : nullptr;
+#pragma unroll 2
+    for (int row = 0; row < C::TY; ++row) {
+        float* __restrict__ st = stage[wave][row & 1];
+#pragma unroll
+        for (int half = 0; half < 2; ++half) {
+            f32x4 acc = {0.f, 0.f, 0.f, 0.f};
+#pragma unroll
+            for (int g = 0; g < C::NG; ++g)
+                acc = __builtin_amdgcn_mfma_f32_16x16x4f32(wa[g], sb[row * C::HX + half * 16 + toff[g]], acc, 0, 0, 0);
+#pragma unroll
+            for (int r = 0; r < 4; ++r) {
+                const float v = acc[r] + bv[r];
+                st[(lk * 4 + r) * C::RS + half * 16 + lj] = v;
+            }
+        }
+        __syncthreads();
+#pragma unroll
+        for (int i = 0; i < 2; ++i) {
+            const int c = sc0 + 8 * i;
+            const float4 q = *reinterpret_cast<const float4*>(st + c * C::RS + sx4);
+            const long long o = (long long)c * S + (long long)row * a.W;
+            if (ro) *reinterpret_cast<float4*>(ro + o) = q;
+            *reinterpret_cast<float4*>(yo + o) =
+                make_float4(mis_norm_act_apply(q.x, sc[i], sh[i], a.slope), mis_norm_act_apply(q.y, sc[i], sh[i], a.slope),
+                            mis_norm_act_apply(q.z, sc[i], sh[i], a.slope), mis_norm_act_apply(q.w, sc[i], sh[i], a.slope));
         }
     }
 }
@@ -609,3 +704,39 @@
     return dispatch_fwd(make_fwd_args(nullptr, 0, nullptr, nullptr, nullptr, 0, N, Cin, Cout, D, H, W), kd, kh, kw,
                         nullptr, name, name_len);
 }
+
+extern "C" int mis_conv_fwd_cin1_stats(const float* x, long long x_bs, const float* wp, const float* bias, int N, int D,
+                                       int H, int W, float* stat, long long stat_sc, long long stat_sn,
+                                       hipStream_t stream) {
+    if (!x || !wp || !stat || N <= 0 || D <= 0 || H <= 0 || W <= 0) return MIS_ERR_ARG;
+    const long long S = (long long)D * H * W;
+    if (x_bs < S) return MIS_ERR_ARG;
+    if (((uintptr_t)stat & 7) != 0) return MIS_ERR_UNSUPPORTED;
+    ConvFwdArgs a = make_fwd_args(x, x_bs, wp, bias, nullptr, 16 * S, N, 1, 16, D, H, W);
+    if (cin1_kd(a, 3, 3, 3) != 3) return MIS_ERR_UNSUPPORTED;
+    a.stat = reinterpret_cast<float2*>(stat); a.stat_sc = stat_sc; a.stat_sn = stat_sn;
+    return launch_cin1<3>(a, stream);
+}
+
+extern "C" int mis_conv_cin1_norm_act_fwd(const float* x, long long x_bs, const float* wp, const float* bias, float* r,
+                                          long long r_bs, float* y, long long y_bs, int N, int D, int H, int W,
+                                          int per_sample, const float* mean, const float* rstd, const float* gamma,
+                                          const float* beta, float slope, hipStream_t stream) {
+    if (!x || !wp || !y || !mean || !rstd || N <= 0 || D <= 0 || H <= 0 || W <= 0) return MIS_ERR_ARG;
+    const long long S = (long long)D * H * W;
+    if (x_bs < S || y_bs < 16 * S || (r && r_bs < 16 * S)) return MIS_ERR_ARG;
+    using C = Cin1W;
+    if (D % C::TZ || H % C::TY || W % C::TX) return MIS_ERR_UNSUPPORTED;
+    if (((uintptr_t)y & 15) || y_bs % 4 || ((uintptr_t)r & 15) || (r && r_bs % 4)) return MIS_ERR_UNSUPPORTED;
+    Cin1NormArgs a{};
+    a.x = x; a.x_bs = x_bs; a.wp = wp; a.bias = bias; a.r = r; a.r_bs = r_bs; a.y = y; a.y_bs = y_bs;
+    a.mean = mean; a.rstd = rstd; a.gamma = gamma; a.beta = beta; a.slope = slope; a.per_sample = per_sample ? 1 : 0;
+    a.D = D; a.H = H; a.W = W; a.Cout_pad = mis_conv_cout_pad(16);
+    a.tiles_z = D / C::TZ; a.tiles_y = H / C::TY; a.tiles_x = W / C::TX;
+    const long long nb = (long long)N * a.tiles_z * a.tiles_y * a.tiles_x;
+    if (nb > 0x7fffffffLL) return MIS_ERR_ARG;
+    a.n_blocks = (unsigned)nb;
+    a.n_blocks_padded = (unsigned)(mis_cdiv(nb, MIS_NUM_XCD) * MIS_NUM_XCD);
+    hipLaunchKernelGGL(conv_cin1_norm_act_kernel, dim3(a.n_blocks_padded), dim3(256), 0, stream, a);
+    return mis_launch_status();
+}
diff --git a/cv-ssl-mis_amd/csrc/conv_wgrad_cin1.hip b/cv-ssl-mis_amd/csrc/conv_wgrad_cin1.hip
--- a/cv-ssl-mis_amd/csrc/conv_wgrad_cin1.hip
+++ b/cv-ssl-mis_amd/csrc/conv_wgrad_cin1.hip
@@ -25,11 +25,17 @@
     int tz, ty, tx, n_tiles;
 };
 
-template <int KD, bool NORM>
-__global__ __launch_bounds__(256) void wgrad_cin1_kernel(const Cin1Args a, const Cin1Norm nb) {
+struct Cin1Rc {
+    const float* wp;
+    const float* bias;
+};
+
+template <int KD, bool NORM, bool RC>
+__device__ __forceinline__ void wgrad_cin1_body(const Cin1Args& a, const Cin1Norm& nb, const Cin1Rc& rc, float* sx) {
     using C = WC1<KD>;
     constexpr int TZ = C::TZ, TY = C::TY, TX = C::TX, HY = C::HY, HX = C::HX, HALO = C::HALO, NG = C::NG;
-    __shared__ float sx[HALO];
+    static_assert(!RC || (KD == 3 && NORM), "the recomputing form serves the 3-D first layer behind a normalisation");
+    constexpr int FG = 7;
     const int tid = threadIdx.x, lane = tid & 63, wave = tid >> 6;
     const int lk = lane >> 4, lj = lane & 15;
     const long long S = (long long)a.D * a.H * a.W;
@@ -42,6 +48,19 @@
     f32x4 acc[NG];
 #pragma unroll
     for (int g = 0; g < NG; ++g) acc[g] = f32x4{0.f, 0.f, 0.f, 0.f};
+    [[maybe_unused]] float wa[FG];
+    [[maybe_unused]] int ftoff[FG];
+    [[maybe_unused]] float bj = 0.f;
+    if constexpr (RC) {
+#pragma unroll
+        for (int g = 0; g < FG; ++g) {
+            const int tap = 4 * g + lk;
+            wa[g] = tap < C::TAPS ? rc.wp[tap * 16 + lj] : 0.f;
+            const int tc = tap < C::TAPS ? tap : C::TAPS - 1;
+            ftoff[g] = ((tc / 9) * HY + (tc / 3) % 3) * HX + tc % 3;
+        }
+        bj = rc.bias ? rc.bias[lj] : 0.f;
+    }
     const int wz = KD == 3 ? wave : 0, wy = KD == 3 ? 0 : wave * 8;
     for (int t = blockIdx.x; t < a.n_tiles; t += gridDim.x) {
         int r = t;
@@ -61,7 +80,7 @@
         __syncthreads();
         const long long voff = (long long)lj * S + ((long long)(z0 + wz) * a.H + y0 + wy) * a.W + x0 + 4 * lk;
         const float* __restrict__ dyp = a.dy + (long long)n * a.dy_bs + voff;
-        const float* __restrict__ yp = NORM ? nb.y + (long long)n * nb.y_bs + voff : nullptr;
+        const float* __restrict__ yp = NORM && !RC ? nb.y + (long long)n * nb.y_bs + voff : nullptr;
         float cm = 0.f, crs = 1.f, cga = 1.f, cbe = 0.f, s1 = 0.f, s2 = 0.f;
         if constexpr (NORM) {
             const int grp = nb.per_sample ? n * 16 + lj : lj;
@@ -71,12 +90,23 @@
             s1 = sm.x; s2 = sm.y;
         }
         const float* __restrict__ sb = sx + (wz * HY + wy) * HX + 4 * lk;
+        const float* __restrict__ sf = sx + (wz * HY + wy) * HX + lj;
 #pragma unroll 4
         for (int it = 0; it < 16; ++it) {
             const int row = it >> 1, half = it & 1;
             f32x4 d4 = *reinterpret_cast<const f32x4*>(dyp + (long long)row * a.W + half * 16);
             if constexpr (NORM) {
-                const f32x4 y4 = *reinterpret_cast<const f32x4*>(yp + (long long)row * a.W + half * 16);
+                f32x4 y4;
+                if constexpr (RC) {
+                    y4 = f32x4{0.f, 0.f, 0.f, 0.f};
+#pragma unroll
+                    for (int g = 0; g < FG; ++g)
+                        y4 = __builtin_amdgcn_mfma_f32_16x16x4f32(sf[row * HX + half * 16 + ftoff[g]], wa[g], y4, 0, 0, 0);
+#pragma unroll
+                    for (int s = 0; s < 4; ++s) y4[s] = y4[s] + bj;
+                } else {
+                    y4 = *reinterpret_cast<const f32x4*>(yp + (long long)row * a.W + half * 16);
+                }
 #pragma unroll
                 for (int s = 0; s < 4; ++s) {
                     const float xh = (y4[s] - cm) * crs;
@@ -98,6 +128,18 @@
     for (int g = 0; g < NG; ++g)
 #pragma unroll
         for (int r = 0; r < 4; ++r) out[g * 256 + (lk * 4 + r) * 16 + lj] = acc[g][r];
+}
+
+template <int KD, bool NORM>
+__global__ __launch_bounds__(256) void wgrad_cin1_kernel(const Cin1Args a, const Cin1Norm nb) {
+    __shared__ float sx[WC1<KD>::HALO];
+    wgrad_cin1_body<KD, NORM, false>(a, nb, Cin1Rc{}, sx);
+}
+
+template <int KD>
+__global__ __launch_bounds__(256) void wgrad_cin1_rc_kernel(const Cin1Args a, const Cin1Norm nb, const Cin1Rc rc) {
+    __shared__ float sx[WC1<KD>::HALO];
+    wgrad_cin1_body<KD, true, true>(a, nb, rc, sx);
 }
 
 __global__ __launch_bounds__(256) void wgrad_cin1_reduce_kernel(const float* __restrict__ ws, float* __restrict__ dw,
@@ -127,7 +169,7 @@
 
 template <int KD>
 int launch_cin1_kd(const float* x, long long x_bs, const float* dy, long long dy_bs, const Cin1Norm* nb, float* dw,
-                   float* ws, int N, int D, int H, int W, int accumulate, hipStream_t stream) {
+                   float* ws, int N, int D, int H, int W, int accumulate, hipStream_t stream, const Cin1Rc* rc = nullptr) {
     using C = WC1<KD>;
     Cin1Args a{};
     a.x = x; a.x_bs = x_bs; a.dy = dy; a.dy_bs = dy_bs; a.ws = ws;
@@ -137,6 +179,14 @@
     if (n_tiles > 0x7fffffffLL) return MIS_ERR_ARG;
     a.n_tiles = (int)n_tiles;
     const int grid = grid_for(n_tiles);
+    if constexpr (KD == 3) {
+        if (nb && rc) {
+            hipLaunchKernelGGL(wgrad_cin1_rc_kernel<KD>, dim3(grid), dim3(256), 0, stream, a, *nb, *rc);
+            hipLaunchKernelGGL(wgrad_cin1_reduce_kernel, dim3(16 * C::TAPS), dim3(256), 0, stream, ws, dw, grid * 4, C::TAPS,
+                               C::NG, accumulate);
+            return mis_launch_status();
+        }
+    }
     if (nb) hipLaunchKernelGGL((wgrad_cin1_kernel<KD, true>), dim3(grid), dim3(256), 0, stream, a, *nb);
     else hipLaunchKernelGGL((wgrad_cin1_kernel<KD, false>), dim3(grid), dim3(256), 0, stream, a, Cin1Norm{});
     hipLaunchKernelGGL(wgrad_cin1_reduce_kernel, dim3(16 * C::TAPS), dim3(256), 0, stream, ws, dw, grid * 4, C::TAPS, C::NG,
@@ -158,11 +208,12 @@
 }
 
 static int launch_cin1(const float* x, long long x_bs, const float* dy, long long dy_bs, const Cin1Norm* nb, float* dw,
-                       float* ws, long long ws_bytes, int N, int D, int H, int W, int accumulate, hipStream_t stream) {
+                       float* ws, long long ws_bytes, int N, int D, int H, int W, int accumulate, hipStream_t stream,
+                       const Cin1Rc* rc = nullptr) {
     if (((uintptr_t)dy & 15) || dy_bs % 4) return MIS_ERR_UNSUPPORTED;
     if (ws_bytes < mis_wgrad_cin1_workspace_bytes(N, D, H, W)) return MIS_ERR_WORKSPACE;
     return D == 1 ? launch_cin1_kd<1>(x, x_bs, dy, dy_bs, nb, dw, ws, N, D, H, W, accumulate, stream)
-                  : launch_cin1_kd<3>(x, x_bs, dy, dy_bs, nb, dw, ws, N, D, H, W, accumulate, stream);
+                  : launch_cin1_kd<3>(x, x_bs, dy, dy_bs, nb, dw, ws, N, D, H, W, accumulate, stream, rc);
 }
 
 int mis_wgrad_cin1(const float* x, long long x_bs, const float* dy, long long dy_bs, float* dw, float* ws,
@@ -186,3 +237,17 @@
     const Cin1Norm nb{y, y_bs, mean, rstd, gamma, beta, reinterpret_cast<const float2*>(sums), slope, per_sample};
     return launch_cin1(x, x_bs, da, da_bs, &nb, dw, workspace, workspace_bytes, N, D, H, W, accumulate, stream);
 }
+
+extern "C" int mis_conv_wgrad_cin1_norm_rc(const float* x, long long x_bs, const float* da, long long da_bs,
+                                           const float* wp, const float* bias, int N, int D, int H, int W, int per_sample,
+                                           const float* mean, const float* rstd, const float* gamma, const float* beta,
+                                           const float* sums, float slope, float* dw, float* workspace,
+                                           long long workspace_bytes, int accumulate, hipStream_t stream) {
+    if (!x || !da || !wp || !mean || !rstd || !sums || !dw || !workspace || N <= 0) return MIS_ERR_ARG;
+    if (D == 1 || !mis_wgrad_cin1_eligible(N, 1, 16, D, H, W, 3, 3, 3) || (per_sample && (gamma || beta)))
+        return MIS_ERR_UNSUPPORTED;
+    if ((uintptr_t)sums & 7) return MIS_ERR_UNSUPPORTED;
+    const Cin1Norm nb{nullptr, 0, mean, rstd, gamma, beta, reinterpret_cast<const float2*>(sums), slope, per_sample};
+    const Cin1Rc rc{wp, bias};
+    return launch_cin1(x, x_bs, da, da_bs, &nb, dw, workspace, workspace_bytes, N, D, H, W, accumulate, stream, &rc);
+}
diff --git a/cv-ssl-mis_amd/csrc/norm_act.hip b/cv-ssl-mis_amd/csrc/norm_act.hip
--- a/cv-ssl-mis_amd/csrc/norm_act.hip
+++ b/cv-ssl-mis_amd/csrc/norm_act.hip
@@ -222,8 +222,8 @@
                                                         float* __restrict__ y, long long y_bs, ResArgs ra) {
     const int c = blockIdx.y, n = blockIdx.z;
     const int grp = g.per_sample ? (n * g.C + c) / g.cg : c;
-    const float sc = (gamma ? gamma[c] : 1.f) * rstd[grp];
-    const float sh = (beta ? beta[c] : 0.f) - mean[grp] * sc;
+    float sc, sh;
+    mis_norm_scale_shift(gamma ? gamma[c] : 1.f, beta ? beta[c] : 0.f, mean[grp], rstd[grp], sc, sh);
     const float* __restrict__ xb = x + (long long)n * g.x_bs + (long long)c * g.S;
     float* __restrict__ yb = y + (long long)n * y_bs + (long long)c * g.S;
     const unsigned long long lbase = ((unsigned long long)n * g.C + c) * g.S;
@@ -234,14 +234,15 @@
         const long long u = ((long long)blockIdx.x * APPLY_U + i) * 256 + threadIdx.x;
         if (u >= units) break;
         const float4 q = *reinterpret_cast<const float4*>(xb + u * 4);
-        float v[4] = {q.x * sc + sh, q.y * sc + sh, q.z * sc + sh, q.w * sc + sh};
+        float v[4] = {mis_norm_lin(q.x, sc, sh), mis_norm_lin(q.y, sc, sh), mis_norm_lin(q.z, sc, sh),
+                      mis_norm_lin(q.w, sc, sh)};
         float4 rq = make_float4(0.f, 0.f, 0.f, 0.f);
         if constexpr (RES) {
             rq = *reinterpret_cast<const float4*>(ra.r + (long long)n * ra.r_bs + (long long)c * g.S + u * 4);
             if (!ra.post) { v[0] += rq.x; v[1] += rq.y; v[2] += rq.z; v[3] += rq.w; }
         }
 #pragma unroll
-        for (int j = 0; j < 4; ++j) v[j] = v[j] > 0.f ? v[j] : v[j] * slope;
+        for (int j = 0; j < 4; ++j) v[j] = mis_lrelu(v[j], slope);
         if constexpr (RES) {
             if (ra.post) { v[0] += rq.x; v[1] += rq.y; v[2] += rq.z; v[3] += rq.w; }
         }
diff --git a/cv-ssl-mis_amd/mis_hip/lib.py b/cv-ssl-mis_amd/mis_hip/lib.py
--- a/cv-ssl-mis_amd/mis_hip/lib.py
+++ b/cv-ssl-mis_amd/mis_hip/lib.py
@@ -93,6 +93,11 @@
     "mis_conv_wgrad_cin1_norm_eligible": (c_i, [c_i, c_i, c_i, c_i, c_i]),
     "mis_conv_wgrad_cin1_norm": (c_i, [c_p, c_ll, c_p, c_ll, c_p, c_ll, c_i, c_i, c_i, c_i, c_i, c_p, c_p, c_p, c_p, c_p,
                                        c_f, c_p, c_p, c_ll, c_i, c_p]),
+    "mis_conv_fwd_cin1_stats": (c_i, [c_p, c_ll, c_p, c_p, c_i, c_i, c_i, c_i, c_p, c_ll, c_ll, c_p]),
+    "mis_conv_cin1_norm_act_fwd": (c_i, [c_p, c_ll, c_p, c_p, c_p, c_ll, c_p, c_ll, c_i, c_i, c_i, c_i, c_i, c_p, c_p, c_p,
+                                         c_p, c_f, c_p]),
+    "mis_conv_wgrad_cin1_norm_rc": (c_i, [c_p, c_ll, c_p, c_ll, c_p, c_p, c_i, c_i, c_i, c_i, c_i, c_p, c_p, c_p, c_p, c_p,
+                                          c_f, c_p, c_p, c_ll, c_i, c_p]),
     "mis_norm_head_eligible": (c_i, [c_i, c_i]),
     "mis_norm_head_workspace_bytes": (c_ll, [c_i, c_i, c_ll, c_i, c_i]),
     "mis_norm_head_fwd": (c_i, [c_p, c_ll, c_i, c_i, c_ll, c_i, c_p, c_p, c_p, c_p, c_f, c_f, c_u, c_p, c_p, c_p, c_p, c_i,
diff --git a/cv-ssl-mis_amd/mis_hip/ops.py b/cv-ssl-mis_amd/mis_hip/ops.py
--- a/cv-ssl-mis_amd/mis_hip/ops.py
+++ b/cv-ssl-mis_amd/mis_hip/ops.py
@@ -548,6 +548,48 @@
              "mis_conv_wgrad_cin1_norm")
 
 
+def conv_fwd_cin1_stats(x, wp, bias, stat):
+    L = _l.load()
+    N, Cin, D, H, W, S, xbs = _geom(x)
+    assert Cin == 1
+    prof = PROFILE
+    if prof is not None:
+        e0, e1 = torch.cuda.Event(enable_timing=True), torch.cuda.Event(enable_timing=True)
+        e0.record()
+    _l.check(L.mis_conv_fwd_cin1_stats(_l.ptr(x), xbs, _l.ptr(wp), _l.ptr(bias), N, D, H, W, _l.ptr(stat[0]), stat[1],
+                                       stat[2], _l.stream_ptr()), "mis_conv_fwd_cin1_stats")
+    if prof is not None:
+        e1.record()
+        buf = _ctypes.create_string_buffer(128)
+        L.mis_conv_fwd_kernel_name(N, 1, 16, D, H, W, 3, 3, 3, buf, 128)
+        prof.append((buf.value.decode(), 2.0 * N * 16 * 27 * S, e0, e1, 4.0 * (N * 17 * S + 16 * 27)))
+
+
+def conv_cin1_norm_act_fwd(x, wp, bias, r, y, per_sample, mean, rstd, gamma, beta, slope):
+    L = _l.load()
+    N, Cin, D, H, W, S, xbs = _geom(x)
+    _, Cy, _, _, _, _, ybs = _geom(y)
+    assert Cin == 1 and Cy == 16
+    rbs = _geom(r)[6] if r is not None else 0
+    _l.check(L.mis_conv_cin1_norm_act_fwd(_l.ptr(x), xbs, _l.ptr(wp), _l.ptr(bias), _l.ptr(r), rbs, _l.ptr(y), ybs, N, D,
+                                          H, W, int(per_sample), _l.ptr(mean), _l.ptr(rstd), _l.ptr(gamma), _l.ptr(beta),
+                                          slope, _l.stream_ptr()), "mis_conv_cin1_norm_act_fwd")
+
+
+def conv_wgrad_cin1_norm_rc(x, da, wp, bias, per_sample, mean, rstd, gamma, beta, sums, slope, dw, accumulate=False):
+    L = _l.load()
+    N, Cin, D, H, W, S, xbs = _geom(x)
+    _, Cout, _, _, _, _, dabs = _geom(da)
+    nb = L.mis_conv_wgrad_workspace_bytes(N, Cin, Cout, D, H, W, 3, 3, 3)
+    if nb < 0:
+        _l.check(nb, "mis_conv_wgrad_workspace_bytes")
+    ws = scratch(nb, "wgrad")
+    _l.check(L.mis_conv_wgrad_cin1_norm_rc(_l.ptr(x), xbs, _l.ptr(da), dabs, _l.ptr(wp), _l.ptr(bias), N, D, H, W,
+                                           int(per_sample), _l.ptr(mean), _l.ptr(rstd), _l.ptr(gamma), _l.ptr(beta),
+                                           _l.ptr(sums), slope, _l.ptr(dw), _l.ptr(ws), ws.numel(), int(accumulate),
+                                           _l.stream_ptr()), "mis_conv_wgrad_cin1_norm_rc")
+
+
 def norm_head_eligible(C, K, per_sample, gamma, beta, cg=1, no_norm=False):
     return bool(_l.load().mis_norm_head_eligible(C, K)) and cg == 1 and not no_norm and not (
         per_sample and (gamma is not None or beta is not None))
diff --git a/cv-ssl-mis_amd/mis_hip/plan.py b/cv-ssl-mis_amd/mis_hip/plan.py
--- a/cv-ssl-mis_amd/mis_hip/plan.py
+++ b/cv-ssl-mis_amd/mis_hip/plan.py
@@ -13,6 +13,7 @@
 FUSE_CONV_STATS = os.environ.get("MIS_FUSE_STATS", "1") != "0"
 FUSE_HEAD = os.environ.get("MIS_FUSE_HEAD", "1") != "0"
 FUSE_FIRST = os.environ.get("MIS_FUSE_FIRST", "1") != "0"
+FIRST_RECOMPUTE = int(os.environ.get("MIS_FIRST_RECOMPUTE", "3"))
 FUSE_POOL = os.environ.get("MIS_FUSE_POOL", "1") != "0"
 FUSE_POOL_FWD = os.environ.get("MIS_FUSE_POOL_FWD", "1") != "0"
 WGRAD_STREAM = os.environ.get("MIS_WGRAD_STREAM", "1") != "0"
@@ -93,6 +94,12 @@
         self.fused_into = None
         self.norm_bwd = None
         self.dgrad_norm = None
+        self.recompute = 0
+
+    def recompute_fwd(self, ctx):
+        n = self.norm_bwd
+        return (bool(self.recompute & 1) and self.stat is not None and (n.per_sample or ctx.training) and n.res is None
+                and n.pool is None and n.head is None)
 
     def fwd(self, ctx):
         if self.fused_into is not None:
@@ -101,6 +108,9 @@
             self.wp = ops.conv_pack(self.w.data, ops.conv_wino_pack_mode(self.wino_f, False) if self.wino_f >= 0 else 0,
                                     out=self.wp)
         stat = self.stat if (self.stat is not None and (self.stat_norm.per_sample or ctx.training)) else None
+        if self.recompute & 1 and self.recompute_fwd(ctx):
+            ops.conv_fwd_cin1_stats(self.x.t, self.wp, None if self.b is None else self.b.data, stat)
+            return
         ops.conv_fwd(self.x.t, self.wp, None if self.b is None else self.b.data, self.y.t, self.cin, self.cout,
                      self.ksize, stat=stat, wino=self.wino_f)
 
@@ -109,6 +119,11 @@
             return
         if self.norm_bwd is not None:
             n = self.norm_bwd
+            if self.recompute & 2:
+                ops.conv_wgrad_cin1_norm_rc(self.x.t, n.y.grad(), self.wp, None if self.b is None else self.b.data,
+                                            n.per_sample, n.mean, n.rstd, None if n.gamma is None else n.gamma.data,
+                                            None if n.beta is None else n.beta.data, n.sums, n.slope, self.w.grad)
+                return
             ops.conv_wgrad_cin1_norm(self.x.t, n.y.grad(), self.y.t, n.per_sample, n.mean, n.rstd,
                                      None if n.gamma is None else n.gamma.data, None if n.beta is None else n.beta.data,
                                      n.sums, n.slope, self.w.grad)
@@ -170,6 +185,7 @@
         self.res_post = False
         self.head = None
         self.head_w = self.head_b = None
+        self.first = None
 
     def fwd(self, ctx):
         if self.no_norm:
@@ -193,6 +209,13 @@
         self._state = ctx.state
         if self._p > 0 and self._mask is None and ctx.state is None:
             raise RuntimeError("dropout is active but no device step state was supplied (Ctx.state)")
+        c = self.first
+        if c is not None and c.recompute_fwd(ctx):
+            keep = None if getattr(ctx, "no_backward", False) else self.x.t
+            ops.conv_cin1_norm_act_fwd(c.x.t, c.wp, None if c.b is None else c.b.data, keep, self.y.t, self.per_sample,
+                                       self.mean, self.rstd, None if self.gamma is None else self.gamma.data,
+                                       None if self.beta is None else self.beta.data, self.slope)
+            return
         if self.res is not None:
             ops.norm_res_act_fwd(self.x.t, self.res.t, self.y.t, self.per_sample, self.mean, self.rstd,
                                  None if self.gamma is None else self.gamma.data,
@@ -544,6 +567,8 @@
             op.sums = torch.empty((x.shape[0] * x.shape[1] if per_sample else x.shape[1], 2), dtype=torch.float32,
                                   device="cuda")
             prev.norm_bwd = op
+            if prev.ksize == (3, 3, 3) and prev.wino_f < 0 and prev.stat_norm is op and prev.cout == 16:
+                prev.recompute, op.first = FIRST_RECOMPUTE, prev
         self.ops.append(op)
         return y
 
diff --git a/include/mis_hip.h b/include/mis_hip.h
--- a/include/mis_hip.h
+++ b/include/mis_hip.h
@@ -127,6 +127,17 @@
                              const float* rstd, const float* gamma, const float* beta, const float* sums, float slope,
                              float* dw, float* workspace, long long workspace_bytes, int accumulate,
                              mis_stream_t stream);
+int mis_conv_fwd_cin1_stats(const float* x, long long x_bs, const float* wp, const float* bias, int N, int D, int H, int W,
+                            float* stat, long long stat_sc, long long stat_sn, mis_stream_t stream);
+int mis_conv_cin1_norm_act_fwd(const float* x, long long x_bs, const float* wp, const float* bias, float* r, long long r_bs,
+                               float* y, long long y_bs, int N, int D, int H, int W, int per_sample, const float* mean,
+                               const float* rstd, const float* gamma, const float* beta, float slope,
+                               mis_stream_t stream);
+int mis_conv_wgrad_cin1_norm_rc(const float* x, long long x_bs, const float* da, long long da_bs, const float* wp,
+                                const float* bias, int N, int D, int H, int W, int per_sample, const float* mean,
+                                const float* rstd, const float* gamma, const float* beta, const float* sums, float slope,
+                                float* dw, float* workspace, long long workspace_bytes, int accumulate,
+                                mis_stream_t stream);
 
 int mis_norm_head_eligible(int C, int K);
 long long mis_norm_head_workspace_bytes(int N, int C, long long S, int per_sample, int K);
```

Result: no change. 455.9, median of 5 (+0.7%).
